# zju3dv/Diffuman4D

Measured on AMD Instinct MI355X. Metric: denoised view-frame latents/sec (44cam x 150fr grid), higher is better.
Workload: dtype bf16; 1 GPU; demo_4d 44cam x 150fr, sliding_fast (window 12, stride 2, 3 rounds, 18 steps/latent), CFG 2.0, 72x40x4 latents; step = 2 spatial (F=16) + 1 temporal (F=24) window calls = 2 denoised latents; VAE excluded; mode=task, unet=SD-2.1 geometry (320,640,1280,1280), 815.6M params, random init seed 0, parallelism=task-parallel x1 (independent tasks per round, no data-path collective), task_streams=3, task_batch=2, precision=fast, finite_outputs=True

## Files before the change

diffuman4d_amd/csrc/gemm.hip:

```cpp
#include "common.h"
#include "gemm_common.h"
#include "gemm_select.h"
#include <stdio.h>


namespace {

template <int BM, int BN, int WM, int WN, bool CONV, int PAR = 0>
__global__ __launch_bounds__(256) void gemm_kernel_glds(GemmParams p) {
  constexpr int BK = 64;
  constexpr int TM = BM / WM, TN = BN / WN, MI = TM / 32, NI = TN / 32;
  constexpr int AW = BM / 32, BW = BN / 32;
  static_assert(WM * WN == 4, "4 waves");
  constexpr int SMEM_MAIN = 2 * (BM + BN) * BK * 2;
  constexpr int SMEM_EPI = 4 * 32 * (EpiGeom<TN>::EPW + 4) * 4;
  constexpr int SMEM_BYTES = SMEM_MAIN > SMEM_EPI ? SMEM_MAIN : SMEM_EPI;
  __shared__ __attribute__((aligned(16))) u16 smem[SMEM_BYTES / 2];
  u16* As = smem;
  u16* Bs = smem + 2 * BM * BK;

  const int tid = threadIdx.x, lane = tid & 63;
  const int wave = __builtin_amdgcn_readfirstlane(tid >> 6);
  const int wm = wave / WN, wn = wave % WN;
  const int l31 = lane & 31, lh = lane >> 5;
// ... 90 lines not shown

  const int sw = (l31 >> 1) & 7;
  issue_slab(0, 0);
  __syncthreads();
  for (int kt = 0; kt < nk; ++kt) {
    const int buf = kt & 1;
    if (kt + 1 < nk) issue_slab(kt + 1, buf ^ 1);
    bf16x8_t af[2][MI], bfr[2][NI];
    auto read_frags = [&](int ks, int slot) {
      const int pos = ((ks * 2 + lh) ^ sw) * 8;
#pragma unroll
      for (int i = 0; i < MI; ++i)
        af[slot][i] = *reinterpret_cast<const bf16x8_t*>(As + (buf * BM + wm * TM + i * 32 + l31) * BK + pos);
#pragma unroll
      for (int j = 0; j < NI; ++j)
        bfr[slot][j] = *reinterpret_cast<const bf16x8_t*>(Bs + (buf * BN + wn * TN + j * 32 + l31) * BK + pos);
    };
    read_frags(0, 0);
#pragma unroll
    for (int ks = 0; ks < 4; ++ks) {
      if (ks + 1 < 4) read_frags(ks + 1, (ks + 1) & 1);
#pragma unroll
      for (int i = 0; i < MI; ++i)
#pragma unroll
        for (int j = 0; j < NI; ++j)
          acc[i][j] = mfma_t<PAR>(af[ks & 1][i], bfr[ks & 1][j], acc[i][j]);
    }
    __syncthreads();
  }
  gemm_epilogue<MI, NI, TM, TN, EpiBudget<WM * WN, MI, NI, SMEM_BYTES>::STRAIGHT, PAR>(p, acc, reinterpret_cast<float*>(smem), m0, n0, wm, wn, wave, lane);
}

template <int Q, int R, int q = 0>
__device__ __forceinline__ void sched_mfma_with_reads() {
  if constexpr (q < Q) {
    constexpr int lo = (q * R) / Q, hi = ((q + 1) * R) / Q;
    if constexpr (hi > lo) __builtin_amdgcn_sched_group_barrier(0x100, hi - lo, 0);
    __builtin_amdgcn_sched_group_barrier(0x008, 1, 0);
    sched_mfma_with_reads<Q, R, q + 1>();
  }
}

template <int MI, int NI, bool RELOAD, int q = 0>
__device__ __forceinline__ void sched_mfma_reload() {
  if constexpr (q < MI * NI) {
    __builtin_amdgcn_sched_group_barrier(0x008, 1, 0);
    constexpr int i = q / NI, j = q % NI;
    constexpr int n = RELOAD ? ((j == NI - 1 ? 1 : 0) + (i == MI - 1 ? 1 : 0)) : 0;
    if constexpr (n > 0) __builtin_amdgcn_sched_group_barrier(0x100, n, 0);
    sched_mfma_reload<MI, NI, RELOAD, q + 1>();
  }
}

template <int BM, int BN, int WM, int WN, int KT = 3, int PAR = 0>
__global__ __launch_bounds__(WM* WN * 64, (BN % 64 != 0 ? 2 : 1)) void conv_strip2_kernel(GemmParams p_in) {
  static_assert(KT == 2 || KT == 3, "3x3 taps, or the 2x2 taps of one upsampling phase");
  constexpr int BK = 64, ROWB = BK * 2;
  constexpr int NW = WM * WN;
  constexpr int TM = BM / WM, TN = BN / WN, MI = TM / 32, NI = TN / 32;
  constexpr int NA = (BM + 8) / 8;
  constexpr int SR = BM + 16;
  constexpr int ZROW = BM + 8;
  constexpr int NB = BN / 8;
  constexpr int AW = (NA + NW - 1) / NW, BW = (NB + NW - 1) / NW;
  constexpr int A_BYTES = SR * ROWB, B_BYTES = BN * ROWB;
  constexpr int SMEM_MAIN = 2 * (A_BYTES + B_BYTES);
  constexpr int SMEM_EPI = NW * 32 * (EpiGeom<TN>::EPW + 4) * 4;
  constexpr int SMEM_BYTES = SMEM_MAIN > SMEM_EPI ? SMEM_MAIN : SMEM_EPI;
  static_assert(SMEM_BYTES <= 160 * 1024, "tile does not fit the LDS");
  static_assert(2 * A_BYTES + 2 * B_BYTES - 1 + 0 < (1 << 20), "LDS offsets");
  __shared__ __attribute__((aligned(16))) char smem[SMEM_BYTES];
  constexpr int BS0 = 2 * A_BYTES;

  const int tid = threadIdx.x, lane = tid & 63;
  const int wave = __builtin_amdgcn_readfirstlane(tid >> 6);
  const int wm = wave / WN, wn = wave % WN;
  const int l31 = lane & 31, lh = lane >> 5;
  int lid = xcd_remap(blockIdx.x, gridDim.x);
  GemmParams p = p_in;
  int xs = -1, ys = -1;
  if constexpr (KT == 2) {
    const int per = gridDim.x / 4, phase = lid / per;
    lid -= phase * per;
    const int py = phase >> 1, px = phase & 1;
    xs = px - 1;
    ys = py - 1;
    p.Wt = p_in.Wt + (int64_t)phase * p_in.N * p_in.ldw;
    p.C = p_in.C + ((int64_t)py * 2 * p_in.W + px) * p_in.ldc * ((PAR && (p_in.flags & DM4D_EPI_F32OUT)) ? 2 : 1);
  }
  int split = 0, tm, tn;
  if (KT == 3 && p.splits > 1) {
    const int rows = gridDim.x / p.tiles_n;
    const int tms = lid % rows;
    tn = lid / rows;
    split = tms / (rows / p.splits);
    tm = tms % (rows / p.splits);
  } else {
    tn = lid % p.tiles_n;
    tm = lid / p.tiles_n;
  }
  const int m0 = tm * BM, n0 = tn * BN;
  const int d_row = lane >> 3, d_pos = lane & 7;
  if (tid < 16) *reinterpret_cast<U4*>(smem + (tid >> 3) * A_BYTES + ZROW * ROWB + (tid & 7) * 16) = U4{0u, 0u, 0u, 0u};

  uint32_t a_voff[AW];
  auto set_a_voff = [&](int ky) {
#pragma unroll
// ... 133 lines not shown
            acc[i][j] = mfma_t<PAR>(af[i], bfr[j], acc[i][j]);
            if (ks + 1 < 4) {
              if (j == NI - 1) af[i] = read_a(ks + 1, i);
              if (i == MI - 1) bfr[j] = read_b(ks + 1, j);
            }
          }
      __builtin_amdgcn_sched_group_barrier(0x100, MI + NI, 0);
      sched_mfma_reload<MI, NI, true>();
      sched_mfma_reload<MI, NI, true>();
      sched_mfma_reload<MI, NI, true>();
      sched_mfma_reload<MI, NI, false>();
    }
  };
  const int cin = p.Cin;
  int c_ky = ky0, c_cs = 0;
  const u16* wp = p.Wt + ky0 * KT * cin;
  set_a_voff(ky0);
  issue_a(p.A, 0);
  issue_b(wp, 0);
  asm volatile("s_waitcnt vmcnt(0)" ::: "memory");
  __syncthreads();
  for (int g = 0; g < nstrips; ++g) {
    if (c_cs == 0) set_a_addrs(c_ky);
    const int abuf = g & 1;
    const int b0 = KT == 3 ? abuf : 0;
    issue_b(wp + cin, b0 ^ 1);
    compute(abuf, std::integral_constant<int, 0>{});
    dma_wait_barrier();
    if constexpr (KT == 3) {
      issue_b(wp + 2 * cin, b0);
      compute(abuf, std::integral_constant<int, 1>{});
      dma_wait_barrier();
    }
    if (++c_cs == nci) {
      c_cs = 0;
      ++c_ky;
    }
    if (g + 1 < nstrips) {
      if (c_cs == 0) set_a_voff(c_ky);
      wp = p.Wt + (c_ky * KT * cin + c_cs * BK);
      issue_a(p.A + c_cs * BK, abuf ^ 1);
      issue_b(wp, KT == 3 ? (abuf ^ 1) : 0);
    }
    compute(abuf, std::integral_constant<int, KT - 1>{});
    dma_wait_barrier();
  }
  if (KT == 3 && p.splits > 1) {
    p.C = reinterpret_cast<u16*>(p.ws + (int64_t)split * p.M * p.N);
    p.ldc = p.N;
    p.flags = DM4D_EPI_F32OUT;
    p.bias = p.rowbias = p.res = nullptr;
    p.out_scale = 1.0f;
  }
  gemm_epilogue<MI, NI, TM, TN, EpiBudget<WM * WN, MI, NI, SMEM_BYTES>::STRAIGHT, PAR>(p, acc, reinterpret_cast<float*>(smem), m0, n0, wm, wn, wave, lane);
}

template <int BM, int BN, int WM, int WN, int NST, bool CONV, int BK = 32, int PAR = 0>
__global__ __launch_bounds__(WM* WN * 64) void gemm_kernel_pipe(GemmParams p) {
  constexpr int NW = WM * WN;
  static_assert(BK == 32 || BK == 64, "K-slab of 32 (64-byte row pieces) or 64 (whole 128-byte lines)");
  constexpr int RPI = 1024 / (BK * 2);
  constexpr int TM = BM / WM, TN = BN / WN, MI = TM / 32, NI = TN / 32;
  constexpr int AW = BM / RPI / NW, BW = BN / RPI / NW;
  static_assert(AW >= 1 && BW >= 1 && NST >= 2 && NST <= 4, "tile/wave/stage combination");
  constexpr int LD = AW + BW;
  constexpr int STAGE = (BM + BN) * BK;
  constexpr int SMEM_MAIN = NST * STAGE * 2;
  constexpr int SMEM_EPI = NW * 32 * (EpiGeom<TN>::EPW + 4) * 4;
  constexpr int SMEM_BYTES = SMEM_MAIN > SMEM_EPI ? SMEM_MAIN : SMEM_EPI;
  __shared__ __attribute__((aligned(16))) u16 smem[SMEM_BYTES / 2];

  const int tid = threadIdx.x, lane = tid & 63;
  const int wave = __builtin_amdgcn_readfirstlane(tid >> 6);
  const int wm = wave / WN, wn = wave % WN;
  const int l31 = lane & 31, lh = lane >> 5;
  const int bid = xcd_remap(blockIdx.x, gridDim.x);
  const int tn = bid % p.tiles_n, tm = bid / p.tiles_n;
  const int m0 = tm * BM;
  const bool geglu = (p.flags & DM4D_EPI_GEGLU) != 0;
  const int n0 = tn * (geglu ? BN / 2 : BN);

  constexpr int CPRW = BK / 8;
  const int d_row = lane / CPRW, d_pos = lane % CPRW;
  auto src_chunk = [&](int row) { return BK == 32 ? (d_pos ^ ((row >> 2) & 3)) : (d_pos ^ ((row >> 1) & 7)); };
  const u16* a_src[AW];
  const u16* a2_src[AW];
  int iy0[AW], ix0[AW], img_off[AW], tap_off[AW];
#pragma unroll
  for (int i = 0; i < AW; ++i) {
    img_off[i] = tap_off[i] = 0;
    const int d_chunk = src_chunk((wave + NW * i) * RPI + d_row);
    int m = m0 + (wave + NW * i) * RPI + d_row;
    if (m > p.M - 1) m = p.M - 1;
    if constexpr (CONV) {
      int ox = m % p.Wo;
      int t = m / p.Wo;
      int oy = t % p.Ho;
      int b = t / p.Ho;
      iy0[i] = oy * p.stride - p.pad;
      ix0[i] = ox * p.stride - p.pad;
      img_off[i] = b * p.H * p.W * p.Cin + d_chunk * 8;
      a_src[i] = p.A;
      a2_src[i] = nullptr;
    } else {
      a_src[i] = p.A + (int64_t)m * p.lda + d_chunk * 8;
      a2_src[i] = p.A2 ? p.A2 + (int64_t)m * p.lda2 + d_chunk * 8 : nullptr;
      iy0[i] = ix0[i] = 0;
    }
  }
  const u16* w_src[BW];
// ... 39 lines not shown
      }
      __builtin_amdgcn_global_load_lds((gptr_t)src, (lptr_t)(As + (wave + NW * i) * RPI * BK), 16, 0, 0);
    }
    if constexpr (CONV) {
      ci0 += BK;
      if (ci0 >= p.Cin) {
        ci0 = 0;
        if (++kx == 3) {
          kx = 0;
          ++ky;
        }
      }
    }
#pragma unroll
    for (int i = 0; i < BW; ++i)
      __builtin_amdgcn_global_load_lds((gptr_t)(w_src[i] + kt * BK), (lptr_t)(Bs + (wave + NW * i) * RPI * BK), 16, 0, 0);
  };

  const int sw = BK == 32 ? ((l31 >> 2) & 3) : ((l31 >> 1) & 7);
#pragma unroll
  for (int s = 0; s < NST - 1; ++s)
    if (s < nk) issue_slab(s, s);
  int st = 0, st_issue = NST - 1;
  for (int kt = 0; kt < nk; ++kt) {
    const int younger = nk - 1 - kt;
    if (NST >= 4 && younger >= 2) {
      asm volatile("s_waitcnt vmcnt(%0)" ::"n"(2 * LD) : "memory");
    } else if (NST >= 3 && younger >= 1) {
      asm volatile("s_waitcnt vmcnt(%0)" ::"n"(LD) : "memory");
    } else {
      asm volatile("s_waitcnt vmcnt(0)" ::: "memory");
    }
    __builtin_amdgcn_s_barrier();
    asm volatile("" ::: "memory");
    if (kt + NST - 1 < nk) issue_slab(kt + NST - 1, st_issue);
    const u16* As = smem + st * STAGE;
    const u16* Bs = As + BM * BK;
#pragma unroll
    for (int ks = 0; ks < BK / 16; ++ks) {
      const int pos = ((ks * 2 + lh) ^ sw) * 8;
      bf16x8_t af[MI], bfr[NI];
#pragma unroll
      for (int i = 0; i < MI; ++i) af[i] = *reinterpret_cast<const bf16x8_t*>(As + (wm * TM + i * 32 + l31) * BK + pos);
#pragma unroll
      for (int j = 0; j < NI; ++j) bfr[j] = *reinterpret_cast<const bf16x8_t*>(Bs + (wn * TN + j * 32 + l31) * BK + pos);
#pragma unroll
      for (int i = 0; i < MI; ++i)
#pragma unroll
        for (int j = 0; j < NI; ++j) acc[i][j] = mfma_t<PAR>(af[i], bfr[j], acc[i][j]);
    }
    st = (st + 1 == NST) ? 0 : st + 1;
    st_issue = (st_issue + 1 == NST) ? 0 : st_issue + 1;
  }
  gemm_epilogue<MI, NI, TM, TN, EpiBudget<WM * WN, MI, NI, SMEM_BYTES>::STRAIGHT, PAR>(p, acc, reinterpret_cast<float*>(smem), m0, n0, wm, wn, wave, lane);
}

template <int BM, int BN, int WM, int WN, int NST, int BK = 64, int PAR = 0>
__global__ __launch_bounds__(WM* WN * 64) void gemm_lin2_kernel(GemmParams p) {
  static_assert(BK == 32 || BK == 64, "K-slab of 32 (64-byte rows, 16 per DMA instruction) or 64 (128-byte rows, 8 per instruction)");
  constexpr int ROWB = BK * 2, RPI = 1024 / ROWB, CPR = BK / 8, KS = BK / 16;
  constexpr int NW = WM * WN;
  constexpr int TM = BM / WM, TN = BN / WN, MI = TM / 32, NI = TN / 32;
  constexpr int AW = BM / RPI / NW, BW = BN / RPI / NW;
  static_assert(AW >= 1 && BW >= 1 && NST >= 2 && NST <= 3, "tile/wave/stage combination");
  constexpr int LD = AW + BW;
  constexpr int STAGE_BYTES = (BM + BN) * ROWB;
  constexpr int SMEM_MAIN = NST * STAGE_BYTES;
  constexpr int SMEM_EPI = NW * 32 * (EpiGeom<TN>::EPW + 4) * 4;
  constexpr int SMEM_BYTES = SMEM_MAIN > SMEM_EPI ? SMEM_MAIN : SMEM_EPI;
  static_assert(SMEM_BYTES <= 160 * 1024, "tile does not fit the LDS");
  __shared__ __attribute__((aligned(16))) char smem[SMEM_BYTES];

  const int tid = threadIdx.x, lane = tid & 63;
  const int wave = __builtin_amdgcn_readfirstlane(tid >> 6);
  const int wm = wave / WN, wn = wave % WN;
  const int l31 = lane & 31, lh = lane >> 5;
  const int bid = xcd_remap(blockIdx.x, gridDim.x);
  const int tn = bid % p.tiles_n, tm = bid / p.tiles_n;
  const int m0 = tm * BM;
  const bool geglu = (p.flags & DM4D_EPI_GEGLU) != 0;
  const int n0 = tn * (geglu ? BN / 2 : BN);
  const int d_row = lane / CPR, d_pos = lane % CPR;
  auto key = [](int row) { return BK == 64 ? ((row >> 1) & 7) : ((row >> 2) & 3); };

  uint32_t a_voff[AW], a2_voff[AW], w_voff[BW];
#pragma unroll
  for (int i = 0; i < AW; ++i) {
    const int row = (wave + NW * i) * RPI + d_row;
    const uint32_t chunk = (uint32_t)(d_pos ^ key(row)) * 16u;
    int m = m0 + row;
    if (m > p.M - 1) m = p.M - 1;
    a_voff[i] = (uint32_t)m * (uint32_t)(p.lda * 2) + chunk;
    a2_voff[i] = (uint32_t)m * (uint32_t)(p.lda2 * 2) + chunk;
  }
#pragma unroll
  for (int i = 0; i < BW; ++i) {
    const int row = (wave + NW * i) * RPI + d_row;
    w_voff[i] = (uint32_t)weight_row<TN>(p, n0, row, geglu) * (uint32_t)(p.ldw * 2) + (uint32_t)(d_pos ^ key(row)) * 16u;
  }
  const uint32_t lds0 = lds_addr(smem);
  const uint32_t a_dst0 = lds0 + wave * 1024, b_dst0 = lds0 + BM * ROWB + wave * 1024;
  const int k1 = p.A2 ? p.K1 : p.K;
  auto issue_slab = [&](int kt, int st) {
    const int k = kt * BK;
    const uint32_t so = st * STAGE_BYTES;
    if (k < k1) {
      const u16* ab = p.A + k;
#pragma unroll
      for (int i = 0; i < AW; ++i) dma16_sv(ab, a_voff[i], a_dst0 + so + NW * i * 1024);
    } else {
// ... 55 lines not shown
        sched_mfma_with_reads<MI * NI, MI + NI>();
        sched_mfma_with_reads<MI * NI, MI + NI>();
      }
      sched_mfma_with_reads<MI * NI, 0>();
    } else {
      bf16x8_t af[MI], bfr[NI];
#pragma unroll
      for (int i = 0; i < MI; ++i) af[i] = read_a(0, i);
#pragma unroll
      for (int j = 0; j < NI; ++j) bfr[j] = read_b(0, j);
#pragma unroll
      for (int ks = 0; ks < KS; ++ks)
#pragma unroll
        for (int i = 0; i < MI; ++i)
#pragma unroll
          for (int j = 0; j < NI; ++j) {
            acc[i][j] = mfma_t<PAR>(af[i], bfr[j], acc[i][j]);
            if (ks + 1 < KS) {
              if (j == NI - 1) af[i] = read_a(ks + 1, i);
              if (i == MI - 1) bfr[j] = read_b(ks + 1, j);
            }
          }
      __builtin_amdgcn_sched_group_barrier(0x100, MI + NI, 0);
      sched_mfma_reload<MI, NI, true>();
      if constexpr (KS == 4) {
        sched_mfma_reload<MI, NI, true>();
        sched_mfma_reload<MI, NI, true>();
      }
      sched_mfma_reload<MI, NI, false>();
    }
  };

  const int nk = p.K / BK;
#pragma unroll
  for (int s = 0; s < NST - 1; ++s)
    if (s < nk) issue_slab(s, s);
  int st = 0, st_issue = NST - 1;
  for (int kt = 0; kt < nk; ++kt) {
    if (NST >= 3 && nk - 1 - kt >= 1) {
      asm volatile("s_waitcnt vmcnt(%0) lgkmcnt(0)" ::"n"(LD) : "memory");
    } else {
      asm volatile("s_waitcnt vmcnt(0) lgkmcnt(0)" ::: "memory");
    }
    __builtin_amdgcn_s_barrier();
    asm volatile("" ::: "memory");
    if (kt + NST - 1 < nk) issue_slab(kt + NST - 1, st_issue);
    compute(st);
    st = (st + 1 == NST) ? 0 : st + 1;
    st_issue = (st_issue + 1 == NST) ? 0 : st_issue + 1;
  }
  asm volatile("s_waitcnt lgkmcnt(0)" ::: "memory");
  __builtin_amdgcn_s_barrier();
  asm volatile("" ::: "memory");
  gemm_epilogue<MI, NI, TM, TN, EpiBudget<WM * WN, MI, NI, SMEM_BYTES>::STRAIGHT, PAR>(p, acc, reinterpret_cast<float*>(smem), m0, n0, wm, wn, wave, lane);
}

template <int BM, int BN, int WM, int WN, bool CONV, int PAR = 0>
__global__ __launch_bounds__(256) void gemm_kernel(GemmParams p) {
  constexpr int LDK = 40;
  constexpr int TM = BM / WM, TN = BN / WN, MI = TM / 32, NI = TN / 32;
  constexpr int AI = BM / 64, BI = BN / 64;
  static_assert(WM * WN == 4, "4 waves");
  constexpr int SMEM_MAIN = 2 * (BM + BN) * LDK * 2;
  constexpr int SMEM_EPI = 4 * 32 * (EpiGeom<TN>::EPW + 4) * 4;
  constexpr int SMEM_BYTES = SMEM_MAIN > SMEM_EPI ? SMEM_MAIN : SMEM_EPI;
  __shared__ __attribute__((aligned(16))) u16 smem[SMEM_BYTES / 2];
  u16* As = smem;
  u16* Bs = smem + 2 * BM * LDK;

  const int tid = threadIdx.x, lane = tid & 63, wave = tid >> 6;
  const int wm = wave / WN, wn = wave % WN;
  const int l31 = lane & 31, lh = lane >> 5;
  const int bid = xcd_remap(blockIdx.x, gridDim.x);
  const int tn = bid % p.tiles_n, tm = bid / p.tiles_n;
  const int m0 = tm * BM;
  const bool geglu = (p.flags & DM4D_EPI_GEGLU) != 0;
  const int n0 = tn * (geglu ? BN / 2 : BN);
  const int a_c = tid & 3, a_r = tid >> 2;

  const u16* a_base[AI];
  const u16* a2_base[AI];
  int iy0[AI], ix0[AI];
#pragma unroll
  for (int i = 0; i < AI; ++i) {
    int m = m0 + a_r + 64 * i;
    if (m > p.M - 1) m = p.M - 1;
    if constexpr (CONV) {
      int ox = m % p.Wo;
      int t = m / p.Wo;
      int oy = t % p.Ho;
      int b = t / p.Ho;
      iy0[i] = oy * p.stride - p.pad;
      ix0[i] = ox * p.stride - p.pad;
      a_base[i] = p.A + (int64_t)b * p.H * p.W * p.Cin;
      a2_base[i] = nullptr;
    } else {
      a_base[i] = p.A + (int64_t)m * p.lda;
      a2_base[i] = p.A2 ? p.A2 + (int64_t)m * p.lda2 : nullptr;
      iy0[i] = ix0[i] = 0;
    }
  }
  const u16* w_base[BI];
#pragma unroll
  for (int i = 0; i < BI; ++i) w_base[i] = p.Wt + (int64_t)weight_row<TN>(p, n0, a_r + 64 * i, geglu) * p.ldw;

  f32x16_t acc[MI][NI];
  acc_init<MI, NI, TN, PAR>(p, acc, n0, wn, lane, geglu);

  const int nk = p.K / 32;
  const int Hin = p.upsample ? 2 * p.H : p.H, Win = p.upsample ? 2 * p.W : p.W;
// ... 8 lines not shown
        bool ok = (unsigned)iy < (unsigned)Hin && (unsigned)ix < (unsigned)Win;
        int sy = p.upsample ? (iy >> 1) : iy, sx = p.upsample ? (ix >> 1) : ix;
        U4 z = {0u, 0u, 0u, 0u};
        ra[i] = ok ? ldg16(a_base[i] + ((int64_t)sy * p.W + sx) * p.Cin + ci0 + a_c * 8) : z;
      }
      ci0 += 32;
      if (ci0 >= p.Cin) {
        ci0 = 0;
        if (++kx == 3) {
          kx = 0;
          ++ky;
        }
      }
    } else {
      const int kcol = kt * 32;
      const bool second = (p.A2 != nullptr) && (kcol >= p.K1);
#pragma unroll
      for (int i = 0; i < AI; ++i)
        ra[i] = second ? ldg16(a2_base[i] + (kcol - p.K1) + a_c * 8) : ldg16(a_base[i] + kcol + a_c * 8);
    }
#pragma unroll
    for (int i = 0; i < BI; ++i) rb[i] = ldg16(w_base[i] + kt * 32 + a_c * 8);
  };
  auto store_slab = [&](int buf) {
#pragma unroll
    for (int i = 0; i < AI; ++i) *reinterpret_cast<U4*>(As + (buf * BM + a_r + 64 * i) * LDK + a_c * 8) = ra[i];
#pragma unroll
    for (int i = 0; i < BI; ++i) *reinterpret_cast<U4*>(Bs + (buf * BN + a_r + 64 * i) * LDK + a_c * 8) = rb[i];
  };

  load_slab(0);
  store_slab(0);
  __syncthreads();
  for (int kt = 0; kt < nk; ++kt) {
    const int buf = kt & 1;
    if (kt + 1 < nk) load_slab(kt + 1);
#pragma unroll
    for (int ks = 0; ks < 2; ++ks) {
      bf16x8_t af[MI], bfr[NI];
#pragma unroll
      for (int i = 0; i < MI; ++i)
        af[i] = *reinterpret_cast<const bf16x8_t*>(As + (buf * BM + wm * TM + i * 32 + l31) * LDK + ks * 16 + lh * 8);
#pragma unroll
      for (int j = 0; j < NI; ++j)
        bfr[j] = *reinterpret_cast<const bf16x8_t*>(Bs + (buf * BN + wn * TN + j * 32 + l31) * LDK + ks * 16 + lh * 8);
#pragma unroll
      for (int i = 0; i < MI; ++i)
#pragma unroll
        for (int j = 0; j < NI; ++j) acc[i][j] = mfma_t<PAR>(af[i], bfr[j], acc[i][j]);
    }
    if (kt + 1 < nk) store_slab(buf ^ 1);
    __syncthreads();
  }
  gemm_epilogue<MI, NI, TM, TN, EpiBudget<WM * WN, MI, NI, SMEM_BYTES>::STRAIGHT, PAR>(p, acc, reinterpret_cast<float*>(smem), m0, n0, wm, wn, wave, lane);
}

template <int BM, int BN>
unsigned tile_grid(GemmParams& p) {
  const int bn_out = is_geglu(p) ? BN / 2 : BN;
  p.tiles_n = (p.N + bn_out - 1) / bn_out;
  return (unsigned)(((p.M + BM - 1) / BM) * p.tiles_n);
}

template <int BM, int BN, int WM, int WN, bool CONV, bool GLDS, int PAR = 0>
int launch_cfg(hipStream_t st, GemmParams& p) {
  const dim3 grid(tile_grid<BM, BN>(p));
  if constexpr (GLDS) {
    hipLaunchKernelGGL((gemm_kernel_glds<BM, BN, WM, WN, CONV, PAR>), grid, dim3(256), 0, st, p);
  } else {
    hipLaunchKernelGGL((gemm_kernel<BM, BN, WM, WN, CONV, PAR>), grid, dim3(256), 0, st, p);
  }
  return dm4d_check_launch("gemm_kernel");
}

template <int BM, int BN, int WM, int WN, int NST, bool CONV, int BK = 32, int PAR = 0>
int launch_pipe(hipStream_t st, GemmParams& p) {
  const dim3 grid(tile_grid<BM, BN>(p));
  hipLaunchKernelGGL((gemm_kernel_pipe<BM, BN, WM, WN, NST, CONV, BK, PAR>), grid, dim3(WM * WN * 64), 0, st, p);
  return dm4d_check_launch("gemm_kernel_pipe");
}

template <int BM, int BN, int WM, int WN, int NST, int BK = 64, int PAR = 0>
int launch_lin2(hipStream_t st, GemmParams& p) {
  const dim3 grid(tile_grid<BM, BN>(p));
  hipLaunchKernelGGL((gemm_lin2_kernel<BM, BN, WM, WN, NST, BK, PAR>), grid, dim3(WM * WN * 64), 0, st, p);
  return dm4d_check_launch("gemm_lin2_kernel");
}

template <int PAR = 0>
__global__ __launch_bounds__(256) void splitk_reduce_kernel(GemmParams p) {
  const int nv = p.N / 8;
  const int64_t id = (int64_t)blockIdx.x * 256 + threadIdx.x;
  if (id >= (int64_t)p.M * nv) return;
  const int m = (int)(id / nv), n = (int)(id % nv) * 8;
  const int64_t plane = (int64_t)p.M * p.N;
  const float* w = p.ws + (int64_t)m * p.N + n;
  float v[8];
  {
    const f32x4_t a0 = *reinterpret_cast<const f32x4_t*>(w), a1 = *reinterpret_cast<const f32x4_t*>(w + 4);
    v[0] = a0[0]; v[1] = a0[1]; v[2] = a0[2]; v[3] = a0[3];
    v[4] = a1[0]; v[5] = a1[1]; v[6] = a1[2]; v[7] = a1[3];
  }
  for (int s = 1; s < p.splits; ++s) {
    const f32x4_t a0 = *reinterpret_cast<const f32x4_t*>(w + s * plane), a1 = *reinterpret_cast<const f32x4_t*>(w + s * plane + 4);
    v[0] += a0[0]; v[1] += a0[1]; v[2] += a0[2]; v[3] += a0[3];
    v[4] += a1[0]; v[5] += a1[1]; v[6] += a1[2]; v[7] += a1[3];
  }
  const bool f32side = PAR == 2 && (p.flags & DM4D_EPI_F32SIDE) != 0;
  auto side = [&](const u16* base, int64_t off, float* t) {
    if (f32side) {
      const float* f = reinterpret_cast<const float*>(base) + off;
      const f32x4_t t0 = *reinterpret_cast<const f32x4_t*>(f), t1 = *reinterpret_cast<const f32x4_t*>(f + 4);
      t[0] = t0[0]; t[1] = t0[1]; t[2] = t0[2]; t[3] = t0[3];
      t[4] = t1[0]; t[5] = t1[1]; t[6] = t1[2]; t[7] = t1[3];
    } else if constexpr (PAR == 2) {
      unpack8h(ldg16(base + off), t);
    } else {
      unpack8(ldg16(base + off), t);
    }
  };
  float t[8];
  if (p.bias) {
    if constexpr (PAR == 2) unpack8h(ldg16(p.bias + n), t);
    else unpack8(ldg16(p.bias + n), t);
#pragma unroll
    for (int e = 0; e < 8; ++e) v[e] += t[e];
  }
  if (p.rowbias) {
    side(p.rowbias, (int64_t)(m / p.rows_per_rb) * p.ld_rb + n, t);
#pragma unroll
    for (int e = 0; e < 8; ++e) v[e] += t[e];
  }
  if (p.res) {
    side(p.res, (int64_t)m * p.ld_res + n, t);
#pragma unroll
    for (int e = 0; e < 8; ++e) v[e] += t[e];
  }
#pragma unroll
  for (int e = 0; e < 8; ++e) v[e] *= p.out_scale;
  if (PAR == 2 && (p.flags & DM4D_EPI_F32OUT)) {
    float* cf = reinterpret_cast<float*>(p.C) + (int64_t)m * p.ldc + n;
    const f32x4_t o0 = {v[0], v[1], v[2], v[3]}, o1 = {v[4], v[5], v[6], v[7]};
    *reinterpret_cast<f32x4_t*>(cf) = o0;
    *reinterpret_cast<f32x4_t*>(cf + 4) = o1;
  } else if constexpr (PAR == 2) {
    stg16(p.C + (int64_t)m * p.ldc + n, pack8h(v));
  } else {
    stg16(p.C + (int64_t)m * p.ldc + n, pack8(v));
  }
}

template <int BM, int BN, int WM, int WN, int PAR = 0>
int launch_strip2(hipStream_t st, GemmParams& p) {
  if (!strip2_ok(p)) return DM4D_ERR_ARG;
  if (BN % 64 != 0 && p.splits > 1) return DM4D_ERR_ARG;
  if (p.splits < 1) p.splits = 1;
  const dim3 grid(tile_grid<BM, BN>(p) * p.splits);
  hipLaunchKernelGGL((conv_strip2_kernel<BM, BN, WM, WN, 3, PAR>), grid, dim3(WM * WN * 64), 0, st, p);
  int rc = dm4d_check_launch("conv_strip2_kernel");
  if (rc || p.splits == 1) return rc;
  const int64_t nthreads = (int64_t)p.M * (p.N / 8);
  hipLaunchKernelGGL((splitk_reduce_kernel<PAR>), dim3((unsigned)((nthreads + 255) / 256)), dim3(256), 0, st, p);
  return dm4d_check_launch("splitk_reduce_kernel");
}

template <int BM, int BN, int WM, int WN, int PAR = 0>
int launch_up2x(hipStream_t st, GemmParams& p) {
  p.splits = 1;
  const dim3 grid(4 * tile_grid<BM, BN>(p));
  hipLaunchKernelGGL((conv_strip2_kernel<BM, BN, WM, WN, 2, PAR>), grid, dim3(WM * WN * 64), 0, st, p);
  return dm4d_check_launch("conv_strip2_kernel<up2x>");
}

template <bool H16 = false>
__global__ __launch_bounds__(256) void up2x_prepare_kernel(const u16* W, u16* Wp, int N, int Cin) {
  const int64_t total = (int64_t)4 * N * 4 * Cin;
  const int64_t id = (int64_t)blockIdx.x * 256 + threadIdx.x;
  if (id >= total) return;
  const int ci = (int)(id % Cin);
  int64_t t = id / Cin;
  const int dx = (int)(t & 1), dy = (int)((t >> 1) & 1);
  t >>= 2;
  const int n = (int)(t % N), phase = (int)(t / N);
  const int py = phase >> 1, px = phase & 1;
  const int ky_lo = py == 0 ? (dy == 0 ? 0 : 1) : (dy == 0 ? 0 : 2), ky_hi = py == 0 ? (dy == 0 ? 0 : 2) : (dy == 0 ? 1 : 2);
  const int kx_lo = px == 0 ? (dx == 0 ? 0 : 1) : (dx == 0 ? 0 : 2), kx_hi = px == 0 ? (dx == 0 ? 0 : 2) : (dx == 0 ? 1 : 2);
  float acc = 0.f;
  for (int ky = ky_lo; ky <= ky_hi; ++ky)
    for (int kx = kx_lo; kx <= kx_hi; ++kx) {
      const u16 w = W[(int64_t)n * 9 * Cin + (ky * 3 + kx) * Cin + ci];
      acc += H16 ? h2f(w) : bf2f(w);
    }
  Wp[id] = H16 ? f2h(acc) : f2bf(acc);
}

int g_tune_cfg = 0;

template <int ID, bool CONV, int PAR>
int launch_id(hipStream_t st, GemmParams& p) {
  constexpr bool STRIP = ID >= 31 && ID <= 37, LIN2 = ID >= 61;
  const bool geglu = is_geglu(p);
  if constexpr ((STRIP && !CONV) || (LIN2 && CONV)) return DM4D_ERR_ARG;
  else if ((ID <= 4 && !k64<CONV>(p)) || (STRIP && !strip_conv(p)) || (LIN2 && !lin2_ok(p))) return DM4D_ERR_ARG;
  else if constexpr (ID == 1) return launch_cfg<128, 128, 2, 2, CONV, true, PAR>(st, p);
  else if constexpr (ID == 2) return launch_cfg<256, 64, 4, 1, CONV, true, PAR>(st, p);
  else if constexpr (ID == 3) return launch_cfg<128, 64, 4, 1, CONV, true, PAR>(st, p);
  else if constexpr (ID == 4) return geglu ? DM4D_ERR_ARG : launch_cfg<64, 64, 2, 2, CONV, true, PAR>(st, p);
  else if constexpr (ID == 13) return launch_pipe<256, 256, 2, 4, 4, CONV, 32, PAR>(st, p);
  else if constexpr (ID == 14) return launch_pipe<256, 128, 4, 2, 3, CONV, 32, PAR>(st, p);
  else if constexpr (ID == 20) return launch_pipe<256, 256, 4, 4, 4, CONV, 32, PAR>(st, p);
  else if constexpr (ID == 46) return (k64<CONV>(p) && !geglu) ? launch_pipe<256, 320, 4, 2, 2, CONV, 64, PAR>(st, p) : DM4D_ERR_ARG;
  else if constexpr (ID == 31) return launch_strip2<128, 128, 2, 2, PAR>(st, p);
  else if constexpr (ID == 32) return launch_strip2<256, 128, 4, 2, PAR>(st, p);
  else if constexpr (ID == 33) return launch_strip2<128, 64, 4, 1, PAR>(st, p);
  else if constexpr (ID == 34) return launch_strip2<256, 256, 2, 4, PAR>(st, p);
  else if constexpr (ID == 35) return launch_strip2<256, 320, 4, 2, PAR>(st, p);
  else if constexpr (ID == 36) return launch_strip2<128, 160, 4, 1, PAR>(st, p);
  else if constexpr (ID == 37) return launch_strip2<256, 160, 8, 1, PAR>(st, p);
  else if constexpr (ID == 67) return launch_lin2<256, 256, 2, 4, 2, 64, PAR>(st, p);
  else if constexpr (ID == 65) return launch_lin2<256, 128, 4, 2, 3, 32, PAR>(st, p);
  else if constexpr (ID == 61) return launch_lin2<256, 128, 4, 2, 3, 64, PAR>(st, p);
  else if constexpr (ID == 69) return geglu ? DM4D_ERR_ARG : launch_lin2<128, 160, 4, 1, 2, 64, PAR>(st, p);
  else if constexpr (ID == 63) return launch_lin2<128, 128, 2, 2, 2, 64, PAR>(st, p);
  else if constexpr (ID == 64) return launch_lin2<128, 128, 4, 2, 3, 64, PAR>(st, p);
  else if constexpr (ID == 21) return launch_cfg<256, 128, 2, 2, CONV, false, PAR>(st, p);
  else if constexpr (ID == 22) return launch_cfg<128, 128, 2, 2, CONV, false, PAR>(st, p);
  else if constexpr (ID == 23) return launch_cfg<256, 64, 4, 1, CONV, false, PAR>(st, p);
  else return launch_cfg<128, 64, 4, 1, CONV, false, PAR>(st, p);
}

template <bool CONV, int PAR>
int launch_from(IdList<>, int, hipStream_t, GemmParams&) { return DM4D_ERR_ARG; }
template <bool CONV, int PAR, int ID, int... REST>
int launch_from(IdList<ID, REST...>, int id, hipStream_t st, GemmParams& p) {
  return id == ID ? launch_id<ID, CONV, PAR>(st, p) : launch_from<CONV, PAR>(IdList<REST...>{}, id, st, p);
}
template <bool CONV, int PAR = 0>
int launch_by_id(int id, hipStream_t st, GemmParams& p) {
  return launch_from<CONV, PAR>(std::conditional_t<PAR == 1, ParIds<CONV>, AllIds>{}, id, st, p);
}

template <bool CONV, bool H16>
int launch(hipStream_t st, GemmParams& p) {
  const bool par = !H16 && (p.flags & (DM4D_EPI_F32SIDE | DM4D_EPI_SPLITOUT)) != 0, forced = !H16 && !par && g_tune_cfg != 0;
  const GemmChoice c = forced ? GemmChoice{g_tune_cfg, 1} : select_cfg<CONV>(p, H16 ? PREC_H16 : par ? PREC_PAR : PREC_FAST);
  if (!c.id) return dm4d_set_error(DM4D_ERR_ARG, "conv3x3: parity-precision launches need Cin % 64 == 0 (a two-term operand of Cin / 2 channels)");
  p.splits = c.splits;
  int rc;
  if constexpr (H16) rc = launch_by_id<CONV, 2>(c.id, st, p);
  else rc = par ? launch_by_id<CONV, 1>(c.id, st, p) : launch_by_id<CONV>(c.id, st, p);
  if (forced && rc == DM4D_ERR_ARG) return dm4d_set_error(DM4D_ERR_ARG, "gemm: forced configuration does not support this shape");
  return rc;
}

int arg_error(const char* name, const char* what) {
  char msg[256];
  snprintf(msg, sizeof(msg), "%s: %s", name, what);
  return dm4d_set_error(DM4D_ERR_ARG, msg);
}

template <bool H16>
int gemm_entry(const char* name, void* stream, const void* A, int64_t lda, const void* A2, int64_t lda2, int K1, const void* W, int64_t ldw, void* C,
               int64_t ldc, int M, int N, int K, const void* bias, const void* rowbias, int64_t ld_rowbias, int rows_per_rowbias,
               const void* residual, int64_t ld_res, unsigned flags, float out_scale, int scale_cols, float col_scale) {
  if (!A || !W || !C || M <= 0 || N <= 0 || K <= 0) return arg_error(name, "null pointer or empty shape");
  if (K % 32 != 0) return arg_error(name, "K must be a multiple of 32");
  if ((lda & 7) || (ldw & 7)) return arg_error(name, "lda/ldw must be multiples of 8");
  if (A2 && ((K1 % 32) != 0 || K1 <= 0 || K1 >= K || (lda2 & 7))) return arg_error(name, "bad split-A arguments");
  if (rowbias && rows_per_rowbias <= 0) return arg_error(name, "rows_per_rowbias <= 0");
  if ((flags & DM4D_EPI_GEGLU) && (N % 32 != 0)) return arg_error(name, "GEGLU needs N % 32 == 0");
  if (H16 && (flags & ~(DM4D_EPI_GEGLU | DM4D_EPI_SILU | DM4D_EPI_F32OUT | DM4D_EPI_F32SIDE)))
    return arg_error(name, "only GEGLU, SILU, F32OUT and F32SIDE apply");
  if (H16 && (scale_cols < 0 || scale_cols > N || (scale_cols & 7))) return arg_error(name, "scale_cols must be a multiple of 8 in [0, N]");
  GemmParams p{};
  p.A = (const u16*)A; p.lda = lda; p.A2 = (const u16*)A2; p.lda2 = lda2; p.K1 = K1;
  p.Wt = (const u16*)W; p.ldw = ldw; p.C = (u16*)C; p.ldc = ldc; p.M = M; p.N = N; p.K = K;
  p.bias = (const u16*)bias; p.rowbias = (const u16*)rowbias; p.ld_rb = ld_rowbias; p.rows_per_rb = rows_per_rowbias;
  p.res = (const u16*)residual; p.ld_res = ld_res; p.flags = H16 ? flags | DM4D_EPI_H16 : flags; p.out_scale = out_scale;
  p.scale_cols = scale_cols; p.col_scale = col_scale;
  return launch<false, H16>((hipStream_t)stream, p);
}

template <bool H16>
int conv3x3_entry(const char* name, void* stream, const void* X, int B, int H, int W, int Cin, const void* Wt, void* Y, int Ho, int Wo, int Cout,
                  int stride, int pad, int upsample, const void* bias, const void* rowbias, int64_t ld_rowbias, const void* residual, int64_t ld_res,
                  float out_scale, unsigned flags, void* ws, size_t ws_bytes) {
  if (!X || !Wt || !Y || B <= 0 || H <= 0 || W <= 0 || Ho <= 0 || Wo <= 0 || Cout <= 0) return arg_error(name, "null pointer or empty shape");
  if (Cin % 32 != 0) return arg_error(name, "Cin must be a multiple of 32 (pad the input)");
  if (stride != 1 && stride != 2) return arg_error(name, "stride must be 1 or 2");
  if (upsample && stride != 1) return arg_error(name, "upsample needs stride 1");
  if (flags & ~(DM4D_EPI_F32OUT | DM4D_EPI_F32SIDE)) return arg_error(name, "only DM4D_EPI_F32OUT and DM4D_EPI_F32SIDE apply to a convolution");
  if ((int64_t)B * H * W * Cin >= (int64_t)1 << 31 || (int64_t)B * Ho * Wo * Cout >= (int64_t)1 << 31)
    return arg_error(name, "tensors of 2^31 or more elements are not supported (split the batch)");
  GemmParams p{};
  p.A = (const u16*)X; p.H = H; p.W = W; p.Cin = Cin; p.Ho = Ho; p.Wo = Wo; p.stride = stride; p.pad = pad; p.upsample = upsample;
  p.Wt = (const u16*)Wt; p.ldw = (int64_t)9 * Cin; p.C = (u16*)Y; p.ldc = Cout; p.M = B * Ho * Wo; p.N = Cout; p.K = 9 * Cin;
  p.bias = (const u16*)bias; p.rowbias = (const u16*)rowbias; p.ld_rb = ld_rowbias; p.rows_per_rb = Ho * Wo;
  p.res = (const u16*)residual; p.ld_res = ld_res; p.flags = H16 ? flags | DM4D_EPI_H16 : flags; p.out_scale = out_scale;
  const size_t need = strip_ws_bytes(p, B);
  p.ws = (ws && need && ws_bytes >= need) ? (float*)ws : nullptr;
  return launch<true, H16>((hipStream_t)stream, p);
}

template <bool H16>
int conv_up2x_entry(const char* name, void* stream, const void* X, int B, int H, int W, int Cin, const void* Wp, void* Y, int Cout, const void* bias,
                    unsigned flags) {
  if (!X || !Wp || !Y || B <= 0 || H <= 0 || W <= 0 || Cout <= 0) return arg_error(name, "null pointer or empty shape");
  if (Cin % 64 != 0 || (Cout & 7) != 0)
    return arg_error(name, H16 ? "Cin must be a multiple of 64 and Cout of 8 (use conv3x3_f16 with upsample = 1)"
                               : "Cin must be a multiple of 64 and Cout of 8 (use conv3x3 with upsample = 1)");
  if (H16 && (flags & ~DM4D_EPI_F32OUT)) return arg_error(name, "only DM4D_EPI_F32OUT applies");
  if ((int64_t)B * H * W * Cin >= (int64_t)1 << 31 || (int64_t)B * 4 * H * W * Cout >= (int64_t)1 << 31)
    return arg_error(name, "tensors of 2^31 or more elements are not supported (split the batch)");
  GemmParams p{};
  p.A = (const u16*)X; p.H = H; p.W = W; p.Cin = Cin; p.Ho = H; p.Wo = W; p.stride = 1; p.pad = 1; p.upsample = 0;
  p.Wt = (const u16*)Wp; p.ldw = (int64_t)4 * Cin; p.C = (u16*)Y; p.ldc = Cout; p.M = B * H * W; p.N = Cout; p.K = 4 * Cin;
  p.bias = (const u16*)bias; p.rows_per_rb = H * W; p.flags = H16 ? flags | DM4D_EPI_H16 : flags; p.out_scale = 1.0f; p.up_w = W;
  if (!strip2_ok(p)) return arg_error(name, "input or weights of 4 GiB or more");
  constexpr int PAR = H16 ? 2 : 0;
  hipStream_t st = (hipStream_t)stream;
  switch (choose_up2x(p)) {
    case 32: return launch_up2x<256, 128, 4, 2, PAR>(st, p);
    case 31: return launch_up2x<128, 128, 2, 2, PAR>(st, p);
    default: return launch_up2x<128, 64, 4, 1, PAR>(st, p);
  }
}

template <bool H16>
int conv_up2x_prepare_entry(const char* name, void* stream, const void* W, void* Wp, int Cout, int Cin) {
  if (!W || !Wp || Cout <= 0 || Cin <= 0) return arg_error(name, "null pointer or empty shape");
  const int64_t total = (int64_t)16 * Cout * Cin;
  hipLaunchKernelGGL(up2x_prepare_kernel<H16>, dim3((unsigned)((total + 255) / 256)), dim3(256), 0, (hipStream_t)stream,
                     (const u16*)W, (u16*)Wp, Cout, Cin);
  return dm4d_check_launch("up2x_prepare_kernel");
}

}

#ifdef DM4D_GEMM_H16_TU
extern "C" int dm4d_gemm_f16(void* stream, const void* A, int64_t lda, const void* A2, int64_t lda2, int K1, const void* W, int64_t ldw, void* C,
                             int64_t ldc, int M, int N, int K, const void* bias, const void* rowbias, int64_t ld_rowbias, int rows_per_rowbias,
                             const void* residual, int64_t ld_res, unsigned flags, float out_scale, int scale_cols, float col_scale) {
  return gemm_entry<true>("gemm_f16", stream, A, lda, A2, lda2, K1, W, ldw, C, ldc, M, N, K, bias, rowbias, ld_rowbias, rows_per_rowbias, residual,
                          ld_res, flags, out_scale, scale_cols, col_scale);
}

extern "C" int dm4d_conv3x3_nhwc_f16(void* stream, const void* X, int B, int H, int W, int Cin, const void* Wt, void* Y, int Ho, int Wo, int Cout,
                                     int stride, int pad, int upsample, const void* bias, const void* rowbias, int64_t ld_rowbias,
                                     const void* residual, int64_t ld_res, float out_scale, unsigned flags, void* ws, size_t ws_bytes) {
  return conv3x3_entry<true>("conv3x3_f16", stream, X, B, H, W, Cin, Wt, Y, Ho, Wo, Cout, stride, pad, upsample, bias, rowbias, ld_rowbias, residual,
                             ld_res, out_scale, flags, ws, ws_bytes);
}

extern "C" int dm4d_conv_up2x_prepare_f16(void* stream, const void* W, void* Wp, int Cout, int Cin) {
  return conv_up2x_prepare_entry<true>("conv_up2x_prepare_f16", stream, W, Wp, Cout, Cin);
}

extern "C" int dm4d_conv_up2x_nhwc_f16(void* stream, const void* X, int B, int H, int W, int Cin, const void* Wp, void* Y, int Cout, const void* bias,
                                       unsigned flags) {
  return conv_up2x_entry<true>("conv_up2x_f16", stream, X, B, H, W, Cin, Wp, Y, Cout, bias, flags);
}
#else

extern "C" int dm4d_tune_set_gemm_config(int id) {
  g_tune_cfg = id;
  return DM4D_OK;
}

extern "C" int dm4d_gemm_bf16(void* stream, const void* A, int64_t lda, const void* A2, int64_t lda2, int K1, const void* W, int64_t ldw, void* C,
                              int64_t ldc, int M, int N, int K, const void* bias, const void* rowbias, int64_t ld_rowbias, int rows_per_rowbias,
                              const void* residual, int64_t ld_res, unsigned flags, float out_scale) {
  return gemm_entry<false>("gemm", stream, A, lda, A2, lda2, K1, W, ldw, C, ldc, M, N, K, bias, rowbias, ld_rowbias, rows_per_rowbias, residual, ld_res,
                           flags, out_scale, 0, 0.0f);
}

extern "C" size_t dm4d_conv3x3_ws_bytes(int B, int H, int W, int Cin, int Ho, int Wo, int Cout, int stride, int pad, int upsample) {
  GemmParams p{};
  p.H = H; p.W = W; p.Cin = Cin; p.Ho = Ho; p.Wo = Wo; p.stride = stride; p.pad = pad; p.upsample = upsample; p.N = Cout; p.ldc = Cout;
  return strip_ws_bytes(p, B);
}

extern "C" int dm4d_conv3x3_nhwc_bf16(void* stream, const void* X, int B, int H, int W, int Cin, const void* Wt, void* Y, int Ho, int Wo, int Cout,
                                      int stride, int pad, int upsample, const void* bias, const void* rowbias, int64_t ld_rowbias,
                                      const void* residual, int64_t ld_res, float out_scale) {
  return conv3x3_entry<false>("conv3x3", stream, X, B, H, W, Cin, Wt, Y, Ho, Wo, Cout, stride, pad, upsample, bias, rowbias, ld_rowbias, residual,
                              ld_res, out_scale, 0, nullptr, 0);
}

extern "C" int dm4d_conv3x3_nhwc_bf16_flags(void* stream, const void* X, int B, int H, int W, int Cin, const void* Wt, void* Y, int Ho, int Wo,
                                            int Cout, int stride, int pad, int upsample, const void* bias, const void* rowbias, int64_t ld_rowbias,
                                            const void* residual, int64_t ld_res, float out_scale, unsigned flags) {
  return conv3x3_entry<false>("conv3x3", stream, X, B, H, W, Cin, Wt, Y, Ho, Wo, Cout, stride, pad, upsample, bias, rowbias, ld_rowbias, residual,
                              ld_res, out_scale, flags, nullptr, 0);
}

extern "C" int dm4d_conv3x3_nhwc_bf16_ws(void* stream, const void* X, int B, int H, int W, int Cin, const void* Wt, void* Y, int Ho, int Wo, int Cout,
                                         int stride, int pad, int upsample, const void* bias, const void* rowbias, int64_t ld_rowbias,
                                         const void* residual, int64_t ld_res, float out_scale, void* ws, size_t ws_bytes) {
  return conv3x3_entry<false>("conv3x3", stream, X, B, H, W, Cin, Wt, Y, Ho, Wo, Cout, stride, pad, upsample, bias, rowbias, ld_rowbias, residual,
                              ld_res, out_scale, 0, ws, ws_bytes);
}

extern "C" int dm4d_conv_up2x_prepare_bf16(void* stream, const void* W, void* Wp, int Cout, int Cin) {
  return conv_up2x_prepare_entry<false>("conv_up2x_prepare", stream, W, Wp, Cout, Cin);
}

extern "C" int dm4d_conv_up2x_nhwc_bf16(void* stream, const void* X, int B, int H, int W, int Cin, const void* Wp, void* Y, int Cout,
                                        const void* bias) {
  return conv_up2x_entry<false>("conv_up2x", stream, X, B, H, W, Cin, Wp, Y, Cout, bias, 0);
}
#endif
```

diffuman4d_amd/csrc/gemm_common.h:

```cpp
#pragma once
#include "common.h"
#include "dm4d.h"
#include "errors.h"
#include "gemm_params.h"
#include <stdlib.h>
#include <type_traits>

namespace {

__device__ __attribute__((aligned(16))) const uint32_t g_zero16[4] = {0u, 0u, 0u, 0u};

template <int TN>
__device__ __forceinline__ int weight_row(const GemmParams& p, int n0, int r, bool geglu) {
  int n;
  if (geglu) {
    int wr = r / TN, rr = r % TN;
    n = n0 + wr * (TN / 2) + (rr % (TN / 2));
    if (n > p.N - 1) n = p.N - 1;
    if (rr >= TN / 2) n += p.N;
  } else {
    n = n0 + r;
    if (n > p.N - 1) n = p.N - 1;
  }
  return n;
// ... 12 lines not shown
#pragma unroll
    for (int q = 0; q < 4; ++q) {
      float v[4];
#pragma unroll
      for (int e = 0; e < 4; ++e) {
        const int r = 4 * q + e;
        v[e] = a[J0 + j][r];
        if constexpr (geglu) {
          v[e] = v[e] * gelu_erf_f(a[J0 + j + NI / 2][r]);
        }
        if constexpr (MODE == 1) v[e] = silu_f(v[e]);
      }
      if constexpr (PLAIN) {
        uint2 pk;
        pk.x = pack_bf2(v[0], v[1]);
        pk.y = pack_bf2(v[2], v[3]);
        *reinterpret_cast<uint2*>(reinterpret_cast<u16*>(srow) + j * 32 + 8 * q) = pk;
      } else {
        const f32x4_t v4 = {v[0], v[1], v[2], v[3]};
        *reinterpret_cast<f32x4_t*>(reinterpret_cast<float*>(srow) + j * 32 + 8 * q) = v4;
      }
    }
  }
}

__device__ __forceinline__ bf16x8_t k0_fragment(u16 bits, int lh) {
  union {
    uint32_t u[4];
    bf16x8_t v;
  } f;
  f.u[0] = lh ? 0u : (uint32_t)bits;
  f.u[1] = f.u[2] = f.u[3] = 0u;
  return f.v;
}

template <int MI, int NI, int TN, int PAR = 0>
__device__ __forceinline__ void acc_init(const GemmParams& p, f32x16_t (&acc)[MI][NI], int n0, int wn, int lane, bool geglu) {
  const int l31 = lane & 31, lh = lane >> 5;
  const bf16x8_t one0 = k0_fragment(PAR == 2 ? 0x3c00 : 0x3f80, lh);
  f32x16_t zero;
#pragma unroll
  for (int r = 0; r < 16; ++r) zero[r] = 0.f;
  const bool use = p.bias != nullptr && p.splits <= 1;
#pragma unroll
  for (int j = 0; j < NI; ++j) {
    u16 bits = 0;
    if (use) bits = p.bias[weight_row<TN>(p, n0, wn * TN + j * 32 + l31, geglu)];
    const bf16x8_t bf = k0_fragment(bits, lh);
#pragma unroll
    for (int i = 0; i < MI; ++i) acc[i][j] = mfma_t<PAR>(one0, bf, zero);
  }
}

template <int MI, int NI, int TM, int TN, int MODE, int EPW, int J0, int JN, bool SYNC, bool STRAIGHT, int PAR = 0>
__device__ __forceinline__ void gemm_epilogue_impl(const GemmParams& p, f32x16_t (&acc)[MI][NI], float* smem_f, int m0, int n0,
                                                   int wm, int wn, int wave, int lane) {
  const int l31 = lane & 31, lh = lane >> 5;
  constexpr bool geglu = MODE == 2;
  constexpr int NJ = geglu ? NI / 2 : NI;
  static_assert(J0 + JN <= NJ && JN * 32 <= EPW, "column group outside the wave's tile or wider than its staging area");
  constexpr int TNO = JN * 32;
  constexpr int SLD = TNO + 4;
  constexpr int SBH = TNO + 4;
  constexpr int CPR = TNO / 8;
  constexpr int TASKS = 32 * CPR;
  float* stage = smem_f + wave * 32 * (EPW + 4);
  const int ncol0 = n0 + wn * (NJ * 32) + J0 * 32;

  const bool vec_ok = ((p.ldc & 7) == 0) && ((p.N & 7) == 0) && (!p.res || (p.ld_res & 7) == 0) &&
                      (!p.rowbias || (p.ld_rb & 7) == 0);
  const bool f32out = (p.flags & DM4D_EPI_F32OUT) != 0;
  constexpr bool CPR_POW2 = (CPR & (CPR - 1)) == 0;
  constexpr int cshift = CPR >= 16 ? 4 : (CPR >= 8 ? 3 : (CPR >= 4 ? 2 : (CPR >= 2 ? 1 : 0)));
  constexpr int cmask = CPR - 1;
  constexpr bool H16 = PAR == 2;
  const bool f32side = PAR && (p.flags & DM4D_EPI_F32SIDE) != 0, splitout = PAR == 1 && (p.flags & DM4D_EPI_SPLITOUT) != 0;
  const bool fast_ok = CPR_POW2 && vec_ok && p.ldc < (1 << 24) && (!p.res || p.ld_res < (1 << 24)) &&
                       (!p.rowbias || p.rows_per_rb > 0) && !f32out && !(PAR && (f32side || splitout)) && p.up_w == 0 && !H16;
  const bool plain = fast_ok && !p.res && !p.rowbias && p.out_scale == 1.0f;
  if constexpr (SYNC) __syncthreads();
#pragma unroll
  for (int i = 0; i < MI; ++i) {
    const int m_base = m0 + wm * TM + i * 32;
    if (plain) {
      u16* sb = reinterpret_cast<u16*>(stage);
      u16* srow = sb + l31 * SBH + 4 * lh;
      stage_block<NI, MODE, J0, JN, true>(acc[i], srow);
      __builtin_amdgcn_fence(__ATOMIC_RELEASE, "wavefront");
      __builtin_amdgcn_fence(__ATOMIC_ACQUIRE, "wavefront");
      u16* c_base = p.C + (int64_t)m_base * p.ldc + ncol0;
      if (TASKS % 64 == 0 && m_base + 32 <= p.M && ncol0 + TNO <= p.N) {
        U4 o[TASKS / 64 > 0 ? TASKS / 64 : 1];
#pragma unroll
        for (int it = 0; it < TASKS / 64; ++it) {
          const int id = lane + it * 64;
          const int row = id >> cshift, cc = id & cmask;
          const uint2* s = reinterpret_cast<const uint2*>(sb + row * SBH + cc * 8);
          const uint2 lo = s[0], hi = s[1];
          o[it].x = lo.x; o[it].y = lo.y; o[it].z = hi.x; o[it].w = hi.y;
        }
#pragma unroll
        for (int it = 0; it < TASKS / 64; ++it) {
          const int id = lane + it * 64;
          const int row = id >> cshift, cc = id & cmask;
          stg16(c_base + (uint32_t)(row * (int)p.ldc + cc * 8), o[it]);
        }
      } else {
#pragma unroll
        for (int it = 0; it < (TASKS + 63) / 64; ++it) {
          const int id = lane + it * 64;
          if (TASKS % 64 != 0 && id >= TASKS) continue;
          const int row = id >> cshift, cc = id & cmask;
          if (m_base + row >= p.M || ncol0 + cc * 8 >= p.N) continue;
          const uint2* s = reinterpret_cast<const uint2*>(sb + row * SBH + cc * 8);
          const uint2 lo = s[0], hi = s[1];
          U4 o;
          o.x = lo.x; o.y = lo.y; o.z = hi.x; o.w = hi.y;
          stg16(c_base + (uint32_t)(row * (int)p.ldc + cc * 8), o);
        }
      }
      __builtin_amdgcn_fence(__ATOMIC_RELEASE, "wavefront");
      __builtin_amdgcn_fence(__ATOMIC_ACQUIRE, "wavefront");
      continue;
    }
    float* srow = stage + l31 * SLD + 4 * lh;
    stage_block<NI, MODE, J0, JN, false>(acc[i], srow);
    __builtin_amdgcn_fence(__ATOMIC_RELEASE, "wavefront");
    __builtin_amdgcn_fence(__ATOMIC_ACQUIRE, "wavefront");
    if (fast_ok) {
      const u16* res_base = p.res ? p.res + (int64_t)m_base * p.ld_res + ncol0 : nullptr;
      u16* c_base = p.C + (int64_t)m_base * p.ldc + ncol0;
      int q0 = 0, r0 = 0;
      if (p.rowbias) {
        q0 = m_base / p.rows_per_rb;
        r0 = m_base - q0 * p.rows_per_rb;
      }
// ... 242 lines not shown
              const u16 hi = f2bf(x);
              p.C[mo * p.ldc + n + e] = hi;
              p.C[mo * p.ldc + p.N + n + e] = f2bf(x - bf2f(hi));
            } else {
              p.C[mo * p.ldc + n + e] = f2bf(x);
            }
          }
        }
      } else {
        if (vec_ok) {
          if (p.rowbias) {
            float t[8];
            unpack8(ldg16(p.rowbias + (int64_t)(m / p.rows_per_rb) * p.ld_rb + n), t);
  #pragma unroll
            for (int e = 0; e < 8; ++e) v[e] += t[e];
          }
          if (p.res) {
            float t[8];
            unpack8(ldg16(p.res + (int64_t)m * p.ld_res + n), t);
  #pragma unroll
            for (int e = 0; e < 8; ++e) v[e] += t[e];
          }
  #pragma unroll
          for (int e = 0; e < 8; ++e) v[e] *= p.out_scale;
          if (f32out) {
            float* cf = reinterpret_cast<float*>(p.C) + mo * p.ldc + n;
            f32x4_t o0 = {v[0], v[1], v[2], v[3]}, o1 = {v[4], v[5], v[6], v[7]};
            *reinterpret_cast<f32x4_t*>(cf) = o0;
            *reinterpret_cast<f32x4_t*>(cf + 4) = o1;
          } else {
            stg16(p.C + mo * p.ldc + n, pack8(v));
          }
        } else {
          for (int e = 0; e < 8 && n + e < p.N; ++e) {
            float x = v[e];
            if (p.rowbias) x += bf2f(p.rowbias[(int64_t)(m / p.rows_per_rb) * p.ld_rb + n + e]);
            if (p.res) x += bf2f(p.res[(int64_t)m * p.ld_res + n + e]);
            if (f32out) reinterpret_cast<float*>(p.C)[mo * p.ldc + n + e] = x * p.out_scale;
            else p.C[mo * p.ldc + n + e] = f2bf(x * p.out_scale);
          }
        }
      }
    }
    __builtin_amdgcn_fence(__ATOMIC_RELEASE, "wavefront");
    __builtin_amdgcn_fence(__ATOMIC_ACQUIRE, "wavefront");
  }
}

template <int TN>
struct EpiGeom {
  static constexpr int EPW = TN <= 128 ? TN : 128;
};

template <int MI, int NI, int TM, int TN, int MODE, bool STRAIGHT, int PAR = 0>
__device__ __forceinline__ void gemm_epilogue_mode(const GemmParams& p, f32x16_t (&acc)[MI][NI], float* smem_f, int m0, int n0,
                                                   int wm, int wn, int wave, int lane) {
  constexpr int NJ = MODE == 2 ? NI / 2 : NI;
  constexpr int EPW = EpiGeom<TN>::EPW;
  constexpr int G = EPW / 32;
  if constexpr (NJ <= G) {
    gemm_epilogue_impl<MI, NI, TM, TN, MODE, EPW, 0, NJ, true, STRAIGHT, PAR>(p, acc, smem_f, m0, n0, wm, wn, wave, lane);
  } else {
    static_assert(NJ <= 2 * G, "at most two column groups");
    gemm_epilogue_impl<MI, NI, TM, TN, MODE, EPW, 0, G, true, STRAIGHT, PAR>(p, acc, smem_f, m0, n0, wm, wn, wave, lane);
    gemm_epilogue_impl<MI, NI, TM, TN, MODE, EPW, G, NJ - G, false, STRAIGHT, PAR>(p, acc, smem_f, m0, n0, wm, wn, wave, lane);
  }
}

template <int NW, int MI, int NI, int SMEM>
struct EpiBudget {
  static constexpr bool STRAIGHT = NW <= 8 && MI * NI <= 8 && !(NW == 8 && SMEM <= 80 * 1024);
};

template <int MI, int NI, int TM, int TN, bool STRAIGHT = false, int PAR = 0>
__device__ __forceinline__ void gemm_epilogue(const GemmParams& p, f32x16_t (&acc)[MI][NI], float* smem_f, int m0, int n0,
                                              int wm, int wn, int wave, int lane) {
  if constexpr (NI >= 2 && NI % 2 == 0) {
    if (p.flags & DM4D_EPI_GEGLU) {
      gemm_epilogue_mode<MI, NI, TM, TN, 2, STRAIGHT, PAR>(p, acc, smem_f, m0, n0, wm, wn, wave, lane);
      return;
    }
  }
  if (p.flags & DM4D_EPI_SILU) gemm_epilogue_mode<MI, NI, TM, TN, 1, STRAIGHT, PAR>(p, acc, smem_f, m0, n0, wm, wn, wave, lane);
  else gemm_epilogue_mode<MI, NI, TM, TN, 0, STRAIGHT, PAR>(p, acc, smem_f, m0, n0, wm, wn, wave, lane);
}


__device__ __forceinline__ void dma16_sv(const void* uniform_base, uint32_t lane_byte_off, uint32_t lds_dst) {
  asm volatile("s_mov_b32 m0, %2\n\ts_nop 0\n\tglobal_load_lds_dwordx4 %0, %1"
               :
               : "v"(lane_byte_off), "s"(uniform_base), "s"(lds_dst)
               : "memory");
}


}
```

diffuman4d_amd/csrc/gemm_params.h:

```cpp
#pragma once
#include <stdint.h>

typedef unsigned short u16;

namespace {

struct GemmParams {
  const u16* A;
  int64_t lda;
  const u16* A2;
  int64_t lda2;
  int K1;
  int H, W, Cin, Ho, Wo, stride, pad, upsample;
  const u16* Wt;
  int64_t ldw;
  u16* C;
  int64_t ldc;
  int M, N, K;
  const u16* bias;
  const u16* rowbias;
  int64_t ld_rb;
  int rows_per_rb;
  const u16* res;
  int64_t ld_res;
  unsigned flags;
  float out_scale;
  int tiles_n;
  int splits;
  float* ws;
  int up_w;
  int scale_cols;
  float col_scale;
};

}
```

diffuman4d_amd/csrc/gemm_select.h:

```cpp
#pragma once
#include "dm4d.h"
#include "gemm_params.h"
#include <stddef.h>
#include <type_traits>
#include <utility>

namespace {

enum { PREC_FAST = 0, PREC_PAR = 1, PREC_H16 = 2 };
struct GemmChoice { int id, splits; };

inline bool is_geglu(const GemmParams& p) { return (p.flags & DM4D_EPI_GEGLU) != 0; }

inline bool strip_conv(const GemmParams& p) {
  return p.stride == 1 && p.pad == 1 && !p.upsample && p.Ho == p.H && p.Wo == p.W && p.Cin % 64 == 0;
}

template <bool CONV>
inline bool k64(const GemmParams& p) { return CONV ? (p.Cin % 64 == 0) : (p.K % 64 == 0 && (!p.A2 || p.K1 % 64 == 0)); }
inline bool n128(const GemmParams& p) { return is_geglu(p) || (p.N % 128 == 0) || (p.N > 1024); }

inline bool lin2_ok(const GemmParams& p) {
  return p.K % 64 == 0 && (!p.A2 || p.K1 % 64 == 0) && (uint64_t)p.M * (uint64_t)p.lda * 2u < (1ull << 32) &&
         (!p.A2 || (uint64_t)p.M * (uint64_t)p.lda2 * 2u < (1ull << 32)) &&
// ... 74 lines not shown
      if (p.N % 256 == 0 && tm256 * (p.N / 256) >= 256) return 20;
    }
    if (!geglu && p.N % 256 == 0 && tm256 * (p.N / 256) >= 384) return 13;
  }
  if (n128(p)) {
    if (tm128 * tn >= 256) return 1;
    if (geglu) return 3;
    return tm128 * tn >= 200 ? 3 : 4;
  }
  return tm256 * ((p.N + 63) / 64) >= 384 ? 2 : 3;
}

template <int... I>
using IdList = std::integer_sequence<int, I...>;
using AllIds = IdList<1, 2, 3, 4, 13, 14, 20, 46, 31, 32, 33, 35, 36, 37, 34, 67, 65, 61, 69, 63, 64, 21, 22, 23, 24>;
template <bool CONV>
using ParIds = std::conditional_t<CONV, IdList<33, 32, 31, 1, 3, 4>, IdList<22, 24, 67, 65, 61, 69, 63, 64, 1, 3, 4>>;

template <int... I>
constexpr bool has_id(IdList<I...>, int id) { return ((id == I) || ...); }
constexpr bool par_has_id(bool conv, int id) { return conv ? has_id(ParIds<true>{}, id) : has_id(ParIds<false>{}, id); }

template <bool CONV>
int choose_par(const GemmParams& p) {
  const bool geglu = is_geglu(p);
  const long tm128 = (p.M + 127) / 128, tm256 = (p.M + 255) / 256, tn = (p.N + (geglu ? 63 : 127)) / (geglu ? 64 : 128);
  if (CONV) {
    if (!k64<CONV>(p)) return 0;
    if (strip_conv(p) && strip2_ok(p)) {
      if (!n128(p)) return 33;
      return tm256 * tn >= 200 ? 32 : 31;
    }
  } else {
    if (!k64<CONV>(p)) return n128(p) ? 22 : 24;
    if (lin2_ok(p)) {
      const int id = choose_cfg<false>(p);
      if (id >= 61 && par_has_id(false, id)) return id;
    }
  }
  if (n128(p)) {
    if (tm128 * tn >= 256 || geglu) return 1;
    return tm128 * tn >= 200 ? 3 : 4;
  }
  return 3;
}

template <bool CONV>
GemmChoice select_cfg(const GemmParams& p, int prec) {
  if (prec == PREC_PAR) return {choose_par<CONV>(p), 1};
  if (CONV && p.ws && strip_conv(p) && strip_split_ok(p) && strip2_ok(p)) return {31, 3};
  return {choose_cfg<CONV>(p), 1};
}

inline int choose_up2x(const GemmParams& p) {
  const long tm256 = (p.M + 255) / 256;
  if (p.N % 128 == 0) return tm256 * (p.N / 128) >= 200 ? 32 : 31;
  return 33;
}

}
```

diffuman4d_amd/csrc/norm.hip:

```cpp
#include "common.h"
#include "dm4d.h"
#include "errors.h"

namespace {

constexpr int GN_THREADS = 256;
constexpr int GN_MAXC = 4096;

__host__ __device__ inline int gn_nchunk(int B, int HW) {
  int n = (2048 + B - 1) / B;
  int cap = (HW + 15) / 16;
  if (n > cap) n = cap;
  if (n < 1) n = 1;
  return n;
}

template <int IO>
struct NormIO;
template <>
struct NormIO<0> {
  typedef u16 in_t;
  typedef U4 raw_t;
  static __device__ __forceinline__ raw_t ldraw(const u16* p) { return ldg16(p); }
  static __device__ __forceinline__ void unpack(const raw_t& r, float* v) { unpack8(r, v); }
  static __device__ __forceinline__ float ld1(const u16* p) { return bf2f(*p); }
  static __device__ __forceinline__ void st8(u16* p, const float* v) { stg16(p, pack8(v)); }
  static __device__ __forceinline__ void par8(const u16* p, float* v) { unpack8(ldg16(p), v); }
};
template <>
struct NormIO<2> {
  typedef float in_t;
  struct raw_t {
    f32x4_t a, b;
  };
  static __device__ __forceinline__ raw_t ldraw(const float* p) {
    raw_t r;
    r.a = *reinterpret_cast<const f32x4_t*>(p);
    r.b = *reinterpret_cast<const f32x4_t*>(p + 4);
    return r;
  }
  static __device__ __forceinline__ void unpack(const raw_t& r, float* v) {
    v[0] = r.a[0]; v[1] = r.a[1]; v[2] = r.a[2]; v[3] = r.a[3];
    v[4] = r.b[0]; v[5] = r.b[1]; v[6] = r.b[2]; v[7] = r.b[3];
  }
  static __device__ __forceinline__ float ld1(const float* p) { return *p; }
  static __device__ __forceinline__ void st8(u16* p, const float* v) { stg16(p, pack8h_sat(v)); }
  static __device__ __forceinline__ void par8(const u16* p, float* v) { unpack8h(ldg16(p), v); }
};

template <>
struct NormIO<3> {
  typedef u16 in_t;
  typedef U4 raw_t;
  static __device__ __forceinline__ raw_t ldraw(const u16* p) { return ldg16(p); }
  static __device__ __forceinline__ void unpack(const raw_t& r, float* v) { unpack8h(r, v); }
  static __device__ __forceinline__ float ld1(const u16* p) { return h2f(*p); }
  static __device__ __forceinline__ void st8(u16* p, const float* v) { stg16(p, pack8h_sat(v)); }
  static __device__ __forceinline__ void par8(const u16* p, float* v) { unpack8h(ldg16(p), v); }
};

struct GNParams {
  const void* X1;
  const void* X2;
  int C1, C2, B, HW, groups, nchunk;
  float eps;
  const u16* gamma;
  const u16* beta;
  u16* Y;
  int silu;
  float* ws;
  u16* Yraw;
};

template <int IO = 0>
__device__ __forceinline__ float gn_shift(const GNParams& p, int b, int g, int gs) {
  typedef typename NormIO<IO>::in_t in_t;
  const int c = g * gs;
  return c < p.C1 ? NormIO<IO>::ld1(static_cast<const in_t*>(p.X1) + (int64_t)b * p.HW * p.C1 + c)
                  : NormIO<IO>::ld1(static_cast<const in_t*>(p.X2) + (int64_t)b * p.HW * p.C2 + (c - p.C1));
}
template <int IO = 0>
__device__ __forceinline__ void gn_shift8(const GNParams& p, int b, int cv, int gs, float (&sh)[8]) {
  const int g0 = (cv * 8) / gs, g1 = (cv * 8 + 7) / gs;
  if (g1 - g0 <= 1) {
    const float s0 = gn_shift<IO>(p, b, g0, gs), s1 = g1 != g0 ? gn_shift<IO>(p, b, g1, gs) : s0;
#pragma unroll
    for (int e = 0; e < 8; ++e) sh[e] = (cv * 8 + e) / gs == g0 ? s0 : s1;
  } else {
#pragma unroll
    for (int e = 0; e < 8; ++e) sh[e] = gn_shift<IO>(p, b, (cv * 8 + e) / gs, gs);
  }
}

template <int IO = 0>
__global__ __launch_bounds__(GN_THREADS) void gn_stats_kernel(GNParams p) {
  typedef NormIO<IO> io;
  typedef typename io::in_t in_t;
  typedef typename io::raw_t raw_t;
  extern __shared__ __attribute__((aligned(16))) float sm[];
  const int C = p.C1 + p.C2, CV = C / 8, CV1 = p.C1 / 8;
  const int b = blockIdx.x / p.nchunk, chunk = blockIdx.x % p.nchunk;
  const int per = (p.HW + p.nchunk - 1) / p.nchunk;
  const int p0 = chunk * per, p1 = min(p0 + per, p.HW);
  const int PPB = CV >= GN_THREADS ? 1 : GN_THREADS / CV;
  const int tid = threadIdx.x;

  for (int slot = tid; slot < CV * PPB; slot += GN_THREADS) {
    const int cv = slot % CV, prow = slot / CV;
    float s[8], q[8], sh[8];
    gn_shift8<IO>(p, b, cv, C / p.groups, sh);
#pragma unroll
    for (int e = 0; e < 8; ++e) s[e] = q[e] = 0.f;
    const in_t* src;
    int ld, c;
    if (cv < CV1) {
      src = static_cast<const in_t*>(p.X1) + (int64_t)b * p.HW * p.C1;
      ld = p.C1;
      c = cv * 8;
    } else {
      src = static_cast<const in_t*>(p.X2) + (int64_t)b * p.HW * p.C2;
      ld = p.C2;
      c = (cv - CV1) * 8;
    }
    auto add = [&](const raw_t& r) {
// ... 1 lines not shown
      io::unpack(r, v);
#pragma unroll
      for (int e = 0; e < 8; ++e) {
        const float d = v[e] - sh[e];
        s[e] += d;
        q[e] += d * d;
      }
    };
    int px = p0 + prow;
#pragma nounroll
    for (; px + PPB < p1; px += 2 * PPB) {
      const in_t* a = src + (int64_t)px * ld + c;
      const raw_t r0 = io::ldraw(a), r1 = io::ldraw(a + (int64_t)PPB * ld);
      add(r0);
      add(r1);
    }
    for (; px < p1; px += PPB) add(io::ldraw(src + (int64_t)px * ld + c));
#pragma unroll
    for (int e = 0; e < 8; ++e) {
      sm[(prow * C + cv * 8 + e) * 2 + 0] = s[e];
      sm[(prow * C + cv * 8 + e) * 2 + 1] = q[e];
    }
  }
  __syncthreads();
  const int gs = C / p.groups;
  for (int g = tid; g < p.groups; g += GN_THREADS) {
    float s = 0.f, q = 0.f;
    for (int r = 0; r < PPB; ++r)
      for (int c = g * gs; c < (g + 1) * gs; ++c) {
        s += sm[(r * C + c) * 2 + 0];
        q += sm[(r * C + c) * 2 + 1];
      }
    float* w = p.ws + (((int64_t)b * p.nchunk + chunk) * p.groups + g) * 2;
    w[0] = s;
    w[1] = q;
  }
}

template <int IO = 0>
__global__ __launch_bounds__(GN_THREADS) void gn_apply_kernel(GNParams p) {
  typedef NormIO<IO> io;
  typedef typename io::in_t in_t;
  typedef typename io::raw_t raw_t;
  extern __shared__ __attribute__((aligned(16))) float sm[];
  const int C = p.C1 + p.C2, CV = C / 8, CV1 = p.C1 / 8;
  float* sc = sm;
  float* mean = sm + (2 * C > 2 * GN_THREADS ? 2 * C : 2 * GN_THREADS);
  float* rstd = mean + p.groups;
  const int b = blockIdx.x / p.nchunk, chunk = blockIdx.x % p.nchunk;
  const int per = (p.HW + p.nchunk - 1) / p.nchunk;
  const int p0 = chunk * per, p1 = min(p0 + per, p.HW);
  const int tid = threadIdx.x;
  const int gs = C / p.groups;
  {
    const int slices = GN_THREADS / p.groups > 0 ? GN_THREADS / p.groups : 1;
    const int g = tid % p.groups, sl = tid / p.groups;
    float s = 0.f, q = 0.f;
    if (sl < slices) {
      for (int k = sl; k < p.nchunk; k += slices) {
        const float* w = p.ws + (((int64_t)b * p.nchunk + k) * p.groups + g) * 2;
        s += w[0];
        q += w[1];
      }
      sc[(sl * p.groups + g) * 2 + 0] = s;
      sc[(sl * p.groups + g) * 2 + 1] = q;
    }
    __syncthreads();
  }
  for (int g = tid; g < p.groups; g += GN_THREADS) {
    const int slices = GN_THREADS / p.groups > 0 ? GN_THREADS / p.groups : 1;
    float s = 0.f, q = 0.f;
    for (int sl = 0; sl < slices; ++sl) {
      s += sc[(sl * p.groups + g) * 2 + 0];
      q += sc[(sl * p.groups + g) * 2 + 1];
    }
    const float n = (float)gs * (float)p.HW;
    const float dm = s / n;
    float var = q / n - dm * dm;
    var = var < 0.f ? 0.f : var;
    mean[g] = gn_shift<IO>(p, b, g, gs) + dm;
    rstd[g] = rsqrtf(var + p.eps);
  }
  __syncthreads();
  const int PPB = CV >= GN_THREADS ? 1 : GN_THREADS / CV;
  for (int slot = tid; slot < CV * PPB; slot += GN_THREADS) {
    const int cv = slot % CV, prow = slot / CV;
    float a[8], sft[8];
    {
      float gm[8], bt[8];
      io::par8(p.gamma + cv * 8, gm);
      io::par8(p.beta + cv * 8, bt);
#pragma unroll
      for (int e = 0; e < 8; ++e) {
        const int g = (cv * 8 + e) / gs;
        a[e] = gm[e] * rstd[g];
        sft[e] = bt[e] - mean[g] * a[e];
      }
    }
    const in_t* src;
    int ld;
    if (cv < CV1) {
      src = static_cast<const in_t*>(p.X1) + (int64_t)b * p.HW * p.C1 + cv * 8;
      ld = p.C1;
    } else {
      src = static_cast<const in_t*>(p.X2) + (int64_t)b * p.HW * p.C2 + (cv - CV1) * 8;
      ld = p.C2;
    }
    u16* dst = p.Y + (int64_t)b * p.HW * C + cv * 8;
    u16* dst_raw = (IO == 2 && p.Yraw) ? p.Yraw + (int64_t)b * p.HW * C + cv * 8 : nullptr;
    auto put = [&](const raw_t& r, int px) {
      float v[8];
      io::unpack(r, v);
      if constexpr (IO == 2) {
        if (dst_raw) io::st8(dst_raw + (int64_t)px * C, v);
      }
#pragma unroll
      for (int e = 0; e < 8; ++e) {
        const float y = v[e] * a[e] + sft[e];
        v[e] = p.silu ? silu_f(y) : y;
      }
      io::st8(dst + (int64_t)px * C, v);
    };
    int px = p0 + prow;
#pragma nounroll
    for (; px + 3 * PPB < p1; px += 4 * PPB) {
      const in_t* s0 = src + (int64_t)px * ld;
      const raw_t r0 = io::ldraw(s0), r1 = io::ldraw(s0 + (int64_t)PPB * ld), r2 = io::ldraw(s0 + (int64_t)2 * PPB * ld), r3 = io::ldraw(s0 + (int64_t)3 * PPB * ld);
      put(r0, px);
      put(r1, px + PPB);
      put(r2, px + 2 * PPB);
      put(r3, px + 3 * PPB);
    }
    for (; px < p1; px += PPB) put(io::ldraw(src + (int64_t)px * ld), px);
  }
}

constexpr int GN_RES_MAXGPS = 8;

template <int NV, int IO = 0>
__global__ __launch_bounds__(GN_THREADS) void gn_resident_kernel(GNParams p, int gps, int SV, int PPB, int NS, int xcd_map) {
  typedef NormIO<IO> io;
  typedef typename io::in_t in_t;
  typedef typename io::raw_t raw_t;
  __shared__ float sm[2 * 8 * GN_THREADS];
  __shared__ float sm2[2 * GN_THREADS];
  __shared__ float stat[2 * GN_RES_MAXGPS];
  const int C = p.C1 + p.C2, CV1 = p.C1 / 8, gs = C / p.groups, SC = SV * 8;
  int b, slab;
  if (xcd_map) {
    const int x = blockIdx.x & 7, j = blockIdx.x >> 3;
    b = x + 8 * (j / NS);
    slab = j % NS;
  } else {
    b = blockIdx.x / NS;
    slab = blockIdx.x % NS;
  }
  const int tid = threadIdx.x, sv = tid % SV, prow = tid / SV;
  const bool active = prow < PPB;
  const int cv = slab * gps * gs / 8 + sv;
  const in_t* src;
  int ld;
  if (cv < CV1) {
    src = static_cast<const in_t*>(p.X1) + (int64_t)b * p.HW * p.C1 + cv * 8;
    ld = p.C1;
  } else {
    src = static_cast<const in_t*>(p.X2) + (int64_t)b * p.HW * p.C2 + (cv - CV1) * 8;
    ld = p.C2;
  }
  raw_t r[NV];
#pragma unroll
  for (int k = 0; k < NV; ++k) {
    const int px = prow + k * PPB;
    if (active && px < p.HW) r[k] = io::ldraw(src + (int64_t)px * ld);
  }
  {
    float s[8], q[8], sh[8];
    gn_shift8<IO>(p, b, cv, gs, sh);
#pragma unroll
    for (int e = 0; e < 8; ++e) s[e] = q[e] = 0.f;
#pragma unroll
    for (int k = 0; k < NV; ++k) {
      const int px = prow + k * PPB;
      if (active && px < p.HW) {
        float v[8];
        io::unpack(r[k], v);
#pragma unroll
// ... 204 lines not shown
    w.y = pack_bf2(__builtin_amdgcn_exp2f(fmaf(v[2], c, -mc)) * inv, __builtin_amdgcn_exp2f(fmaf(v[3], c, -mc)) * inv);
    o[i] = w;
  }
  if (tail) prow[4 * n4 + tid] = f2bf(et * inv);
}

}

extern "C" size_t dm4d_groupnorm_ws_bytes(int B, int HW, int groups) {
  return (size_t)B * gn_nchunk(B, HW) * groups * 2 * sizeof(float);
}

template <int IO>
static int groupnorm_impl(void* stream, const void* X1, int C1, const void* X2, int C2, int B, int HW, int groups, float eps,
                          const void* gamma, const void* beta, void* Y, int apply_silu, void* ws, void* Yraw = nullptr) {
  if (!X1 || !gamma || !beta || !Y || !ws || B <= 0 || HW <= 0 || groups <= 0)
    return dm4d_set_error(DM4D_ERR_ARG, "groupnorm: null pointer or empty shape");
  if (!X2) C2 = 0;
  const int C = C1 + C2;
  if ((C1 & 7) || (C2 & 7) || C % groups != 0 || C > GN_MAXC)
    return dm4d_set_error(DM4D_ERR_ARG, "groupnorm: channels must be multiples of 8, divisible by groups, <= 4096");
  GNParams p{X1, X2, C1, C2, B, HW, groups, gn_nchunk(B, HW), eps,
             (const u16*)gamma, (const u16*)beta, (u16*)Y, apply_silu, (float*)ws, (u16*)Yraw};
  hipStream_t st = (hipStream_t)stream;
  {
    int gps, SV, RPB, NV;
    if (g_gn_resident && gn_resident_plan(C, HW, groups, &gps, &SV, &RPB, &NV)) {
      const int NS = groups / gps, xcd = (B % 8 == 0);
      const dim3 grid(B * NS), blk(GN_THREADS);
      if (NV <= 2) hipLaunchKernelGGL((gn_resident_kernel<2, IO>), grid, blk, 0, st, p, gps, SV, RPB, NS, xcd);
      else if (NV <= 4) hipLaunchKernelGGL((gn_resident_kernel<4, IO>), grid, blk, 0, st, p, gps, SV, RPB, NS, xcd);
      else if (NV <= 8) hipLaunchKernelGGL((gn_resident_kernel<8, IO>), grid, blk, 0, st, p, gps, SV, RPB, NS, xcd);
      else hipLaunchKernelGGL((gn_resident_kernel<16, IO>), grid, blk, 0, st, p, gps, SV, RPB, NS, xcd);
      return dm4d_check_launch("gn_resident_kernel");
    }
  }
  const int CV = C / 8;
  const int PPB = CV >= GN_THREADS ? 1 : GN_THREADS / CV;
  const size_t sm1 = (size_t)PPB * C * 2 * sizeof(float);
  const size_t sm2 = ((size_t)(2 * C > 2 * GN_THREADS ? 2 * C : 2 * GN_THREADS) + 2 * groups) * sizeof(float);
  hipLaunchKernelGGL(gn_stats_kernel<IO>, dim3(B * p.nchunk), dim3(GN_THREADS), sm1, st, p);
  int rc = dm4d_check_launch("gn_stats_kernel");
  if (rc) return rc;
  hipLaunchKernelGGL(gn_apply_kernel<IO>, dim3(B * p.nchunk), dim3(GN_THREADS), sm2, st, p);
  return dm4d_check_launch("gn_apply_kernel");
}

extern "C" int dm4d_groupnorm_nhwc_bf16(void* stream, const void* X1, int C1, const void* X2, int C2, int B, int HW,
                                        int groups, float eps, const void* gamma, const void* beta, void* Y,
                                        int apply_silu, void* ws) {
  return groupnorm_impl<0>(stream, X1, C1, X2, C2, B, HW, groups, eps, gamma, beta, Y, apply_silu, ws);
}

extern "C" int dm4d_groupnorm_f32_f16_general(void* stream, const float* X1, int C1, const float* X2, int C2, int B, int HW, int groups,
                                              float eps, const void* gamma, const void* beta, void* Y, int apply_silu, void* ws);
extern "C" int dm4d_groupnorm_nhwc_f32_f16(void* stream, const float* X1, int C1, const float* X2, int C2, int B, int HW, int groups,
                                           float eps, const void* gamma, const void* beta, void* Y, int apply_silu, void* ws) {
  if (!X2) C2 = 0;
  if ((C1 & 7) || (C2 & 7) || (((uintptr_t)X1) & 15) || (X2 && (((uintptr_t)X2) & 15)) || (((uintptr_t)Y) & 15))
    return dm4d_groupnorm_f32_f16_general(stream, X1, C1, X2, C2, B, HW, groups, eps, gamma, beta, Y, apply_silu, ws);
  return groupnorm_impl<2>(stream, X1, C1, X2, C2, B, HW, groups, eps, gamma, beta, Y, apply_silu, ws);
}

extern "C" int dm4d_groupnorm_nhwc_f16_f16(void* stream, const void* X1, int C1, const void* X2, int C2, int B, int HW, int groups,
                                           float eps, const void* gamma, const void* beta, void* Y, int apply_silu, void* ws) {
  if (!X2) C2 = 0;
  if ((C1 & 7) || (C2 & 7) || (((uintptr_t)X1) & 15) || (X2 && (((uintptr_t)X2) & 15)) || (((uintptr_t)Y) & 15))
    return dm4d_set_error(DM4D_ERR_ARG, "groupnorm_f16_f16: channel counts must be multiples of 8, tensors 16-byte aligned");
  return groupnorm_impl<3>(stream, X1, C1, X2, C2, B, HW, groups, eps, gamma, beta, Y, apply_silu, ws);
}

extern "C" int dm4d_groupnorm_nhwc_f32_f16_raw(void* stream, const float* X1, int C1, const float* X2, int C2, int B, int HW, int groups,
                                               float eps, const void* gamma, const void* beta, void* Y, void* Yraw, int apply_silu,
                                               void* ws) {
  if (!X2) C2 = 0;
  if (!Yraw || (C1 & 7) || (C2 & 7) || (((uintptr_t)X1) & 15) || (X2 && (((uintptr_t)X2) & 15)) || ((((uintptr_t)Y) | ((uintptr_t)Yraw)) & 15))
    return dm4d_set_error(DM4D_ERR_ARG, "groupnorm_f32_f16_raw: needs Yraw, channel counts that are multiples of 8 and 16-byte aligned tensors");
  return groupnorm_impl<2>(stream, X1, C1, X2, C2, B, HW, groups, eps, gamma, beta, Y, apply_silu, ws, Yraw);
}

template <int IO>
static int layernorm_impl(void* stream, const void* X, int64_t ldx, const void* gamma, const void* beta, void* Y, int64_t ldy, int M,
                          int C, float eps) {
  typedef typename NormIO<IO>::in_t in_t;
  hipStream_t st = (hipStream_t)stream;
  const int nv = (C / 8 + 63) / 64;
  dim3 grid((M + 3) / 4), block(256);
#define LN_LAUNCH(NV) \
  hipLaunchKernelGGL((ln_kernel<NV, IO>), grid, block, 0, st, (const in_t*)X, ldx, (const u16*)gamma, (const u16*)beta, (u16*)Y, ldy, M, C, eps)
  if (nv <= 1) LN_LAUNCH(1);
  else if (nv <= 2) LN_LAUNCH(2);
  else if (nv <= 3) LN_LAUNCH(3);
  else if (nv <= 4) LN_LAUNCH(4);
  else LN_LAUNCH(8);
#undef LN_LAUNCH
  return dm4d_check_launch("ln_kernel");
}

extern "C" int dm4d_layernorm_bf16(void* stream, const void* X, int64_t ldx, const void* gamma, const void* beta,
                                   void* Y, int64_t ldy, int M, int C, float eps) {
  if (!X || !gamma || !beta || !Y || M <= 0 || C <= 0)
    return dm4d_set_error(DM4D_ERR_ARG, "layernorm: null pointer or empty shape");
  if ((C & 7) || (ldx & 7) || (ldy & 7) || C > 64 * 8 * 8)
    return dm4d_set_error(DM4D_ERR_ARG, "layernorm: C must be a multiple of 8 and <= 4096");
  return layernorm_impl<0>(stream, X, ldx, gamma, beta, Y, ldy, M, C, eps);
}
// ... 35 lines not shown
```

diffuman4d_amd/host/lib.py:

```python
from __future__ import annotations

import ctypes as C
from pathlib import Path

_LIB_PATH = Path(__file__).resolve().parent.parent / "libdm4d.so"
_lib = None

_vp, _i, _i64, _f, _u = C.c_void_p, C.c_int, C.c_int64, C.c_float, C.c_uint

SIGNATURES = {
    "dm4d_version": (_i, []),
    "dm4d_last_error": (C.c_char_p, []),
    "dm4d_gemm_bf16": (_i, [_vp, _vp, _i64, _vp, _i64, _i, _vp, _i64, _vp, _i64, _i, _i, _i, _vp, _vp, _i64, _i, _vp,
                            _i64, _u, _f]),
    "dm4d_conv3x3_nhwc_bf16": (_i, [_vp, _vp, _i, _i, _i, _i, _vp, _vp, _i, _i, _i, _i, _i, _i, _vp, _vp, _i64, _vp,
                                    _i64, _f]),
    "dm4d_conv3x3_nhwc_bf16_ws": (_i, [_vp, _vp, _i, _i, _i, _i, _vp, _vp, _i, _i, _i, _i, _i, _i, _vp, _vp, _i64, _vp,
                                    _i64, _f, _vp, C.c_size_t]),
    "dm4d_conv3x3_nhwc_bf16_flags": (_i, [_vp, _vp, _i, _i, _i, _i, _vp, _vp, _i, _i, _i, _i, _i, _i, _vp, _vp, _i64, _vp,
                                          _i64, _f, _u]),
    "dm4d_conv3x3_ws_bytes": (C.c_size_t, [_i, _i, _i, _i, _i, _i, _i, _i, _i, _i]),
    "dm4d_conv2d_direct_nhwc_bf16": (_i, [_vp, _vp, _i, _i, _i, _i, _vp, _vp, _vp, _i, _i, _i, _i, _i, _i, _i]),
    "dm4d_conv2d_direct_nhwc_f32": (_i, [_vp, _vp, _i, _i, _i, _i, _vp, _vp, _vp, _i, _i, _i, _i, _i, _i, _i]),
    "dm4d_groupnorm_ws_bytes": (C.c_size_t, [_i, _i, _i]),
    "dm4d_groupnorm_nhwc_bf16": (_i, [_vp, _vp, _i, _vp, _i, _i, _i, _i, _f, _vp, _vp, _vp, _i, _vp]),
    "dm4d_layernorm_bf16": (_i, [_vp, _vp, _i64, _vp, _vp, _vp, _i64, _i, _i, _f]),
    "dm4d_attention_bf16": (_i, [_vp, _vp, _vp, _vp, _vp, _i64, _i64, _i64, _i64, _i, _i, _i, _f]),
    "dm4d_attention_kv_bf16": (_i, [_vp, _vp, _vp, _vp, _vp, _i64, _i64, _i64, _i64, _i, _i, _i, _i, _f]),
    "dm4d_attention_qscaled_kv_bf16": (_i, [_vp, _vp, _vp, _vp, _vp, _i64, _i64, _i64, _i64, _i, _i, _i, _i]),
    "dm4d_softmax_rows_bf16": (_i, [_vp, _vp, _i64, _vp, _i64, _i, _i, _f]),
    "dm4d_softmax_rows_f32in_bf16": (_i, [_vp, _vp, _i64, _vp, _i64, _i, _i, _f]),
    "dm4d_timestep_embedding_bf16": (_i, [_vp, _vp, _vp, _i, _i, _i, _f]),
    "dm4d_silu_bf16": (_i, [_vp, _vp, _vp, _i64]),
    "dm4d_pack_model_input_bf16": (_i, [_vp, _vp, _vp, _vp, _vp, _vp, _vp, _vp, _vp, _i, _i, _i, _i]),
    "dm4d_cfg_ddim_step_bf16": (_i, [_vp, _vp, _vp, _i64, _vp, _vp, _vp, _i, _i, _i, _f, _i]),
    "dm4d_cfg_linear_step_bf16": (_i, [_vp, _vp, _vp, _vp, _i64, _vp, _vp, _vp, _i, _i, _i, _f]),
    "dm4d_cfg_multistep_step_bf16": (_i, [_vp, _vp, _vp, _vp, _vp, _vp, _i64, _vp, _vp, _vp, _i, _i, _i, _f]),
    "dm4d_vae_sample_bf16": (_i, [_vp, _vp, _i64, _vp, _vp, _i64, _i, _f]),
    "dm4d_scale_pad_bf16": (_i, [_vp, _vp, _i64, _vp, _i, _i64, _i, _f]),
    "dm4d_resize_nchw_f32_to_nhwc_bf16": (_i, [_vp, _vp, _vp, _i, _i, _i, _i, _i, _i, _i]),
    "dm4d_plucker_latent_bf16": (_i, [_vp, _vp, _vp, _i, _i, _i, _i, _i]),
    "dm4d_postprocess_images_bf16": (_i, [_vp, _vp, _vp, _i, _i, _i, _i]),
    "dm4d_resize_aa_nchw_f32": (_i, [_vp, _vp, _vp, _i64, _i, _i, _i, _i]),
    "dm4d_conv_up2x_prepare_bf16": (_i, [_vp, _vp, _vp, _i, _i]),
    "dm4d_conv_up2x_nhwc_bf16": (_i, [_vp, _vp, _i, _i, _i, _i, _vp, _vp, _i, _vp]),
    "dm4d_ff_geglu_prepare_bf16": (_i, [_vp, _vp, _vp, _vp, _vp, _vp, _vp, _i, _i]),
    "dm4d_ff_geglu_supported": (_i, [_i, _i]),
    "dm4d_ff_geglu_fused_bf16": (_i, [_vp, _vp, _i64, _vp, _vp, _f, _vp, _vp, _vp, _vp, _vp, _i64, _vp, _i64, _i, _i, _i]),
    "dm4d_attn_out_ff_geglu_fused_bf16": (_i, [_vp, _vp, _i64, _vp, _vp, _vp, _i64, _vp, _vp, _f, _vp, _vp, _vp, _vp, _vp, _i64, _i, _i,
                                                _i]),
    "dm4d_l0_linear_fused_supported": (_i, [_i]),
    "dm4d_proj_in_ln_qkv_fused_bf16": (_i, [_vp, _vp, _i64, _vp, _vp, _vp, _vp, _f, _vp, _vp, _i64, _vp, _i64, _vp, _i64, _i, _i]),
    "dm4d_split_f32": (_i, [_vp, _vp, _i64, _i64, _i, _vp, _i64, _i, _vp, _i64, _i64, _i, _i, _f, _i]),
    "dm4d_groupnorm_f32_ws_bytes": (C.c_size_t, [_i, _i, _i]),
    "dm4d_groupnorm_nhwc_f32_split": (_i, [_vp, _vp, _i, _vp, _i, _i, _i, _i, _f, _vp, _vp, _vp, _i, _vp]),
    "dm4d_layernorm_f32_split": (_i, [_vp, _vp, _i64, _vp, _vp, _vp, _i64, _i, _i, _f]),
    "dm4d_softmax_rows_f32_split": (_i, [_vp, _vp, _i64, _vp, _i64, _i, _i, _i, _f]),
    "dm4d_attention_split_bf16": (_i, [_vp, _vp, _vp, _vp, _vp, _i64, _i64, _i64, _i64, _i64, _i64, _i64, _i64, _i, _i, _i, _i, _f]),
    "dm4d_timestep_embedding_f32": (_i, [_vp, _vp, _vp, _i, _i, _i, _f]),
    "dm4d_pack_model_input_f32_split": (_i, [_vp, _vp, _vp, _vp, _vp, _vp, _vp, _vp, _vp, _i, _i, _i, _i]),
    "dm4d_cfg_ddim_step_f32": (_i, [_vp, _vp, _vp, _i64, _vp, _vp, _vp, _i, _i, _i, _f, _i]),
    "dm4d_cfg_linear_step_f32": (_i, [_vp, _vp, _vp, _vp, _i64, _vp, _vp, _vp, _i, _i, _i, _f]),
    "dm4d_cfg_multistep_step_f32": (_i, [_vp, _vp, _vp, _vp, _vp, _vp, _i64, _vp, _vp, _vp, _i, _i, _i, _f]),
    "dm4d_vae_sample_f32": (_i, [_vp, _vp, _i64, _vp, _vp, _i64, _i, _f]),
    "dm4d_resize_nchw_f32_to_nhwc_f32": (_i, [_vp, _vp, _vp, _i, _i, _i, _i, _i, _i, _i]),
    "dm4d_plucker_latent_f32": (_i, [_vp, _vp, _vp, _i, _i, _i, _i, _i]),
    "dm4d_postprocess_images_f32": (_i, [_vp, _vp, _vp, _i, _i, _i, _i]),
    "dm4d_nhwc_to_nchw_f32": (_i, [_vp, _vp, _vp, _i, _i, _i, _i]),
    "dm4d_gemm_f16": (_i, [_vp, _vp, _i64, _vp, _i64, _i, _vp, _i64, _vp, _i64, _i, _i, _i, _vp, _vp, _i64, _i, _vp, _i64, _u, _f, _i, _f]),
    "dm4d_conv3x3_nhwc_f16": (_i, [_vp, _vp, _i, _i, _i, _i, _vp, _vp, _i, _i, _i, _i, _i, _i, _vp, _vp, _i64, _vp, _i64, _f, _u, _vp,
                                   C.c_size_t]),
    "dm4d_conv_up2x_prepare_f16": (_i, [_vp, _vp, _vp, _i, _i]),
    "dm4d_conv_up2x_nhwc_f16": (_i, [_vp, _vp, _i, _i, _i, _i, _vp, _vp, _i, _vp, _u]),
    "dm4d_to_f16_f32": (_i, [_vp, _vp, _i64, _i64, _i, _vp, _i64, _i, _vp, _i64, _i64, _i, _i, _f]),
    "dm4d_groupnorm_nhwc_f32_f16": (_i, [_vp, _vp, _i, _vp, _i, _i, _i, _i, _f, _vp, _vp, _vp, _i, _vp]),
    "dm4d_groupnorm_nhwc_f16_f16": (_i, [_vp, _vp, _i, _vp, _i, _i, _i, _i, _f, _vp, _vp, _vp, _i, _vp]),
    "dm4d_groupnorm_nhwc_f32_f16_raw": (_i, [_vp, _vp, _i, _vp, _i, _i, _i, _i, _f, _vp, _vp, _vp, _vp, _i, _vp]),
    "dm4d_layernorm_f32_f16": (_i, [_vp, _vp, _i64, _vp, _vp, _vp, _i64, _i, _i, _f]),
# ... 71 lines not shown
```

diffuman4d_amd/host/ops.py:

```python
from __future__ import annotations

import os

from typing import Optional, Tuple

import torch

from . import lib as _l

BF16 = torch.bfloat16
F16 = torch.float16
F32 = torch.float32


def _stream() -> int:
    return torch.cuda.current_stream().cuda_stream


TRACE = None


def _trace(name: str, out, **inputs) -> None:
    if TRACE is not None:
        TRACE.append((name, inputs, out))


def _req(t: torch.Tensor, name: str, dtype=BF16):
    if not isinstance(t, torch.Tensor) or not t.is_cuda:
        raise _l.Dm4dError(f"{name}: expected a tensor on a HIP device (no CPU fallback in diffuman4d_amd)")
    if t.dtype != dtype:
        raise _l.Dm4dError(f"{name}: expected dtype {dtype}, got {t.dtype}")
    if t.stride(-1) != 1:
        raise _l.Dm4dError(f"{name}: last dim must be contiguous")
    return t


def _p(t: Optional[torch.Tensor]):
    return None if t is None else t.data_ptr()


def gemm(a: torch.Tensor, w: torch.Tensor, *, a2: Optional[torch.Tensor] = None, bias=None, rowbias=None,
         rows_per_rowbias: int = 1, residual=None, geglu: bool = False, silu: bool = False, out_scale: float = 1.0,
         out: Optional[torch.Tensor] = None, out_f32: bool = False, split_out: bool = False, scale_cols: int = 0,
         col_scale: float = 1.0) -> torch.Tensor:
    if isinstance(w, torch.Tensor) and w.dtype == F16:
        return _gemm_f16(a, w, a2, bias, rowbias, rows_per_rowbias, residual, geglu, silu, out_scale, out, out_f32, scale_cols, col_scale)
    assert scale_cols == 0
    lib = _l.load()
    _req(a, "a"), _req(w, "w")
    M, K1 = a.shape
    K = w.shape[1]
    N = w.shape[0] // 2 if geglu else w.shape[0]
    if a2 is not None:
        _req(a2, "a2")
        assert a2.shape[0] == M and K1 + a2.shape[1] == K
    else:
        assert K1 == K, (K1, K)
    if bias is not None:
        _req(bias, "bias")
    side = [t for t in (rowbias, residual) if t is not None]
    f32_side = bool(side) and side[0].dtype == F32
    for t, n in ((rowbias, "rowbias"), (residual, "residual")):
        if t is not None:
            _req(t, n, F32 if f32_side else BF16)
    assert not (out_f32 and split_out)
    odt, ocols = (F32 if out_f32 else BF16), (2 * N if split_out else N)
    if out is None:
        out = torch.empty((M, ocols), dtype=odt, device=a.device)
    _req(out, "out", odt)
    assert out.shape[1] >= ocols or out.stride(0) >= ocols
    flags = ((_l.EPI_GEGLU if geglu else 0) | (_l.EPI_SILU if silu else 0) | (_l.EPI_F32OUT if out_f32 else 0)
             | (_l.EPI_F32SIDE if f32_side else 0) | (_l.EPI_SPLITOUT if split_out else 0))
    with _Prof("linear", 2.0 * M * w.shape[0] * K, "flop", M):
        rc = lib.dm4d_gemm_bf16(_stream(), _p(a), a.stride(0), _p(a2), a2.stride(0) if a2 is not None else 0,
                                K1 if a2 is not None else 0, _p(w), w.stride(0), _p(out), out.stride(0), M, N, K,
                                _p(bias), _p(rowbias), rowbias.stride(0) if rowbias is not None else 0,
                                rows_per_rowbias, _p(residual), residual.stride(0) if residual is not None else 0,
                                flags, out_scale)
    _l.check(rc, "dm4d_gemm_bf16")
    _trace("gemm", out, a=a, w=w, a2=a2, bias=bias, rowbias=rowbias, rows_per_rowbias=rows_per_rowbias, residual=residual, geglu=geglu,
           silu=silu, out_scale=out_scale, out_f32=out_f32, split_out=split_out)
    return out


def _gemm_f16(a, w, a2, bias, rowbias, rows_per_rowbias, residual, geglu, silu, out_scale, out, out_f32, scale_cols, col_scale):
    lib = _l.load()
    _req(a, "a", F16), _req(w, "w", F16)
    M, K1 = a.shape
    K = w.shape[1]
    N = w.shape[0] // 2 if geglu else w.shape[0]
    if a2 is not None:
        _req(a2, "a2", F16)
        assert a2.shape[0] == M and K1 + a2.shape[1] == K
    else:
        assert K1 == K, (K1, K)
    if bias is not None:
        _req(bias, "bias", F16)
    side = [t for t in (rowbias, residual) if t is not None]
    f32_side = bool(side) and side[0].dtype == F32
    for t, n in ((rowbias, "rowbias"), (residual, "residual")):
        if t is not None:
            _req(t, n, F32 if f32_side else F16)
    odt = F32 if out_f32 else F16
    if out is None:
        out = torch.empty((M, N), dtype=odt, device=a.device)
    _req(out, "out", odt)
    assert out.shape[1] >= N or out.stride(0) >= N
    flags = ((_l.EPI_GEGLU if geglu else 0) | (_l.EPI_SILU if silu else 0) | (_l.EPI_F32OUT if out_f32 else 0)
             | (_l.EPI_F32SIDE if f32_side else 0))
    with _Prof("linear", 2.0 * M * w.shape[0] * K, "flop", M):
        rc = lib.dm4d_gemm_f16(_stream(), _p(a), a.stride(0), _p(a2), a2.stride(0) if a2 is not None else 0,
                               K1 if a2 is not None else 0, _p(w), w.stride(0), _p(out), out.stride(0), M, N, K,
                               _p(bias), _p(rowbias), rowbias.stride(0) if rowbias is not None else 0,
                               rows_per_rowbias, _p(residual), residual.stride(0) if residual is not None else 0,
                               flags, out_scale, int(scale_cols), float(col_scale))
    _l.check(rc, "dm4d_gemm_f16")
    return out


def conv_out_hw(h: int, w: int, stride: int, pad: int, upsample: bool, pad_hi: Optional[int] = None) -> Tuple[int, int]:
    if upsample:
        return 2 * h, 2 * w
    ph = pad if pad_hi is None else pad_hi
    return (h + pad + ph - 3) // stride + 1, (w + pad + ph - 3) // stride + 1


def conv3x3(x: torch.Tensor, wt: torch.Tensor, *, bias=None, rowbias=None, residual=None, stride: int = 1,
            pad: int = 1, pad_hi: Optional[int] = None, upsample: bool = False, out_scale: float = 1.0,
            out_f32: bool = False) -> torch.Tensor:
    lib = _l.load()
    if isinstance(wt, torch.Tensor) and wt.dtype == F16:
        return _conv3x3_f16(x, wt, bias, rowbias, residual, stride, pad, pad_hi, upsample, out_scale, out_f32)
    _req(x, "x"), _req(wt, "wt")
    assert x.is_contiguous() and wt.is_contiguous()
    B, H, W, Cin = x.shape
    Cout = wt.shape[0]
    assert wt.shape[1] == 9 * Cin, (wt.shape, Cin)
    Ho, Wo = conv_out_hw(H, W, stride, pad, upsample, pad_hi)
    y = torch.empty((B, Ho, Wo, Cout), dtype=F32 if out_f32 else BF16, device=x.device)
    side = F32 if out_f32 else BF16
    if residual is not None:
        _req(residual, "residual", side)
        assert residual.numel() == y.numel() and residual.is_contiguous()
    if rowbias is not None:
        _req(rowbias, "rowbias", side)
        assert rowbias.shape[0] == B
    if out_f32:
        with _Prof("conv3x3", 2.0 * B * Ho * Wo * 9 * Cin * Cout, "flop", B * Ho * Wo):
            rc = lib.dm4d_conv3x3_nhwc_bf16_flags(_stream(), _p(x), B, H, W, Cin, _p(wt), _p(y), Ho, Wo, Cout, stride, pad,
                                                  1 if upsample else 0, _p(bias), _p(rowbias),
                                                  rowbias.stride(0) if rowbias is not None else 0, _p(residual),
                                                  Cout if residual is not None else 0, out_scale, _l.EPI_F32OUT | _l.EPI_F32SIDE)
        _l.check(rc, "dm4d_conv3x3_nhwc_bf16_flags")
        _trace("conv3x3", y, x=x, wt=wt, bias=bias, rowbias=rowbias, residual=residual, stride=stride, pad=pad, pad_hi=pad_hi,
               upsample=upsample, out_scale=out_scale, out_f32=True)
        return y
    ws_bytes = lib.dm4d_conv3x3_ws_bytes(B, H, W, Cin, Ho, Wo, Cout, stride, pad, 1 if upsample else 0)
    ws = torch.empty(ws_bytes // 4, dtype=torch.float32, device=x.device) if ws_bytes else None
    with _Prof("conv3x3", 2.0 * B * Ho * Wo * 9 * Cin * Cout, "flop", B * Ho * Wo):
        rc = lib.dm4d_conv3x3_nhwc_bf16_ws(_stream(), _p(x), B, H, W, Cin, _p(wt), _p(y), Ho, Wo, Cout, stride, pad,
                                           1 if upsample else 0, _p(bias), _p(rowbias),
                                           rowbias.stride(0) if rowbias is not None else 0, _p(residual),
                                           Cout if residual is not None else 0, out_scale, _p(ws), ws_bytes)
    _l.check(rc, "dm4d_conv3x3_nhwc_bf16_ws")
    _trace("conv3x3", y, x=x, wt=wt, bias=bias, rowbias=rowbias, residual=residual, stride=stride, pad=pad, pad_hi=pad_hi,
           upsample=upsample, out_scale=out_scale, out_f32=False)
    return y


def _conv3x3_f16(x, wt, bias, rowbias, residual, stride, pad, pad_hi, upsample, out_scale, out_f32) -> torch.Tensor:
    lib = _l.load()
    _req(x, "x", F16), _req(wt, "wt", F16)
    assert x.is_contiguous() and wt.is_contiguous()
    B, H, W, Cin = x.shape
    Cout = wt.shape[0]
    assert wt.shape[1] == 9 * Cin, (wt.shape, Cin)
    Ho, Wo = conv_out_hw(H, W, stride, pad, upsample, pad_hi)
    y = torch.empty((B, Ho, Wo, Cout), dtype=F32 if out_f32 else F16, device=x.device)
    sides = [t for t in (rowbias, residual) if t is not None]
    side = F32 if (out_f32 or (sides and sides[0].dtype == F32)) else F16
    if bias is not None:
        _req(bias, "bias", F16)
    if residual is not None:
        _req(residual, "residual", side)
        assert residual.numel() == y.numel() and residual.is_contiguous()
    if rowbias is not None:
        _req(rowbias, "rowbias", side)
        assert rowbias.shape[0] == B
    ws_bytes = lib.dm4d_conv3x3_ws_bytes(B, H, W, Cin, Ho, Wo, Cout, stride, pad, 1 if upsample else 0)
    ws = torch.empty(ws_bytes // 4, dtype=torch.float32, device=x.device) if ws_bytes else None
    with _Prof("conv3x3", 2.0 * B * Ho * Wo * 9 * Cin * Cout, "flop", B * Ho * Wo):
        rc = lib.dm4d_conv3x3_nhwc_f16(_stream(), _p(x), B, H, W, Cin, _p(wt), _p(y), Ho, Wo, Cout, stride, pad,
                                       1 if upsample else 0, _p(bias), _p(rowbias),
                                       rowbias.stride(0) if rowbias is not None else 0, _p(residual),
                                       Cout if residual is not None else 0, out_scale,
                                       (_l.EPI_F32OUT if out_f32 else 0) | (_l.EPI_F32SIDE if side == F32 else 0), _p(ws), ws_bytes)
    _l.check(rc, "dm4d_conv3x3_nhwc_f16")
    return y


def dup_k(w: torch.Tensor, taps: int = 1, times: int = 2) -> torch.Tensor:
    n, k = w.shape
    c = k // taps
    return w.reshape(n, taps, 1, c).expand(n, taps, times, c).reshape(n, taps * times * c).contiguous()


def split(x: torch.Tensor, x2: Optional[torch.Tensor] = None, *, cpad: Optional[int] = None, silu: bool = False,
          scale: float = 1.0, pattern: int = 0, transposed: bool = False, h16: bool = False) -> torch.Tensor:
    lib = _l.load()
    if not isinstance(x, torch.Tensor) or not x.is_cuda or x.dtype != F32:
        raise _l.Dm4dError("split: expected an fp32 tensor on a HIP device")
    planes = 1 if h16 else (2 if pattern == 0 else 3)
    if transposed:
        assert x.ndim == 2 and x2 is None and x.stride(1) == 1
        C1, M = x.shape
        rs1, cs1, lead = 1, x.stride(0), (M,)
    else:
        assert x.stride(-1) == 1
        C1 = x.shape[-1]
        x2d = x.reshape(-1, C1) if x.is_contiguous() else x
# ... 191 lines not shown
                raise _l.Dm4dError("Upsampler: phase kernels were not prepared on the input's device")
            return conv_up2x(split(x, h16=True), self.wp, bias=self.bias, out_f32=True)
        if self.parity:
            return conv3x3(split(x, h16=self.h16), self.wt, bias=self.bias, upsample=True, out_f32=True)
        if not self.phase or x.numel() * 2 >= (1 << 32):
            return conv3x3(x, self.wt, bias=self.bias, upsample=True)
        if self.wp is None or self.wp.device != x.device:
            raise _l.Dm4dError(f"Upsampler: phase kernels live on {None if self.wp is None else self.wp.device}, input on {x.device} "
                            "(reload the pipeline on the new device: host/loader.py does)")
        return conv_up2x(x, self.wp, bias=self.bias)


def conv_up2x(x: torch.Tensor, wp: torch.Tensor, *, bias=None, out_f32: bool = False) -> torch.Tensor:
    lib = _l.load()
    h16 = wp.dtype == F16
    dt = F16 if h16 else BF16
    _req(x, "x", dt), _req(wp, "wp", dt)
    assert x.is_contiguous() and wp.is_contiguous() and (h16 or not out_f32)
    B, H, W, Cin = x.shape
    Cout = wp.shape[1]
    assert wp.shape == (4, Cout, 4 * Cin), (wp.shape, Cin)
    y = torch.empty((B, 2 * H, 2 * W, Cout), dtype=F32 if out_f32 else dt, device=x.device)
    with _Prof("conv3x3", 2.0 * B * 4 * H * W * 4 * Cin * Cout, "flop", B * 4 * H * W):
        if h16:
            rc = lib.dm4d_conv_up2x_nhwc_f16(_stream(), _p(x), B, H, W, Cin, _p(wp), _p(y), Cout, _p(bias), _l.EPI_F32OUT if out_f32 else 0)
        else:
            rc = lib.dm4d_conv_up2x_nhwc_bf16(_stream(), _p(x), B, H, W, Cin, _p(wp), _p(y), Cout, _p(bias))
    _l.check(rc, "dm4d_conv_up2x_nhwc")
    if not h16:
        _trace("conv_up2x", y, x=x, wp=wp, bias=bias)
    return y


def conv2d_direct(x: torch.Tensor, wt: torch.Tensor, *, ksize: int, bias=None, stride: int = 1, pad: int = 1,
                  silu: bool = False) -> torch.Tensor:
    lib = _l.load()
    dt = F32 if x.dtype == F32 else BF16
    _req(x, "x", dt), _req(wt, "wt", dt)
    if bias is not None:
        _req(bias, "bias", dt)
    assert x.is_contiguous() and wt.is_contiguous()
    B, H, W, Cin = x.shape
    Cout = wt.shape[0]
    assert wt.shape[1] == ksize * ksize * Cin, (wt.shape, ksize, Cin)
    Ho, Wo = (H + 2 * pad - ksize) // stride + 1, (W + 2 * pad - ksize) // stride + 1
    y = torch.empty((B, Ho, Wo, Cout), dtype=dt, device=x.device)
    fn = lib.dm4d_conv2d_direct_nhwc_f32 if dt == F32 else lib.dm4d_conv2d_direct_nhwc_bf16
    rc = fn(_stream(), _p(x), B, H, W, Cin, _p(wt), _p(bias), _p(y), Ho, Wo, Cout, ksize, stride, pad, 1 if silu else 0)
    _l.check(rc, "dm4d_conv2d_direct_nhwc")
    return y


def groupnorm(x1: torch.Tensor, gamma: torch.Tensor, beta: torch.Tensor, groups: int, eps: float, *,
              x2: Optional[torch.Tensor] = None, silu: bool = False, raw_out: bool = False):
    lib = _l.load()
    if isinstance(x1, torch.Tensor) and x1.dtype == F32:
        return _groupnorm_f32(x1, gamma, beta, groups, eps, x2, silu, raw_out)
    assert not raw_out
    if isinstance(x1, torch.Tensor) and x1.dtype == F16:
        return _groupnorm_f16(x1, gamma, beta, groups, eps, x2, silu)
    _req(x1, "x1"), _req(gamma, "gamma"), _req(beta, "beta")
    assert x1.is_contiguous()
    B, C1 = x1.shape[0], x1.shape[-1]
    HW = x1.numel() // (B * C1)
    C2 = 0
    if x2 is not None:
        _req(x2, "x2")
        assert x2.is_contiguous() and x2.shape[0] == B
        C2 = x2.shape[-1]
    y = torch.empty(x1.shape[:-1] + (C1 + C2,), dtype=BF16, device=x1.device)
    ws = torch.empty(lib.dm4d_groupnorm_ws_bytes(B, HW, groups) // 4, dtype=torch.float32, device=x1.device)
    with _Prof("groupnorm", 2.0 * y.numel() * 2, "byte", B * HW):
        rc = lib.dm4d_groupnorm_nhwc_bf16(_stream(), _p(x1), C1, _p(x2), C2, B, HW, groups, eps, _p(gamma), _p(beta),
                                          _p(y), 1 if silu else 0, _p(ws))
    _l.check(rc, "dm4d_groupnorm_nhwc_bf16")
    _trace("groupnorm", y, x1=x1, x2=x2, gamma=gamma, beta=beta, groups=groups, eps=eps, silu=silu)
    return y


def _groupnorm_f32(x1, gamma, beta, groups, eps, x2, silu, raw_out=False):
    lib = _l.load()
    h16 = gamma.dtype == F16
    pdt = F16 if h16 else BF16
    _req(x1, "x1", F32), _req(gamma, "gamma", pdt), _req(beta, "beta", pdt)
    assert x1.is_contiguous()
    B, C1 = x1.shape[0], x1.shape[-1]
    HW = x1.numel() // (B * C1)
    C2 = 0
    if x2 is not None:
        _req(x2, "x2", F32)
        assert x2.is_contiguous() and x2.shape[0] == B
        C2 = x2.shape[-1]
    y = torch.empty(x1.shape[:-1] + ((1 if h16 else 2) * (C1 + C2),), dtype=pdt, device=x1.device)
    ws = torch.empty(lib.dm4d_groupnorm_f32_ws_bytes(B, HW, groups) // 8, dtype=torch.float64, device=x1.device)
    bpe = 6.0 if h16 else 8.0
    if raw_out:
        if not h16:
            raise _l.Dm4dError("groupnorm: raw_out is a feature of the fp16 precision")
        fused = C1 % 8 == 0 and C2 % 8 == 0 and all(t is None or t.data_ptr() % 16 == 0 for t in (x1, x2))
        if not fused:
            M = B * HW
            return (_groupnorm_f32(x1, gamma, beta, groups, eps, x2, silu),
                    split(x1.reshape(M, C1), x2.reshape(M, C2) if x2 is not None else None, h16=True).view(y.shape))
        raw = torch.empty_like(y)
        with _Prof("groupnorm", (bpe + 2.0) * (x1.numel() + (x2.numel() if x2 is not None else 0)), "byte", B * HW):
            rc = lib.dm4d_groupnorm_nhwc_f32_f16_raw(_stream(), _p(x1), C1, _p(x2), C2, B, HW, groups, eps, _p(gamma), _p(beta), _p(y), _p(raw),
                                                     1 if silu else 0, _p(ws))
        _l.check(rc, "dm4d_groupnorm_nhwc_f32_f16_raw")
        return y, raw
    with _Prof("groupnorm", bpe * x1.numel() + (bpe * x2.numel() if x2 is not None else 0.0), "byte", B * HW):
        fn = lib.dm4d_groupnorm_nhwc_f32_f16 if h16 else lib.dm4d_groupnorm_nhwc_f32_split
        rc = fn(_stream(), _p(x1), C1, _p(x2), C2, B, HW, groups, eps, _p(gamma), _p(beta), _p(y), 1 if silu else 0, _p(ws))
    _l.check(rc, "dm4d_groupnorm_nhwc_f32_split")
    return y


def _groupnorm_f16(x1, gamma, beta, groups, eps, x2, silu):
    lib = _l.load()
    _req(x1, "x1", F16), _req(gamma, "gamma", F16), _req(beta, "beta", F16)
    assert x1.is_contiguous()
    B, C1 = x1.shape[0], x1.shape[-1]
    HW = x1.numel() // (B * C1)
    C2 = 0
# ... 640 lines not shown
```

diffuman4d_amd/host/unet.py:

```python
from __future__ import annotations

import os

import json
from dataclasses import dataclass, fields
from pathlib import Path
from typing import Dict, List, Optional, Sequence, Tuple

import torch

from . import ops

BF16 = torch.bfloat16
F16 = torch.float16
PRECISIONS = ("fast", "parity", "fp16")
H16_CONV1_F16 = os.environ.get("DM4D_H16_CONV1_F16", "1") != "0"


HEAD_DIMS = (40, 64, 80, 160)


def check_precision(precision: str) -> None:
    if precision not in PRECISIONS:
        raise ValueError(f"Unsupported precision: {precision}. Supported values are 'fast', 'parity' and 'fp16'.")
# ... 78 lines not shown
    def linear(self, key: str) -> torch.Tensor:
        w = self.get(key)
        if w.ndim == 4:
            w = w.reshape(w.shape[0], w.shape[1])
        return self.mat(w)

    def conv3(self, key: str, cin_pad: Optional[int] = None, cout_pad: Optional[int] = None) -> torch.Tensor:
        w = self.get(key).float()
        co, ci = w.shape[0], w.shape[1]
        cin_pad, cout_pad = cin_pad or ci, cout_pad or co
        wp = torch.zeros(cout_pad, 3, 3, cin_pad)
        wp[:co, :, :, :ci] = w.permute(0, 2, 3, 1)
        return self.mat(wp.reshape(cout_pad, 9 * cin_pad), taps=9)


class _PoseEncoder:

    LAYERS = ((3, 3, 3, 1), (3, 16, 4, 2), (16, 16, 3, 1), (16, 32, 4, 2), (32, 32, 3, 1), (32, 64, 4, 2),
              (64, 64, 3, 1), (64, 128, 3, 1))

    def __init__(self, W: _Weights, pfx: str):
        self.layers = []
        for n, (ci, co, k, s) in enumerate(self.LAYERS):
            w = W.get(pfx + f"conv_layers.{2 * n}.weight").float()
            b = W.get(pfx + f"conv_layers.{2 * n}.bias").float()
            if tuple(w.shape) != (co, ci, k, k):
                raise ValueError(f"pose_encoder.conv_layers.{2 * n}: unexpected weight shape {tuple(w.shape)}")
            cip, cop = _round_up(ci, 4), _round_up(co, 4)
            wp, bp = torch.zeros(cop, k, k, cip), torch.zeros(cop)
            wp[:co, :, :, :ci] = w.permute(0, 2, 3, 1)
            bp[:co] = b
            dt = torch.float32 if W.wide else BF16
            self.layers.append((wp.to(W.wdtype).reshape(cop, k * k * cip).to(W.device, dt).contiguous(), bp.to(W.wdtype).to(W.device, dt), k, s))
        self.wide, self.h16 = W.wide, W.h16
        self.proj_w, self.proj_b = W.linear(pfx + "final_proj.weight"), W.vec(pfx + "final_proj.bias")
        self.scale = float(W.get(pfx + "scale").to(W.wdtype).float().reshape(-1)[0])

    def __call__(self, x: torch.Tensor, batch: int = 16) -> torch.Tensor:
        if x.shape[-1] != 4:
            raise ValueError("pose encoder input must be NHWC with 4 (3 + pad) channels")
        outs = []
        for xb in x.split(batch):
            y = xb.float().contiguous() if self.wide else xb.contiguous()
            for (w, b, k, s) in self.layers:
                y = ops.conv2d_direct(y, w, ksize=k, bias=b, stride=s, pad=1, silu=True)
            B, h, wd, C = y.shape
            y = y.view(B * h * wd, C)
            if self.wide:
                y = ops.split(y, h16=self.h16)
            outs.append(ops.gemm(y, self.proj_w, bias=self.proj_b, out_scale=self.scale, out_f32=self.wide).view(B, h, wd, -1))
        return outs[0] if len(outs) == 1 else torch.cat(outs)


class _Resnet:
    def __init__(self, W: _Weights, pfx: str, groups: int, eps: float, scale: float, temb_list: List):
        self.groups, self.eps, self.scale, self.wide, self.h16 = groups, eps, scale, W.wide, W.h16
        self.n1w, self.n1b = W.vec(pfx + "norm1.weight"), W.vec(pfx + "norm1.bias")
        self.c1w, self.c1b = W.conv3(pfx + "conv1.weight"), W.vec(pfx + "conv1.bias")
        self.n2w, self.n2b = W.vec(pfx + "norm2.weight"), W.vec(pfx + "norm2.bias")
        self.c2w, self.c2b = W.conv3(pfx + "conv2.weight"), W.vec(pfx + "conv2.bias")
        self.cout = self.c1w.shape[0]
        self.has_sc = (pfx + "conv_shortcut.weight") in W.sd
        if self.has_sc:
            self.scw, self.scb = W.linear(pfx + "conv_shortcut.weight"), W.vec(pfx + "conv_shortcut.bias")
        self.t_off = sum(t[0].shape[0] for t in temb_list)
        temb_list.append((W.get(pfx + "time_emb_proj.weight"), W.get(pfx + "time_emb_proj.bias")))

    def __call__(self, x: torch.Tensor, tproj: torch.Tensor, skip: Optional[torch.Tensor] = None) -> torch.Tensor:
        P = self.wide
        B, H, Wd = x.shape[:3]
        raw = None
        if self.h16 and self.has_sc:
            h, raw = ops.groupnorm(x, self.n1w, self.n1b, self.groups, self.eps, x2=skip, silu=True, raw_out=True)
        else:
            h = ops.groupnorm(x, self.n1w, self.n1b, self.groups, self.eps, x2=skip, silu=True)
        h = ops.conv3x3(h, self.c1w, bias=self.c1b, rowbias=tproj[:, self.t_off:self.t_off + self.cout],
                        out_f32=P and not (self.h16 and H16_CONV1_F16))
        h = ops.groupnorm(h, self.n2w, self.n2b, self.groups, self.eps, silu=True)
        if self.has_sc:
            M = B * H * Wd
            if raw is not None:
                sc = ops.gemm(raw.view(M, -1), self.scw, bias=self.scb, out_f32=True)
            elif P:
                sc = ops.gemm(ops.split(x.view(M, -1), skip.view(M, -1) if skip is not None else None, h16=self.h16), self.scw, bias=self.scb,
                              out_f32=True)
            else:
                sc = ops.gemm(x.view(M, -1), self.scw, a2=skip.view(M, -1) if skip is not None else None, bias=self.scb)
            sc = sc.view(B, H, Wd, self.cout)
        else:
            assert skip is None
            sc = x
        return ops.conv3x3(h, self.c2w, bias=self.c2b, residual=sc, out_scale=1.0 / self.scale, out_f32=P)


class _TransformerBlock:
    def __init__(self, W: _Weights, pfx: str, heads: int):
        self.heads, self.wide, self.h16 = heads, W.wide, W.h16
        self.n1w, self.n1b = W.vec(pfx + "norm1.weight"), W.vec(pfx + "norm1.bias")
        q, k, v = (W.get(pfx + f"attn1.to_{n}.weight") for n in "qkv")
        self.scale = (q.shape[0] // heads) ** -0.5
        if not W.wide:
            q = q.float() * (self.scale * ops.LOG2E)
        self.qkv = W.mat(torch.cat([q.float(), k.float(), v.float()], dim=0))
        self.ow, self.ob = W.linear(pfx + "attn1.to_out.0.weight"), W.vec(pfx + "attn1.to_out.0.bias")
        self.n3w, self.n3b = W.vec(pfx + "norm3.weight"), W.vec(pfx + "norm3.bias")
        w1, b1 = W.linear(pfx + "ff.net.0.proj.weight"), W.vec(pfx + "ff.net.0.proj.bias")
        w2, b2 = W.linear(pfx + "ff.net.2.weight"), W.vec(pfx + "ff.net.2.bias")
        self.ff = (w1, b1, w2, b2) if (W.wide and not W.h16) else ops.FeedForward(w1, b1, w2, b2)
        if (pfx + "attn2.to_q.weight") in W.sd:
            raise NotImplementedError(f"unet checkpoint holds '{pfx}attn2.*' (a cross-attention block, i.e. unet/config.json: "
                                      "cross_attention_dim is not null): not supported -- the reference never passes encoder_hidden_states "
                                      "(pipeline_diffuman4d.py:398-405)")

    def __call__(self, h: torch.Tensor, batch: int, seq: int, shard=None, operand_out: bool = False, qkv=None) -> torch.Tensor:
        if self.wide:
            return self._call_wide(h, batch, seq, shard, operand_out)
        C = h.shape[1]
        if shard is None:
            if qkv is None:
                qkv = ops.gemm(ops.layernorm(h, self.n1w, self.n1b, 1e-5), self.qkv)
            a = ops.attention(qkv[:, :C], qkv[:, C:2 * C], qkv[:, 2 * C:], batch, self.heads, seq, q_scaled=True)
        else:
            assert qkv is None
            n = ops.layernorm(h, self.n1w, self.n1b, 1e-5)
            kv = ops.gemm(n, self.qkv[C:])
            pending = shard.gather_kv_start(kv.view(batch, seq, 2 * C))
            q = ops.gemm(n, self.qkv[:C])
            kvg = shard.gather_kv_finish(pending).view(batch * shard.world * seq, 2 * C)
            a = ops.attention(q, kvg[:, :C], kvg[:, C:], batch, self.heads, seq, kv_seq=shard.world * seq, q_scaled=True)
        return self.ff.after_attention(a, self.ow, self.ob, h, (self.n3w, self.n3b, 1e-5))

    def _call_wide(self, h: torch.Tensor, batch: int, seq: int, shard=None, operand_out: bool = False) -> torch.Tensor:
        C = h.shape[1]
        n = ops.layernorm(h, self.n1w, self.n1b, 1e-5)
        if self.h16:
            qs = self.scale * ops.LOG2E
            if shard is None:
                qkv = ops.gemm(n, self.qkv, scale_cols=C, col_scale=qs)
                a = ops.attention(qkv[:, :C], qkv[:, C:2 * C], qkv[:, 2 * C:], batch, self.heads, seq, q_scaled=True)
            else:
                kv = ops.gemm(n, self.qkv[C:])
                pending = shard.gather_kv_start(kv.view(batch, seq, 2 * C))
                q = ops.gemm(n, self.qkv[:C], scale_cols=C, col_scale=qs)
                kvg = shard.gather_kv_finish(pending).view(batch * shard.world * seq, 2 * C)
                a = ops.attention(q, kvg[:, :C], kvg[:, C:], batch, self.heads, seq, kv_seq=shard.world * seq, q_scaled=True)
        elif shard is None:
            qkv = ops.gemm(n, self.qkv, split_out=True)
            a = ops.attention_split(qkv, batch, self.heads, seq, self.scale)
        else:
            kv = ops.gemm(n, self.qkv[C:], split_out=True)
            pending = shard.gather_kv_start(kv.view(batch, seq, 4 * C))
            q = ops.gemm(n, self.qkv[:C], split_out=True)
            kvg = shard.gather_kv_finish(pending).view(batch * shard.world * seq, 4 * C)
            a = ops.attention_split(None, batch, self.heads, seq, self.scale, q=q, kv=kvg, kv_seq=shard.world * seq)
        if self.h16:
            return self.ff.after_attention_f16(a, self.ow, self.ob, h, (self.n3w, self.n3b, 1e-5), out_f32=not operand_out)
        w1, b1, w2, b2 = self.ff
        h = ops.gemm(a, self.ow, bias=self.ob, residual=h, out_f32=True)
        f = ops.gemm(ops.layernorm(h, self.n3w, self.n3b, 1e-5), w1, bias=b1, geglu=True, split_out=True)
        return ops.gemm(f, w2, bias=b2, residual=h, out_f32=not operand_out, split_out=operand_out)


class _Transformer:

    def __init__(self, W: _Weights, pfx: str, heads: int, groups: int):
        self.groups, self.wide, self.h16 = groups, W.wide, W.h16
        self.nw, self.nb = W.vec(pfx + "norm.weight"), W.vec(pfx + "norm.bias")
        self.piw, self.pib = W.linear(pfx + "proj_in.weight"), W.vec(pfx + "proj_in.bias")
        self.pow, self.pob = W.linear(pfx + "proj_out.weight"), W.vec(pfx + "proj_out.bias")
        self.blocks = []
        i = 0
        while (pfx + f"transformer_blocks.{i}.norm1.weight") in W.sd:
            self.blocks.append(_TransformerBlock(W, pfx + f"transformer_blocks.{i}.", heads))
            i += 1
        d = self.pob.shape[0] // heads
        if d * heads != self.pob.shape[0] or d not in HEAD_DIMS:
            raise NotImplementedError(
                f"unet/config.json: block_out_channels / attention_head_dim give a head dimension of {d} at "
                f"'{pfx[:-1]}' ({self.pob.shape[0]} channels over {heads} heads -- `attention_head_dim` is the NUMBER of heads, "
                "unet_multiview_condition.py:222-228); the HIP attention kernels are built for head dimensions "
                + ", ".join(str(x) for x in HEAD_DIMS) + " (64: SD-2.1 geometry; 40 / 80 / 160: SD-1.x, attention_head_dim = 8)")

    def __call__(self, x: torch.Tensor, num_frames: int, shard=None) -> torch.Tensor:
        B, H, Wd, C = x.shape
        M, HW = B * H * Wd, H * Wd
        P = self.wide
        n = ops.groupnorm(x, self.nw, self.nb, self.groups, 1e-6, silu=False)
        qkv = None
        if not P and shard is None and self.blocks:
            b0 = self.blocks[0]
            h, qkv = ops.proj_in_ln_qkv(n.view(M, -1), self.piw, self.pib, (b0.n1w, b0.n1b, 1e-5), b0.qkv)
        else:
            h = ops.gemm(n.view(M, -1), self.piw, bias=self.pib, out_f32=P)
        for i, blk in enumerate(self.blocks):
            h = blk(h, B // num_frames, num_frames * HW, shard, operand_out=P and i == len(self.blocks) - 1, qkv=qkv if i == 0 else None)
        if P and not self.blocks:
            h = ops.split(h, h16=self.h16)
        return ops.gemm(h, self.pow, bias=self.pob, residual=x.view(M, C), out_f32=P).view(B, H, Wd, C)


class UNetMultiviewConditionModel:

    IN_PAD = 32

    def __init__(self, config: UNetConfig, state_dict: Dict[str, torch.Tensor], device="cuda", precision: str = "fast",
                 weight_dtype=BF16):
        cfg = self.config = config
        self.device = torch.device(device)
        check_precision(precision)
        self.precision, self.parity, self.h16 = precision, precision == "parity", precision == "fp16"
        self.wide = self.parity or self.h16
        if cfg.cross_attention_dim is not None:
            raise NotImplementedError(
                f"unet/config.json: cross_attention_dim = {cfg.cross_attention_dim}; this path builds self-attention blocks only -- the "
                "reference's UNet forward takes no encoder_hidden_states and its pipeline never passes any "
                "(unet_multiview_condition.py:290-291, :501-509; pipeline_diffuman4d.py:398-405), so cross_attention_dim must be null")
        if cfg.in_channels > 64:
            raise NotImplementedError(f"unet/config.json: in_channels = {cfg.in_channels}; conv_in is built for up to 64 input channels "
                                      "(the reference's pipeline assembles 15, or 11 with enable_pose_encoder: pipeline_diffuman4d.py:389-395)")
        self.IN_PAD = 32 if cfg.in_channels <= 32 else 64
        W = _Weights(state_dict, self.device, self.parity, self.h16, weight_dtype)
        boc = cfg.block_out_channels
        g, eps = cfg.norm_num_groups, cfg.norm_eps
        temb_list: List = []
        self.conv_in_w = W.conv3("conv_in.weight", cin_pad=self.IN_PAD)
        self.conv_in_b = W.vec("conv_in.bias")
        self.te = [W.linear("time_embedding.linear_1.weight"), W.vec("time_embedding.linear_1.bias"),
                   W.linear("time_embedding.linear_2.weight"), W.vec("time_embedding.linear_2.bias")]
        self.pose_encoder = _PoseEncoder(W, "pose_encoder.") if cfg.enable_pose_encoder else None
        self.tpe = None
        if cfg.enable_tem_embeds:
            self.tpe = [W.linear("temporal_pos_embed.linear_1.weight"), W.vec("temporal_pos_embed.linear_1.bias"),
                        W.linear("temporal_pos_embed.linear_2.weight"), W.vec("temporal_pos_embed.linear_2.bias")]
        self.down = []
        for i, t in enumerate(cfg.down_block_types):
            p = f"down_blocks.{i}."
            has_attn = t != "DownBlock2D"
            res = [_Resnet(W, p + f"resnets.{j}.", g, eps, 1.0, temb_list)
                   for j in range(cfg.layers_per_block)]
            att = [_Transformer(W, p + f"attentions.{j}.", cfg.heads(i), g) for j in range(cfg.layers_per_block)] if has_attn else None
            ds = None
            if i != len(boc) - 1:
                ds = (W.conv3(p + "downsamplers.0.conv.weight"), W.vec(p + "downsamplers.0.conv.bias"))
            self.down.append((res, att, ds))
        mp = "mid_block."
        self.mid = ([_Resnet(W, mp + f"resnets.{j}.", g, eps, cfg.mid_block_scale_factor, temb_list) for j in range(2)],
                    _Transformer(W, mp + "attentions.0.", cfg.heads(len(boc) - 1), g))
        self.up = []
        for i, t in enumerate(cfg.up_block_types):
            p = f"up_blocks.{i}."
# ... 20 lines not shown
    def from_pretrained(cls, path, device="cuda", variant: Optional[str] = None, precision: str = "fast",
                        weight_dtype=BF16) -> "UNetMultiviewConditionModel":
        from .weights import load_component_state_dict
        path = Path(path)
        cfg = UNetConfig.from_dict(json.loads((path / "config.json").read_text()))
        return cls(cfg, load_component_state_dict(path, variant), device, precision, weight_dtype)

    def _temb(self, timestep: torch.Tensor, domains: Sequence[str], num_frames: int, shard=None) -> torch.Tensor:
        cfg, P = self.config, self.wide
        c0 = cfg.block_out_channels[0]
        op = (lambda t, **kw: ops.split(t, h16=self.h16, **kw)) if P else (lambda t, silu=False: ops.silu(t) if silu else t)
        t_emb = ops.timestep_embedding(timestep.to(self.device, torch.float32), c0, cfg.flip_sin_to_cos, float(cfg.freq_shift), out_f32=P)
        emb = ops.gemm(ops.gemm(op(t_emb), self.te[0], bias=self.te[1], silu=True, split_out=P), self.te[2], bias=self.te[3], out_f32=P)
        if self.tpe is not None:
            if len(domains) * num_frames != emb.shape[0]:
                raise ValueError(f"num_frames: {num_frames} * len(domains): {len(domains)} != len(emb): {emb.shape[0]}")
            idx = []
            world = shard.world if shard is not None else 1
            for d in domains:
                if d == "spatial":
                    full = torch.zeros(num_frames * world)
                elif d == "temporal":
                    full = torch.arange(num_frames * world // 2).repeat(2).float()
                else:
                    raise ValueError(f"Invalid domain for temporal embedding: {d}")
                idx.append(full if shard is None else full[shard.local_frames(num_frames * world)])
            f_emb = ops.timestep_embedding(torch.cat(idx).to(self.device), c0, True, 0.0, out_f32=P)
            emb = ops.gemm(ops.gemm(op(f_emb), self.tpe[0], bias=self.tpe[1], silu=True, split_out=P), self.tpe[2], bias=self.tpe[3],
                           residual=emb, out_f32=P)
        return ops.gemm(op(emb, silu=True), self.tproj_w, bias=self.tproj_b, out_f32=P)

    @torch.no_grad()
    def forward(self, sample: torch.Tensor, timestep: torch.Tensor, skeletons=None, domains: Sequence[str] = ("spatial",),
                num_frames: int = 1, shard=None, pose_features: Optional[torch.Tensor] = None,
                keep_rows: Optional[torch.Tensor] = None) -> torch.Tensor:
        cfg, P = self.config, self.wide
        if sample.shape[-1] != (2 * self.IN_PAD if self.parity else self.IN_PAD):
            raise ValueError(f"sample must be NHWC with {self.IN_PAD} (padded) channels" + (" as a two-term operand [hi | lo]" if self.parity else ""))
        if sample.dtype != (F16 if self.h16 else BF16):
            raise ValueError(f"sample must be {'fp16' if self.h16 else 'bf16'} for precision '{self.precision}'")
        if sample.shape[0] % num_frames != 0:
            raise ValueError("batch must be a multiple of num_frames")
        tproj = self._temb(timestep, domains, num_frames, shard)
        if self.pose_encoder is not None:
            if pose_features is None:
                if skeletons is None:
                    raise ValueError("enable_pose_encoder: skeletons or pose_features are required")
                pose_features = self.pose_encoder(skeletons)
            if pose_features.shape[:3] != sample.shape[:3]:
                raise ValueError("pose features do not match the sample's batch / latent size")
            pose_features = pose_features.contiguous()
        else:
            pose_features = None
        x = ops.conv3x3(sample, self.conv_in_w, bias=self.conv_in_b, residual=pose_features, out_f32=P)
        skips = [x]
        nd = len(self.down)
        for i, (res, att, ds) in enumerate(self.down):
            is3d = att is not None and nd - i - 1 < cfg.num_3d_attn_blocks
            for j, r in enumerate(res):
                x = r(x, tproj)
                if att is not None:
                    x = att[j](x, num_frames if is3d else 1, shard if is3d else None)
                skips.append(x)
            if ds is not None:
                x = ops.conv3x3(ops.split(x, h16=self.h16) if P else x, ds[0], bias=ds[1], stride=2, pad=1, out_f32=P)
                skips.append(x)
        x = self.mid[0][0](x, tproj)
        x = self.mid[1](x, num_frames, shard)
        x = self.mid[0][1](x, tproj)
        def prune(x, tproj, skips):
            return (x.index_select(0, keep_rows), tproj.index_select(0, keep_rows),
                    [sk.index_select(0, keep_rows) for sk in skips])

        last3d = max((i for i, (_, att, _) in enumerate(self.up) if att is not None and i < cfg.num_3d_attn_blocks), default=-1)
        if keep_rows is not None and last3d < 0:
            x, tproj, skips = prune(x, tproj, skips)
        for i, (res, att, us) in enumerate(self.up):
            is3d = att is not None and i < cfg.num_3d_attn_blocks
            for j, r in enumerate(res):
                x = r(x, tproj, skip=skips.pop())
                if att is not None:
                    x = att[j](x, num_frames if is3d else 1, shard if is3d else None)
            if keep_rows is not None and i == last3d:
                x, tproj, skips = prune(x, tproj, skips)
            if us is not None:
                x = us(x)
        x = ops.groupnorm(x, self.no_w, self.no_b, cfg.norm_num_groups, cfg.norm_eps, silu=True)
        return ops.conv3x3(x, self.conv_out_w, bias=self.conv_out_b, out_f32=P)

    __call__ = forward
```

include/dm4d.h:

```cpp
#ifndef DM4D_H
#define DM4D_H

#include <stddef.h>
#include <stdint.h>

#ifdef __cplusplus
extern "C" {
#endif

#define DM4D_OK 0
#define DM4D_ERR_ARG -1
#define DM4D_ERR_LAUNCH -2

#define DM4D_EPI_GEGLU 1u
#define DM4D_EPI_SILU 2u
#define DM4D_EPI_F32OUT 4u
#define DM4D_EPI_F32SIDE 8u
#define DM4D_EPI_SPLITOUT 16u
#define DM4D_EPI_H16 32u

int dm4d_version(void);
const char* dm4d_last_error(void);

int dm4d_gemm_bf16(void* stream, const void* A, int64_t lda, const void* A2, int64_t lda2, int K1, const void* W,
                   int64_t ldw, void* C, int64_t ldc, int M, int N, int K, const void* bias, const void* rowbias,
                   int64_t ld_rowbias, int rows_per_rowbias, const void* residual, int64_t ld_res, unsigned flags,
                   float out_scale);

int dm4d_conv3x3_nhwc_bf16(void* stream, const void* X, int B, int H, int W, int Cin, const void* Wt, void* Y, int Ho,
                           int Wo, int Cout, int stride, int pad, int upsample, const void* bias, const void* rowbias,
                           int64_t ld_rowbias, const void* residual, int64_t ld_res, float out_scale);

size_t dm4d_conv3x3_ws_bytes(int B, int H, int W, int Cin, int Ho, int Wo, int Cout, int stride, int pad, int upsample);
int dm4d_conv3x3_nhwc_bf16_ws(void* stream, const void* X, int B, int H, int W, int Cin, const void* Wt, void* Y, int Ho,
                              int Wo, int Cout, int stride, int pad, int upsample, const void* bias, const void* rowbias,
                              int64_t ld_rowbias, const void* residual, int64_t ld_res, float out_scale, void* ws,
                              size_t ws_bytes);

int dm4d_conv3x3_nhwc_bf16_flags(void* stream, const void* X, int B, int H, int W, int Cin, const void* Wt, void* Y, int Ho,
                                 int Wo, int Cout, int stride, int pad, int upsample, const void* bias, const void* rowbias,
                                 int64_t ld_rowbias, const void* residual, int64_t ld_res, float out_scale, unsigned flags);

int dm4d_conv_up2x_prepare_bf16(void* stream, const void* W, void* Wp, int Cout, int Cin);
int dm4d_conv_up2x_nhwc_bf16(void* stream, const void* X, int B, int H, int W, int Cin, const void* Wp, void* Y, int Cout,
                             const void* bias);

int dm4d_conv2d_direct_nhwc_bf16(void* stream, const void* X, int B, int H, int W, int Cin, const void* Wt,
                                 const void* bias, void* Y, int Ho, int Wo, int Cout, int ksize, int stride, int pad,
                                 int apply_silu);
int dm4d_conv2d_direct_nhwc_f32(void* stream, const void* X, int B, int H, int W, int Cin, const void* Wt,
                                const void* bias, void* Y, int Ho, int Wo, int Cout, int ksize, int stride, int pad,
                                int apply_silu);

size_t dm4d_groupnorm_ws_bytes(int B, int HW, int groups);
int dm4d_groupnorm_nhwc_bf16(void* stream, const void* X1, int C1, const void* X2, int C2, int B, int HW, int groups,
                             float eps, const void* gamma, const void* beta, void* Y, int apply_silu, void* ws);

int dm4d_layernorm_bf16(void* stream, const void* X, int64_t ldx, const void* gamma, const void* beta, void* Y,
                        int64_t ldy, int M, int C, float eps);

int dm4d_attention_bf16(void* stream, const void* Q, const void* K, const void* V, void* O, int64_t ldq, int64_t ldk,
                        int64_t ldv, int64_t ldo, int batch, int heads, int L, float scale);

int dm4d_attention_kv_bf16(void* stream, const void* Q, const void* K, const void* V, void* O, int64_t ldq, int64_t ldk,
                           int64_t ldv, int64_t ldo, int batch, int heads, int Lq, int Lk, float scale);

#define DM4D_LOG2E 1.4426950408889634
int dm4d_attention_qscaled_kv_bf16(void* stream, const void* Q, const void* K, const void* V, void* O, int64_t ldq,
                                   int64_t ldk, int64_t ldv, int64_t ldo, int batch, int heads, int Lq, int Lk);

int dm4d_softmax_rows_bf16(void* stream, const void* S, int64_t lds, void* P, int64_t ldp, int M, int N, float scale);
int dm4d_softmax_rows_f32in_bf16(void* stream, const float* S, int64_t lds, void* P, int64_t ldp, int M, int N, float scale);

int dm4d_timestep_embedding_bf16(void* stream, const float* t, void* out, int B, int dim, int flip_sin_to_cos,
                                 float freq_shift);

int dm4d_silu_bf16(void* stream, const void* X, void* Y, int64_t n);

int dm4d_pack_model_input_bf16(void* stream, void* latents, const void* pv_lat, const void* plucker, const void* skel,
                               const void* mask, const int32_t* is_cond, const int32_t* frame_idx, void* out, int F,
                               int HW, int cpad, int use_cfg);

int dm4d_cfg_ddim_step_bf16(void* stream, void* latents, const void* noise_pred, int64_t ldn, const float* coef,
                            const int32_t* is_cond, const int32_t* frame_idx, int F, int HW, int use_cfg,
                            float guidance_scale, int v_prediction);

int dm4d_cfg_linear_step_bf16(void* stream, void* latents, void* x0_prev, const void* noise_pred, int64_t ldn,
                              const float* coef, const int32_t* is_cond, const int32_t* frame_idx, int F, int HW, int use_cfg,
                              float guidance_scale);

int dm4d_cfg_multistep_step_bf16(void* stream, void* latents, void* s1, void* s2, void* s3, const void* noise_pred, int64_t ldn,
                                 const float* coef, const int32_t* is_cond, const int32_t* frame_idx, int F, int HW, int use_cfg,
                                 float guidance_scale);

int dm4d_vae_sample_bf16(void* stream, const void* moments, int64_t ldm, const void* noise, void* out, int64_t M, int C,
                         float scale);

int dm4d_scale_pad_bf16(void* stream, const void* X, int64_t ldx, void* Y, int cpad, int64_t M, int C, float scale);

int dm4d_resize_nchw_f32_to_nhwc_bf16(void* stream, const float* X, void* Y, int B, int C, int H, int W, int h, int w,
                                      int bilinear);

int dm4d_plucker_latent_bf16(void* stream, const float* cams, void* Y, int N, int H, int W, int h, int w);

int dm4d_resize_aa_nchw_f32(void* stream, const float* X, float* Y, int64_t planes, int H, int W, int h, int w);

#define DM4D_CAPTURE_FIELDS 16
int dm4d_capture_crop_resize_f32(void* stream, const void* staging, int64_t staging_bytes, const int64_t* desc_host,
                                 const int64_t* desc_dev, int n_frames, const int32_t* tab_host, const int32_t* tab_dev, int64_t tab_len,
// ... 168 lines not shown
```

Baseline: 28.85 latents/s.

## Emit GroupNorm partial statistics from GEMM/conv epilogues to skip the stats pass

Adds a statistics variant of the conv-strip, pipe, lin2 and basic GEMM epilogues. It writes per-32-row per-column mean and M2 partials of the bf16 output, and a GroupNorm entry consumes those partials instead of re-reading the activation to reduce it. The UNet wrapper tracks which tensors carry stats and passes them through resnet blocks, attention outputs, skips and pruning. This removes one full read of each normalized activation, at the cost of extra epilogue work, a stats buffer and more complicated bookkeeping. Numerics differ slightly because the merge is pairwise over bf16-rounded outputs.

```diff
diff --git a/diffuman4d_amd/csrc/gemm.hip b/diffuman4d_amd/csrc/gemm.hip
--- a/diffuman4d_amd/csrc/gemm.hip
+++ b/diffuman4d_amd/csrc/gemm.hip
@@ -166,7 +166,7 @@
   }
 }
 
-template <int BM, int BN, int WM, int WN, int KT = 3, int PAR = 0>
+template <int BM, int BN, int WM, int WN, int KT = 3, int PAR = 0, bool ST = false>
 __global__ __launch_bounds__(WM* WN * 64, (BN % 64 != 0 ? 2 : 1)) void conv_strip2_kernel(GemmParams p_in) {
   static_assert(KT == 2 || KT == 3, "3x3 taps, or the 2x2 taps of one upsampling phase");
   constexpr int BK = 64, ROWB = BK * 2;
@@ -406,10 +406,10 @@
     p.bias = p.rowbias = p.res = nullptr;
     p.out_scale = 1.0f;
   }
-  gemm_epilogue<MI, NI, TM, TN, EpiBudget<WM * WN, MI, NI, SMEM_BYTES>::STRAIGHT, PAR>(p, acc, reinterpret_cast<float*>(smem), m0, n0, wm, wn, wave, lane);
-}
-
-template <int BM, int BN, int WM, int WN, int NST, bool CONV, int BK = 32, int PAR = 0>
+  gemm_epilogue<MI, NI, TM, TN, EpiBudget<WM * WN, MI, NI, SMEM_BYTES>::STRAIGHT, PAR, ST>(p, acc, reinterpret_cast<float*>(smem), m0, n0, wm, wn, wave, lane);
+}
+
+template <int BM, int BN, int WM, int WN, int NST, bool CONV, int BK = 32, int PAR = 0, bool ST = false>
 __global__ __launch_bounds__(WM* WN * 64) void gemm_kernel_pipe(GemmParams p) {
   constexpr int NW = WM * WN;
   static_assert(BK == 32 || BK == 64, "K-slab of 32 (64-byte row pieces) or 64 (whole 128-byte lines)");
@@ -555,10 +555,10 @@
     st = (st + 1 == NST) ? 0 : st + 1;
     st_issue = (st_issue + 1 == NST) ? 0 : st_issue + 1;
   }
-  gemm_epilogue<MI, NI, TM, TN, EpiBudget<WM * WN, MI, NI, SMEM_BYTES>::STRAIGHT, PAR>(p, acc, reinterpret_cast<float*>(smem), m0, n0, wm, wn, wave, lane);
-}
-
-template <int BM, int BN, int WM, int WN, int NST, int BK = 64, int PAR = 0>
+  gemm_epilogue<MI, NI, TM, TN, EpiBudget<WM * WN, MI, NI, SMEM_BYTES>::STRAIGHT, PAR, ST>(p, acc, reinterpret_cast<float*>(smem), m0, n0, wm, wn, wave, lane);
+}
+
+template <int BM, int BN, int WM, int WN, int NST, int BK = 64, int PAR = 0, bool ST = false>
 __global__ __launch_bounds__(WM* WN * 64) void gemm_lin2_kernel(GemmParams p) {
   static_assert(BK == 32 || BK == 64, "K-slab of 32 (64-byte rows, 16 per DMA instruction) or 64 (128-byte rows, 8 per instruction)");
   constexpr int ROWB = BK * 2, RPI = 1024 / ROWB, CPR = BK / 8, KS = BK / 16;
@@ -720,10 +720,10 @@
   asm volatile("s_waitcnt lgkmcnt(0)" ::: "memory");
   __builtin_amdgcn_s_barrier();
   asm volatile("" ::: "memory");
-  gemm_epilogue<MI, NI, TM, TN, EpiBudget<WM * WN, MI, NI, SMEM_BYTES>::STRAIGHT, PAR>(p, acc, reinterpret_cast<float*>(smem), m0, n0, wm, wn, wave, lane);
-}
-
-template <int BM, int BN, int WM, int WN, bool CONV, int PAR = 0>
+  gemm_epilogue<MI, NI, TM, TN, EpiBudget<WM * WN, MI, NI, SMEM_BYTES>::STRAIGHT, PAR, ST>(p, acc, reinterpret_cast<float*>(smem), m0, n0, wm, wn, wave, lane);
+}
+
+template <int BM, int BN, int WM, int WN, bool CONV, int PAR = 0, bool ST = false>
 __global__ __launch_bounds__(256) void gemm_kernel(GemmParams p) {
   constexpr int LDK = 40;
   constexpr int TM = BM / WM, TN = BN / WN, MI = TM / 32, NI = TN / 32;
@@ -838,7 +838,7 @@
     if (kt + 1 < nk) store_slab(buf ^ 1);
     __syncthreads();
   }
-  gemm_epilogue<MI, NI, TM, TN, EpiBudget<WM * WN, MI, NI, SMEM_BYTES>::STRAIGHT, PAR>(p, acc, reinterpret_cast<float*>(smem), m0, n0, wm, wn, wave, lane);
+  gemm_epilogue<MI, NI, TM, TN, EpiBudget<WM * WN, MI, NI, SMEM_BYTES>::STRAIGHT, PAR, ST>(p, acc, reinterpret_cast<float*>(smem), m0, n0, wm, wn, wave, lane);
 }
 
 template <int BM, int BN>
@@ -848,28 +848,29 @@
   return (unsigned)(((p.M + BM - 1) / BM) * p.tiles_n);
 }
 
-template <int BM, int BN, int WM, int WN, bool CONV, bool GLDS, int PAR = 0>
+template <int BM, int BN, int WM, int WN, bool CONV, bool GLDS, int PAR = 0, bool ST = false>
 int launch_cfg(hipStream_t st, GemmParams& p) {
   const dim3 grid(tile_grid<BM, BN>(p));
   if constexpr (GLDS) {
+    static_assert(!ST, "no statistics variant of the K-slab 64 four-wave kernels");
     hipLaunchKernelGGL((gemm_kernel_glds<BM, BN, WM, WN, CONV, PAR>), grid, dim3(256), 0, st, p);
   } else {
-    hipLaunchKernelGGL((gemm_kernel<BM, BN, WM, WN, CONV, PAR>), grid, dim3(256), 0, st, p);
+    hipLaunchKernelGGL((gemm_kernel<BM, BN, WM, WN, CONV, PAR, ST>), grid, dim3(256), 0, st, p);
   }
   return dm4d_check_launch("gemm_kernel");
 }
 
-template <int BM, int BN, int WM, int WN, int NST, bool CONV, int BK = 32, int PAR = 0>
+template <int BM, int BN, int WM, int WN, int NST, bool CONV, int BK = 32, int PAR = 0, bool ST = false>
 int launch_pipe(hipStream_t st, GemmParams& p) {
   const dim3 grid(tile_grid<BM, BN>(p));
-  hipLaunchKernelGGL((gemm_kernel_pipe<BM, BN, WM, WN, NST, CONV, BK, PAR>), grid, dim3(WM * WN * 64), 0, st, p);
+  hipLaunchKernelGGL((gemm_kernel_pipe<BM, BN, WM, WN, NST, CONV, BK, PAR, ST>), grid, dim3(WM * WN * 64), 0, st, p);
   return dm4d_check_launch("gemm_kernel_pipe");
 }
 
-template <int BM, int BN, int WM, int WN, int NST, int BK = 64, int PAR = 0>
+template <int BM, int BN, int WM, int WN, int NST, int BK = 64, int PAR = 0, bool ST = false>
 int launch_lin2(hipStream_t st, GemmParams& p) {
   const dim3 grid(tile_grid<BM, BN>(p));
-  hipLaunchKernelGGL((gemm_lin2_kernel<BM, BN, WM, WN, NST, BK, PAR>), grid, dim3(WM * WN * 64), 0, st, p);
+  hipLaunchKernelGGL((gemm_lin2_kernel<BM, BN, WM, WN, NST, BK, PAR, ST>), grid, dim3(WM * WN * 64), 0, st, p);
   return dm4d_check_launch("gemm_lin2_kernel");
 }
 
@@ -936,13 +937,14 @@
   }
 }
 
-template <int BM, int BN, int WM, int WN, int PAR = 0>
+template <int BM, int BN, int WM, int WN, int PAR = 0, bool ST = false>
 int launch_strip2(hipStream_t st, GemmParams& p) {
   if (!strip2_ok(p)) return DM4D_ERR_ARG;
   if (BN % 64 != 0 && p.splits > 1) return DM4D_ERR_ARG;
   if (p.splits < 1) p.splits = 1;
   const dim3 grid(tile_grid<BM, BN>(p) * p.splits);
-  hipLaunchKernelGGL((conv_strip2_kernel<BM, BN, WM, WN, 3, PAR>), grid, dim3(WM * WN * 64), 0, st, p);
+  if (ST && p.splits > 1) return DM4D_ERR_ARG;
+  hipLaunchKernelGGL((conv_strip2_kernel<BM, BN, WM, WN, 3, PAR, ST>), grid, dim3(WM * WN * 64), 0, st, p);
   int rc = dm4d_check_launch("conv_strip2_kernel");
   if (rc || p.splits == 1) return rc;
   const int64_t nthreads = (int64_t)p.M * (p.N / 8);
@@ -985,7 +987,23 @@
 template <int ID, bool CONV, int PAR>
 int launch_id(hipStream_t st, GemmParams& p) {
   constexpr bool STRIP = ID >= 31 && ID <= 37, LIN2 = ID >= 61;
+  constexpr bool ST = PAR == 0 && stats_id(CONV, ID);
   const bool geglu = is_geglu(p);
+  if (p.stats && !ST) return DM4D_ERR_ARG;
+  if constexpr (ST) {
+    if (p.stats) {
+      if (geglu || (STRIP && !strip_conv(p)) || (LIN2 && !lin2_ok(p))) return DM4D_ERR_ARG;
+      if constexpr (ID == 33) return launch_strip2<128, 64, 4, 1, PAR, true>(st, p);
+      else if constexpr (ID == 35) return launch_strip2<256, 320, 4, 2, PAR, true>(st, p);
+      else if constexpr (ID == 36) return launch_strip2<128, 160, 4, 1, PAR, true>(st, p);
+      else if constexpr (ID == 37) return launch_strip2<256, 160, 8, 1, PAR, true>(st, p);
+      else if constexpr (ID == 23) return launch_cfg<256, 64, 4, 1, CONV, false, PAR, true>(st, p);
+      else if constexpr (ID == 24) return launch_cfg<128, 64, 4, 1, CONV, false, PAR, true>(st, p);
+      else if constexpr (ID == 69) return launch_lin2<128, 160, 4, 1, 2, 64, PAR, true>(st, p);
+      else if constexpr (ID == 46) return k64<CONV>(p) ? launch_pipe<256, 320, 4, 2, 2, CONV, 64, PAR, true>(st, p) : DM4D_ERR_ARG;
+      else return DM4D_ERR_ARG;
+    }
+  }
   if constexpr ((STRIP && !CONV) || (LIN2 && CONV)) return DM4D_ERR_ARG;
   else if ((ID <= 4 && !k64<CONV>(p)) || (STRIP && !strip_conv(p)) || (LIN2 && !lin2_ok(p))) return DM4D_ERR_ARG;
   else if constexpr (ID == 1) return launch_cfg<128, 128, 2, 2, CONV, true, PAR>(st, p);
@@ -1039,6 +1057,17 @@
   return rc;
 }
 
+template <bool CONV>
+void attach_stats(GemmParams& p, void* stats, size_t stats_bytes, int rows_per_sample, int* wrote) {
+  p.stats = nullptr;
+  if (wrote) *wrote = 0;
+  if (!stats || !wrote || (((uintptr_t)stats) & 15)) return;
+  if (!epi_stats_ok<CONV>(p, PREC_FAST, rows_per_sample, g_tune_cfg)) return;
+  if (stats_bytes < (size_t)(p.M / 32) * p.N * 2 * sizeof(float)) return;
+  p.stats = (float*)stats;
+  *wrote = 1;
+}
+
 int arg_error(const char* name, const char* what) {
   char msg[256];
   snprintf(msg, sizeof(msg), "%s: %s", name, what);
@@ -1048,7 +1077,8 @@
 template <bool H16>
 int gemm_entry(const char* name, void* stream, const void* A, int64_t lda, const void* A2, int64_t lda2, int K1, const void* W, int64_t ldw, void* C,
                int64_t ldc, int M, int N, int K, const void* bias, const void* rowbias, int64_t ld_rowbias, int rows_per_rowbias,
-               const void* residual, int64_t ld_res, unsigned flags, float out_scale, int scale_cols, float col_scale) {
+               const void* residual, int64_t ld_res, unsigned flags, float out_scale, int scale_cols, float col_scale, void* stats = nullptr,
+               size_t stats_bytes = 0, int rows_per_sample = 0, int* stats_wrote = nullptr) {
   if (!A || !W || !C || M <= 0 || N <= 0 || K <= 0) return arg_error(name, "null pointer or empty shape");
   if (K % 32 != 0) return arg_error(name, "K must be a multiple of 32");
   if ((lda & 7) || (ldw & 7)) return arg_error(name, "lda/ldw must be multiples of 8");
@@ -1064,13 +1094,15 @@
   p.bias = (const u16*)bias; p.rowbias = (const u16*)rowbias; p.ld_rb = ld_rowbias; p.rows_per_rb = rows_per_rowbias;
   p.res = (const u16*)residual; p.ld_res = ld_res; p.flags = H16 ? flags | DM4D_EPI_H16 : flags; p.out_scale = out_scale;
   p.scale_cols = scale_cols; p.col_scale = col_scale;
+  if constexpr (!H16) attach_stats<false>(p, stats, stats_bytes, rows_per_sample, stats_wrote);
   return launch<false, H16>((hipStream_t)stream, p);
 }
 
 template <bool H16>
 int conv3x3_entry(const char* name, void* stream, const void* X, int B, int H, int W, int Cin, const void* Wt, void* Y, int Ho, int Wo, int Cout,
                   int stride, int pad, int upsample, const void* bias, const void* rowbias, int64_t ld_rowbias, const void* residual, int64_t ld_res,
-                  float out_scale, unsigned flags, void* ws, size_t ws_bytes) {
+                  float out_scale, unsigned flags, void* ws, size_t ws_bytes, void* stats = nullptr, size_t stats_bytes = 0,
+                  int* stats_wrote = nullptr) {
   if (!X || !Wt || !Y || B <= 0 || H <= 0 || W <= 0 || Ho <= 0 || Wo <= 0 || Cout <= 0) return arg_error(name, "null pointer or empty shape");
   if (Cin % 32 != 0) return arg_error(name, "Cin must be a multiple of 32 (pad the input)");
   if (stride != 1 && stride != 2) return arg_error(name, "stride must be 1 or 2");
@@ -1085,6 +1117,7 @@
   p.res = (const u16*)residual; p.ld_res = ld_res; p.flags = H16 ? flags | DM4D_EPI_H16 : flags; p.out_scale = out_scale;
   const size_t need = strip_ws_bytes(p, B);
   p.ws = (ws && need && ws_bytes >= need) ? (float*)ws : nullptr;
+  if constexpr (!H16) attach_stats<true>(p, stats, stats_bytes, Ho * Wo, stats_wrote);
   return launch<true, H16>((hipStream_t)stream, p);
 }
 
@@ -1187,6 +1220,22 @@
                               ld_res, out_scale, 0, ws, ws_bytes);
 }
 
+extern "C" int dm4d_conv3x3_nhwc_bf16_stats(void* stream, const void* X, int B, int H, int W, int Cin, const void* Wt, void* Y, int Ho, int Wo,
+                                            int Cout, int stride, int pad, int upsample, const void* bias, const void* rowbias, int64_t ld_rowbias,
+                                            const void* residual, int64_t ld_res, float out_scale, void* ws, size_t ws_bytes, void* stats,
+                                            size_t stats_bytes, int* stats_wrote) {
+  return conv3x3_entry<false>("conv3x3", stream, X, B, H, W, Cin, Wt, Y, Ho, Wo, Cout, stride, pad, upsample, bias, rowbias, ld_rowbias, residual,
+                              ld_res, out_scale, 0, ws, ws_bytes, stats, stats_bytes, stats_wrote);
+}
+
+extern "C" int dm4d_gemm_bf16_stats(void* stream, const void* A, int64_t lda, const void* A2, int64_t lda2, int K1, const void* W, int64_t ldw,
+                                    void* C, int64_t ldc, int M, int N, int K, const void* bias, const void* rowbias, int64_t ld_rowbias,
+                                    int rows_per_rowbias, const void* residual, int64_t ld_res, unsigned flags, float out_scale, void* stats,
+                                    size_t stats_bytes, int rows_per_sample, int* stats_wrote) {
+  return gemm_entry<false>("gemm", stream, A, lda, A2, lda2, K1, W, ldw, C, ldc, M, N, K, bias, rowbias, ld_rowbias, rows_per_rowbias, residual, ld_res,
+                           flags, out_scale, 0, 0.0f, stats, stats_bytes, rows_per_sample, stats_wrote);
+}
+
 extern "C" int dm4d_conv_up2x_prepare_bf16(void* stream, const void* W, void* Wp, int Cout, int Cin) {
   return conv_up2x_prepare_entry<false>("conv_up2x_prepare", stream, W, Wp, Cout, Cin);
 }
diff --git a/diffuman4d_amd/csrc/gemm_common.h b/diffuman4d_amd/csrc/gemm_common.h
--- a/diffuman4d_amd/csrc/gemm_common.h
+++ b/diffuman4d_amd/csrc/gemm_common.h
@@ -88,7 +88,119 @@
   }
 }
 
-template <int MI, int NI, int TM, int TN, int MODE, int EPW, int J0, int JN, bool SYNC, bool STRAIGHT, int PAR = 0>
+template <int CPL>
+__device__ __forceinline__ void stats_merge(float (&m)[CPL], float (&q)[CPL], const float (&m2)[CPL], const float (&q2)[CPL], float half_n) {
+#pragma clang fp contract(off)
+#pragma unroll
+  for (int e = 0; e < CPL; ++e) {
+    const float d = m[e] - m2[e];
+    q[e] = (q[e] + q2[e]) + (d * d) * half_n;
+    m[e] = (m[e] + m2[e]) * 0.5f;
+  }
+}
+
+template <int TNO, int SROWB, int CHUNKB>
+struct EpiStatsCols {
+  static constexpr int CPL = TNO >= 128 ? 2 : 1;
+  const char* col;
+
+  __device__ __forceinline__ void load(int r, float (&x)[CPL]) const {
+    if constexpr (CPL == 2) {
+      const uint32_t u = *reinterpret_cast<const uint32_t*>(col + r * SROWB);
+      x[0] = __uint_as_float(u << 16);
+      x[1] = __uint_as_float(u & 0xffff0000u);
+    } else {
+      x[0] = bf2f(*reinterpret_cast<const u16*>(col + r * SROWB));
+    }
+  }
+  template <int LO, int N>
+  __device__ __forceinline__ void node(float (&m)[CPL], float (&q)[CPL]) const {
+    if constexpr (N == 2) {
+      float a[CPL], b[CPL];
+      load(LO, a);
+      load(LO + 1, b);
+      {
+#pragma clang fp contract(off)
+#pragma unroll
+        for (int e = 0; e < CPL; ++e) {
+          const float d = a[e] - b[e];
+          m[e] = (a[e] + b[e]) * 0.5f;
+          q[e] = (d * d) * 0.5f;
+        }
+      }
+    } else {
+      float m2[CPL], q2[CPL];
+      node<LO, N / 2>(m, q);
+      node<LO + N / 2, N / 2>(m2, q2);
+      stats_merge<CPL>(m, q, m2, q2, (float)(N / 4));
+    }
+  }
+  static __device__ __forceinline__ void run(const void* stage, float* w, int lane, int ncols) {
+    const int c = lane * CPL;
+    if (c >= TNO || c >= ncols) return;
+    const EpiStatsCols me{reinterpret_cast<const char*>(stage) + (c >> 3) * CHUNKB + (c & 7) * 2};
+    float m[CPL], q[CPL];
+    me.template node<0, 32>(m, q);
+    if constexpr (CPL == 2) {
+      const f32x4_t o = {m[0], q[0], m[1], q[1]};
+      *reinterpret_cast<f32x4_t*>(w + 2 * c) = o;
+    } else {
+      const float2 o = {m[0], q[0]};
+      *reinterpret_cast<float2*>(w + 2 * c) = o;
+    }
+  }
+};
+
+template <int CPR, int SLD, int CH>
+__device__ __forceinline__ void stats_readback(const GemmParams& p, float* stage, u16* c_base, const u16* res_base, const u16* rb_base, int q0,
+                                               int r0, int lane, bool col_ok) {
+  constexpr int T = CPR / 2, cshift = CPR >= 16 ? 4 : (CPR >= 8 ? 3 : 2), cmask = CPR - 1;
+  static_assert((CPR == 4 || CPR == 8 || CPR == 16) && T % CH == 0, "8-column chunks per staged row");
+#pragma unroll
+  for (int c0 = 0; c0 < T; c0 += CH) {
+    U4 trb[CH], trs[CH];
+    if (col_ok) {
+#pragma unroll
+      for (int u = 0; u < CH; ++u) {
+        const int id = lane + (c0 + u) * 64;
+        const int row = id >> cshift, cc = id & cmask;
+        if (rb_base) trb[u] = ldg16(rb_base + (int64_t)(q0 + ((r0 + row >= p.rows_per_rb) ? 1 : 0)) * p.ld_rb + cc * 8);
+        if (res_base) trs[u] = ldg16(res_base + (uint32_t)(row * (int)p.ld_res + cc * 8));
+      }
+    }
+#pragma unroll
+    for (int u = 0; u < CH; ++u) {
+      const int id = lane + (c0 + u) * 64;
+      const int row = id >> cshift, cc = id & cmask;
+      float v[8];
+      float* s = stage + row * SLD + cc * 8;
+      const f32x4_t s0 = *reinterpret_cast<const f32x4_t*>(s), s1 = *reinterpret_cast<const f32x4_t*>(s + 4);
+      v[0] = s0[0]; v[1] = s0[1]; v[2] = s0[2]; v[3] = s0[3];
+      v[4] = s1[0]; v[5] = s1[1]; v[6] = s1[2]; v[7] = s1[3];
+      if (rb_base && col_ok) {
+        float t[8];
+        unpack8(trb[u], t);
+#pragma unroll
+        for (int e = 0; e < 8; ++e) v[e] += t[e];
+      }
+      if (res_base && col_ok) {
+        float t[8];
+        unpack8(trs[u], t);
+#pragma unroll
+        for (int e = 0; e < 8; ++e) v[e] += t[e];
+      }
+      if (p.out_scale != 1.0f) {
+#pragma unroll
+        for (int e = 0; e < 8; ++e) v[e] *= p.out_scale;
+      }
+      const U4 o = pack8(v);
+      if (col_ok) stg16(c_base + (uint32_t)(row * (int)p.ldc + cc * 8), o);
+      *reinterpret_cast<U4*>(s) = o;
+    }
+  }
+}
+
+template <int MI, int NI, int TM, int TN, int MODE, int EPW, int J0, int JN, bool SYNC, bool STRAIGHT, int PAR = 0, bool STATS = false>
 __device__ __forceinline__ void gemm_epilogue_impl(const GemmParams& p, f32x16_t (&acc)[MI][NI], float* smem_f, int m0, int n0,
                                                    int wm, int wn, int wave, int lane) {
   const int l31 = lane & 31, lh = lane >> 5;
@@ -118,6 +230,47 @@
 #pragma unroll
   for (int i = 0; i < MI; ++i) {
     const int m_base = m0 + wm * TM + i * 32;
+    if constexpr (STATS && MODE == 0 && PAR == 0 && CPR_POW2) {
+      if (p.stats && fast_ok && m_base + 32 <= p.M && (!p.rowbias || p.rows_per_rb >= 32)) {
+        const bool col_ok = ncol0 + (lane & cmask) * 8 < p.N;
+        u16* c_base = p.C + (int64_t)m_base * p.ldc + ncol0;
+        float* st_w = p.stats + ((int64_t)(m_base >> 5) * p.N + ncol0) * 2;
+        if (plain) {
+          u16* sb = reinterpret_cast<u16*>(stage);
+          stage_block<NI, MODE, J0, JN, true>(acc[i], sb + l31 * SBH + 4 * lh);
+          __builtin_amdgcn_fence(__ATOMIC_RELEASE, "wavefront");
+          __builtin_amdgcn_fence(__ATOMIC_ACQUIRE, "wavefront");
+#pragma unroll
+          for (int it = 0; it < TASKS / 64; ++it) {
+            const int id = lane + it * 64;
+            const int row = id >> cshift, cc = id & cmask;
+            const uint2* s = reinterpret_cast<const uint2*>(sb + row * SBH + cc * 8);
+            const uint2 lo = s[0], hi = s[1];
+            U4 o;
+            o.x = lo.x; o.y = lo.y; o.z = hi.x; o.w = hi.y;
+            if (col_ok) stg16(c_base + (uint32_t)(row * (int)p.ldc + cc * 8), o);
+          }
+          EpiStatsCols<TNO, SBH * 2, 16>::run(sb, st_w, lane, p.N - ncol0);
+        } else {
+          stage_block<NI, MODE, J0, JN, false>(acc[i], stage + l31 * SLD + 4 * lh);
+          __builtin_amdgcn_fence(__ATOMIC_RELEASE, "wavefront");
+          __builtin_amdgcn_fence(__ATOMIC_ACQUIRE, "wavefront");
+          int q0 = 0, r0 = 0;
+          if (p.rowbias) {
+            q0 = m_base / p.rows_per_rb;
+            r0 = m_base - q0 * p.rows_per_rb;
+          }
+          stats_readback<CPR, SLD, STRAIGHT ? 2 : 1>(p, stage, c_base, p.res ? p.res + (int64_t)m_base * p.ld_res + ncol0 : nullptr,
+                                                     p.rowbias ? p.rowbias + ncol0 : nullptr, q0, r0, lane, col_ok);
+          __builtin_amdgcn_fence(__ATOMIC_RELEASE, "wavefront");
+          __builtin_amdgcn_fence(__ATOMIC_ACQUIRE, "wavefront");
+          EpiStatsCols<TNO, SLD * 4, 32>::run(stage, st_w, lane, p.N - ncol0);
+        }
+        __builtin_amdgcn_fence(__ATOMIC_RELEASE, "wavefront");
+        __builtin_amdgcn_fence(__ATOMIC_ACQUIRE, "wavefront");
+        continue;
+      }
+    }
     if (plain) {
       u16* sb = reinterpret_cast<u16*>(stage);
       u16* srow = sb + l31 * SBH + 4 * lh;
@@ -466,18 +619,18 @@
   static constexpr int EPW = TN <= 128 ? TN : 128;
 };
 
-template <int MI, int NI, int TM, int TN, int MODE, bool STRAIGHT, int PAR = 0>
+template <int MI, int NI, int TM, int TN, int MODE, bool STRAIGHT, int PAR = 0, bool STATS = false>
 __device__ __forceinline__ void gemm_epilogue_mode(const GemmParams& p, f32x16_t (&acc)[MI][NI], float* smem_f, int m0, int n0,
                                                    int wm, int wn, int wave, int lane) {
   constexpr int NJ = MODE == 2 ? NI / 2 : NI;
   constexpr int EPW = EpiGeom<TN>::EPW;
   constexpr int G = EPW / 32;
   if constexpr (NJ <= G) {
-    gemm_epilogue_impl<MI, NI, TM, TN, MODE, EPW, 0, NJ, true, STRAIGHT, PAR>(p, acc, smem_f, m0, n0, wm, wn, wave, lane);
+    gemm_epilogue_impl<MI, NI, TM, TN, MODE, EPW, 0, NJ, true, STRAIGHT, PAR, STATS>(p, acc, smem_f, m0, n0, wm, wn, wave, lane);
   } else {
     static_assert(NJ <= 2 * G, "at most two column groups");
-    gemm_epilogue_impl<MI, NI, TM, TN, MODE, EPW, 0, G, true, STRAIGHT, PAR>(p, acc, smem_f, m0, n0, wm, wn, wave, lane);
-    gemm_epilogue_impl<MI, NI, TM, TN, MODE, EPW, G, NJ - G, false, STRAIGHT, PAR>(p, acc, smem_f, m0, n0, wm, wn, wave, lane);
+    gemm_epilogue_impl<MI, NI, TM, TN, MODE, EPW, 0, G, true, STRAIGHT, PAR, STATS>(p, acc, smem_f, m0, n0, wm, wn, wave, lane);
+    gemm_epilogue_impl<MI, NI, TM, TN, MODE, EPW, G, NJ - G, false, STRAIGHT, PAR, STATS>(p, acc, smem_f, m0, n0, wm, wn, wave, lane);
   }
 }
 
@@ -486,17 +639,17 @@
   static constexpr bool STRAIGHT = NW <= 8 && MI * NI <= 8 && !(NW == 8 && SMEM <= 80 * 1024);
 };
 
-template <int MI, int NI, int TM, int TN, bool STRAIGHT = false, int PAR = 0>
+template <int MI, int NI, int TM, int TN, bool STRAIGHT = false, int PAR = 0, bool STATS = false>
 __device__ __forceinline__ void gemm_epilogue(const GemmParams& p, f32x16_t (&acc)[MI][NI], float* smem_f, int m0, int n0,
                                               int wm, int wn, int wave, int lane) {
   if constexpr (NI >= 2 && NI % 2 == 0) {
     if (p.flags & DM4D_EPI_GEGLU) {
-      gemm_epilogue_mode<MI, NI, TM, TN, 2, STRAIGHT, PAR>(p, acc, smem_f, m0, n0, wm, wn, wave, lane);
+      gemm_epilogue_mode<MI, NI, TM, TN, 2, STRAIGHT, PAR, STATS>(p, acc, smem_f, m0, n0, wm, wn, wave, lane);
       return;
     }
   }
-  if (p.flags & DM4D_EPI_SILU) gemm_epilogue_mode<MI, NI, TM, TN, 1, STRAIGHT, PAR>(p, acc, smem_f, m0, n0, wm, wn, wave, lane);
-  else gemm_epilogue_mode<MI, NI, TM, TN, 0, STRAIGHT, PAR>(p, acc, smem_f, m0, n0, wm, wn, wave, lane);
+  if (p.flags & DM4D_EPI_SILU) gemm_epilogue_mode<MI, NI, TM, TN, 1, STRAIGHT, PAR, STATS>(p, acc, smem_f, m0, n0, wm, wn, wave, lane);
+  else gemm_epilogue_mode<MI, NI, TM, TN, 0, STRAIGHT, PAR, STATS>(p, acc, smem_f, m0, n0, wm, wn, wave, lane);
 }
 
 
diff --git a/diffuman4d_amd/csrc/gemm_params.h b/diffuman4d_amd/csrc/gemm_params.h
--- a/diffuman4d_amd/csrc/gemm_params.h
+++ b/diffuman4d_amd/csrc/gemm_params.h
@@ -31,6 +31,7 @@
   int up_w;
   int scale_cols;
   float col_scale;
+  float* stats;
 };
 
 }
diff --git a/diffuman4d_amd/csrc/gemm_select.h b/diffuman4d_amd/csrc/gemm_select.h
--- a/diffuman4d_amd/csrc/gemm_select.h
+++ b/diffuman4d_amd/csrc/gemm_select.h
@@ -150,6 +150,27 @@
   return {choose_cfg<CONV>(p), 1};
 }
 
+constexpr bool stats_id(bool conv, int id) {
+  return conv ? (id == 33 || id == 35 || id == 36 || id == 37 || id == 23 || id == 24) : (id == 69 || id == 46);
+}
+
+template <bool CONV>
+inline bool epi_stats_ok(const GemmParams& p, int prec, int hw, int forced_id) {
+  if (prec != PREC_FAST || hw < 32 || hw % 32 != 0 || p.M % hw != 0) return false;
+  if (p.up_w != 0 || p.flags != 0) return false;
+  if ((p.N & 7) || (p.ldc & 7) || p.ldc >= (1 << 24)) return false;
+  if (p.res && ((p.ld_res & 7) || p.ld_res >= (1 << 24))) return false;
+  if (p.rowbias && ((p.ld_rb & 7) || p.rows_per_rb < 32)) return false;
+  const GemmChoice c = forced_id ? GemmChoice{forced_id, 1} : select_cfg<CONV>(p, prec);
+  return c.splits <= 1 && stats_id(CONV, c.id);
+}
+
+inline bool gn_partials_ok(int C1, int C2, int HW, int groups, bool has1, bool has2) {
+  if (HW < 32 || HW % 32 != 0 || groups <= 0) return false;
+  if (C1 <= 0 || (C1 & 7) || C2 < 0 || (C2 & 7) || (C1 + C2) % groups != 0) return false;
+  return has1 && (C2 == 0 || has2);
+}
+
 inline int choose_up2x(const GemmParams& p) {
   const long tm256 = (p.M + 255) / 256;
   if (p.N % 128 == 0) return tm256 * (p.N / 128) >= 200 ? 32 : 31;
diff --git a/diffuman4d_amd/csrc/norm.hip b/diffuman4d_amd/csrc/norm.hip
--- a/diffuman4d_amd/csrc/norm.hip
+++ b/diffuman4d_amd/csrc/norm.hip
@@ -1,6 +1,7 @@
 #include "common.h"
 #include "dm4d.h"
 #include "errors.h"
+#include "gemm_select.h"
 
 namespace {
 
@@ -70,6 +71,7 @@
   int silu;
   float* ws;
   u16* Yraw;
+  const float* stat;
 };
 
 template <int IO = 0>
@@ -177,6 +179,12 @@
   const int p0 = chunk * per, p1 = min(p0 + per, p.HW);
   const int tid = threadIdx.x;
   const int gs = C / p.groups;
+  if (p.stat) {
+    for (int g = tid; g < p.groups; g += GN_THREADS) {
+      mean[g] = p.stat[((int64_t)b * p.groups + g) * 2 + 0];
+      rstd[g] = p.stat[((int64_t)b * p.groups + g) * 2 + 1];
+    }
+  } else {
   {
     const int slices = GN_THREADS / p.groups > 0 ? GN_THREADS / p.groups : 1;
     const int g = tid % p.groups, sl = tid / p.groups;
@@ -205,6 +213,7 @@
     var = var < 0.f ? 0.f : var;
     mean[g] = gn_shift<IO>(p, b, g, gs) + dm;
     rstd[g] = rsqrtf(var + p.eps);
+  }
   }
   __syncthreads();
   const int PPB = CV >= GN_THREADS ? 1 : GN_THREADS / CV;
@@ -257,6 +266,49 @@
       put(r3, px + 3 * PPB);
     }
     for (; px < p1; px += PPB) put(io::ldraw(src + (int64_t)px * ld), px);
+  }
+}
+
+struct GNFinParams {
+  const float* S1;
+  const float* S2;
+  int C1, C2, B, HW, groups;
+  float eps;
+  float* stat;
+};
+
+__global__ __launch_bounds__(GN_THREADS) void gn_finalize_kernel(GNFinParams p) {
+  __shared__ float sn[GN_THREADS], sm[GN_THREADS], sq[GN_THREADS];
+  const int b = blockIdx.x / p.groups, g = blockIdx.x % p.groups, t = threadIdx.x;
+  const int C = p.C1 + p.C2, gs = C / p.groups, nb = p.HW / 32, c0 = g * gs;
+  auto part = [&](int blk, int c) -> const float* {
+    return c < p.C1 ? p.S1 + (((int64_t)b * nb + blk) * p.C1 + c) * 2 : p.S2 + (((int64_t)b * nb + blk) * p.C2 + (c - p.C1)) * 2;
+  };
+  const float shift = part(0, c0)[0];
+  float n = 0.f, dm = 0.f, q = 0.f;
+  for (int k = t; k < nb * gs; k += GN_THREADS) {
+    const float* v = part(k / gs, c0 + k % gs);
+    const float d = (v[0] - shift) - dm, nt = n + 32.f, w = 32.f / nt;
+    dm += d * w;
+    q += v[1] + d * d * (n * w);
+    n = nt;
+  }
+  sn[t] = n; sm[t] = dm; sq[t] = q;
+  __syncthreads();
+  for (int s = GN_THREADS / 2; s > 0; s >>= 1) {
+    if (t < s && sn[t + s] > 0.f) {
+      const float na = sn[t], nb2 = sn[t + s], nt = na + nb2, w = nb2 / nt, d = sm[t + s] - sm[t];
+      sm[t] += d * w;
+      sq[t] += sq[t + s] + d * d * (na * w);
+      sn[t] = nt;
+    }
+    __syncthreads();
+  }
+  if (t == 0) {
+    float var = sq[0] / sn[0];
+    var = var < 0.f ? 0.f : var;
+    p.stat[((int64_t)b * p.groups + g) * 2 + 0] = shift + sm[0];
+    p.stat[((int64_t)b * p.groups + g) * 2 + 1] = rsqrtf(var + p.eps);
   }
 }
 
@@ -567,6 +619,33 @@
   return groupnorm_impl<0>(stream, X1, C1, X2, C2, B, HW, groups, eps, gamma, beta, Y, apply_silu, ws);
 }
 
+extern "C" int dm4d_groupnorm_partials_supported(int C1, int C2, int HW, int groups, int has1, int has2) {
+  if (!gn_partials_ok(C1, C2, HW, groups, has1 != 0, has2 != 0) || C1 + C2 > GN_MAXC) return 0;
+  int gps, SV, RPB, NV;
+  return !(g_gn_resident && gn_resident_plan(C1 + C2, HW, groups, &gps, &SV, &RPB, &NV));
+}
+
+extern "C" int dm4d_groupnorm_nhwc_bf16_partials(void* stream, const void* X1, int C1, const void* S1, const void* X2, int C2, const void* S2,
+                                                 int B, int HW, int groups, float eps, const void* gamma, const void* beta, void* Y,
+                                                 int apply_silu, void* stat) {
+  if (!X1 || !gamma || !beta || !Y || !stat || B <= 0 || HW <= 0 || groups <= 0)
+    return dm4d_set_error(DM4D_ERR_ARG, "groupnorm_partials: null pointer or empty shape");
+  if (!X2) C2 = 0;
+  if (!dm4d_groupnorm_partials_supported(C1, C2, HW, groups, S1 != nullptr, S2 != nullptr))
+    return dm4d_set_error(DM4D_ERR_ARG, "groupnorm_partials: not eligible (dm4d_groupnorm_partials_supported)");
+  const int C = C1 + C2;
+  hipStream_t st = (hipStream_t)stream;
+  const GNFinParams f{(const float*)S1, (const float*)S2, C1, C2, B, HW, groups, eps, (float*)stat};
+  hipLaunchKernelGGL(gn_finalize_kernel, dim3(B * groups), dim3(GN_THREADS), 0, st, f);
+  int rc = dm4d_check_launch("gn_finalize_kernel");
+  if (rc) return rc;
+  GNParams p{X1, X2, C1, C2, B, HW, groups, gn_nchunk(B, HW), eps, (const u16*)gamma, (const u16*)beta, (u16*)Y, apply_silu, nullptr, nullptr,
+             (const float*)stat};
+  const size_t sm2 = ((size_t)(2 * C > 2 * GN_THREADS ? 2 * C : 2 * GN_THREADS) + 2 * groups) * sizeof(float);
+  hipLaunchKernelGGL(gn_apply_kernel<0>, dim3(B * p.nchunk), dim3(GN_THREADS), sm2, st, p);
+  return dm4d_check_launch("gn_apply_kernel");
+}
+
 extern "C" int dm4d_groupnorm_f32_f16_general(void* stream, const float* X1, int C1, const float* X2, int C2, int B, int HW, int groups,
                                               float eps, const void* gamma, const void* beta, void* Y, int apply_silu, void* ws);
 extern "C" int dm4d_groupnorm_nhwc_f32_f16(void* stream, const float* X1, int C1, const float* X2, int C2, int B, int HW, int groups,
diff --git a/diffuman4d_amd/host/lib.py b/diffuman4d_amd/host/lib.py
--- a/diffuman4d_amd/host/lib.py
+++ b/diffuman4d_amd/host/lib.py
@@ -24,6 +24,12 @@
     "dm4d_conv2d_direct_nhwc_f32": (_i, [_vp, _vp, _i, _i, _i, _i, _vp, _vp, _vp, _i, _i, _i, _i, _i, _i, _i]),
     "dm4d_groupnorm_ws_bytes": (C.c_size_t, [_i, _i, _i]),
     "dm4d_groupnorm_nhwc_bf16": (_i, [_vp, _vp, _i, _vp, _i, _i, _i, _i, _f, _vp, _vp, _vp, _i, _vp]),
+    "dm4d_conv3x3_nhwc_bf16_stats": (_i, [_vp, _vp, _i, _i, _i, _i, _vp, _vp, _i, _i, _i, _i, _i, _i, _vp, _vp, _i64, _vp,
+                                          _i64, _f, _vp, C.c_size_t, _vp, C.c_size_t, C.POINTER(_i)]),
+    "dm4d_gemm_bf16_stats": (_i, [_vp, _vp, _i64, _vp, _i64, _i, _vp, _i64, _vp, _i64, _i, _i, _i, _vp, _vp, _i64, _i, _vp,
+                                  _i64, _u, _f, _vp, C.c_size_t, _i, C.POINTER(_i)]),
+    "dm4d_groupnorm_partials_supported": (_i, [_i, _i, _i, _i, _i, _i]),
+    "dm4d_groupnorm_nhwc_bf16_partials": (_i, [_vp, _vp, _i, _vp, _vp, _i, _vp, _i, _i, _i, _f, _vp, _vp, _vp, _i, _vp]),
     "dm4d_layernorm_bf16": (_i, [_vp, _vp, _i64, _vp, _vp, _vp, _i64, _i, _i, _f]),
     "dm4d_attention_bf16": (_i, [_vp, _vp, _vp, _vp, _vp, _i64, _i64, _i64, _i64, _i, _i, _i, _f]),
     "dm4d_attention_kv_bf16": (_i, [_vp, _vp, _vp, _vp, _vp, _i64, _i64, _i64, _i64, _i, _i, _i, _i, _f]),
diff --git a/diffuman4d_amd/host/ops.py b/diffuman4d_amd/host/ops.py
--- a/diffuman4d_amd/host/ops.py
+++ b/diffuman4d_amd/host/ops.py
@@ -1,5 +1,6 @@
 from __future__ import annotations
 
+import ctypes
 import os
 
 from typing import Optional, Tuple
@@ -39,11 +40,25 @@
     return None if t is None else t.data_ptr()
 
 
+GN_EPI_STATS = os.environ.get("DM4D_GN_EPI_STATS", "0") != "0"
+
+
+def gn_stats_wanted(C: int, HW: int, groups: int) -> bool:
+    return GN_EPI_STATS and bool(_l.load().dm4d_groupnorm_partials_supported(C, 0, HW, groups, 1, 0))
+
+
+def _stats_buffer(samples: int, rows_per_sample: int, N: int, device) -> Optional[torch.Tensor]:
+    if not GN_EPI_STATS or rows_per_sample < 32 or rows_per_sample % 32 or N % 8:
+        return None
+    return torch.empty((samples, rows_per_sample // 32, N, 2), dtype=F32, device=device)
+
+
 def gemm(a: torch.Tensor, w: torch.Tensor, *, a2: Optional[torch.Tensor] = None, bias=None, rowbias=None,
          rows_per_rowbias: int = 1, residual=None, geglu: bool = False, silu: bool = False, out_scale: float = 1.0,
          out: Optional[torch.Tensor] = None, out_f32: bool = False, split_out: bool = False, scale_cols: int = 0,
-         col_scale: float = 1.0) -> torch.Tensor:
+         col_scale: float = 1.0, stats_rows: int = 0):
     if isinstance(w, torch.Tensor) and w.dtype == F16:
+        assert not stats_rows
         return _gemm_f16(a, w, a2, bias, rowbias, rows_per_rowbias, residual, geglu, silu, out_scale, out, out_f32, scale_cols, col_scale)
     assert scale_cols == 0
     lib = _l.load()
@@ -71,16 +86,24 @@
     assert out.shape[1] >= ocols or out.stride(0) >= ocols
     flags = ((_l.EPI_GEGLU if geglu else 0) | (_l.EPI_SILU if silu else 0) | (_l.EPI_F32OUT if out_f32 else 0)
              | (_l.EPI_F32SIDE if f32_side else 0) | (_l.EPI_SPLITOUT if split_out else 0))
+    stats = _stats_buffer(M // stats_rows, stats_rows, N, a.device) if stats_rows > 0 and M % stats_rows == 0 and not flags else None
     with _Prof("linear", 2.0 * M * w.shape[0] * K, "flop", M):
-        rc = lib.dm4d_gemm_bf16(_stream(), _p(a), a.stride(0), _p(a2), a2.stride(0) if a2 is not None else 0,
-                                K1 if a2 is not None else 0, _p(w), w.stride(0), _p(out), out.stride(0), M, N, K,
-                                _p(bias), _p(rowbias), rowbias.stride(0) if rowbias is not None else 0,
-                                rows_per_rowbias, _p(residual), residual.stride(0) if residual is not None else 0,
-                                flags, out_scale)
+        args = (_stream(), _p(a), a.stride(0), _p(a2), a2.stride(0) if a2 is not None else 0,
+                K1 if a2 is not None else 0, _p(w), w.stride(0), _p(out), out.stride(0), M, N, K,
+                _p(bias), _p(rowbias), rowbias.stride(0) if rowbias is not None else 0,
+                rows_per_rowbias, _p(residual), residual.stride(0) if residual is not None else 0,
+                flags, out_scale)
+        if stats is not None:
+            wrote = ctypes.c_int(0)
+            rc = lib.dm4d_gemm_bf16_stats(*args, _p(stats), stats.numel() * 4, stats_rows, ctypes.byref(wrote))
+            if not wrote.value:
+                stats = None
+        else:
+            rc = lib.dm4d_gemm_bf16(*args)
     _l.check(rc, "dm4d_gemm_bf16")
     _trace("gemm", out, a=a, w=w, a2=a2, bias=bias, rowbias=rowbias, rows_per_rowbias=rows_per_rowbias, residual=residual, geglu=geglu,
            silu=silu, out_scale=out_scale, out_f32=out_f32, split_out=split_out)
-    return out
+    return (out, stats) if stats_rows > 0 else out
 
 
 def _gemm_f16(a, w, a2, bias, rowbias, rows_per_rowbias, residual, geglu, silu, out_scale, out, out_f32, scale_cols, col_scale):
@@ -127,10 +150,12 @@
 
 def conv3x3(x: torch.Tensor, wt: torch.Tensor, *, bias=None, rowbias=None, residual=None, stride: int = 1,
             pad: int = 1, pad_hi: Optional[int] = None, upsample: bool = False, out_scale: float = 1.0,
-            out_f32: bool = False) -> torch.Tensor:
+            out_f32: bool = False, stats_out: bool = False):
     lib = _l.load()
     if isinstance(wt, torch.Tensor) and wt.dtype == F16:
+        assert not stats_out
         return _conv3x3_f16(x, wt, bias, rowbias, residual, stride, pad, pad_hi, upsample, out_scale, out_f32)
+    assert not (stats_out and out_f32)
     _req(x, "x"), _req(wt, "wt")
     assert x.is_contiguous() and wt.is_contiguous()
     B, H, W, Cin = x.shape
@@ -157,15 +182,23 @@
         return y
     ws_bytes = lib.dm4d_conv3x3_ws_bytes(B, H, W, Cin, Ho, Wo, Cout, stride, pad, 1 if upsample else 0)
     ws = torch.empty(ws_bytes // 4, dtype=torch.float32, device=x.device) if ws_bytes else None
+    stats = _stats_buffer(B, Ho * Wo, Cout, x.device) if stats_out else None
     with _Prof("conv3x3", 2.0 * B * Ho * Wo * 9 * Cin * Cout, "flop", B * Ho * Wo):
-        rc = lib.dm4d_conv3x3_nhwc_bf16_ws(_stream(), _p(x), B, H, W, Cin, _p(wt), _p(y), Ho, Wo, Cout, stride, pad,
-                                           1 if upsample else 0, _p(bias), _p(rowbias),
-                                           rowbias.stride(0) if rowbias is not None else 0, _p(residual),
-                                           Cout if residual is not None else 0, out_scale, _p(ws), ws_bytes)
+        args = (_stream(), _p(x), B, H, W, Cin, _p(wt), _p(y), Ho, Wo, Cout, stride, pad,
+                1 if upsample else 0, _p(bias), _p(rowbias),
+                rowbias.stride(0) if rowbias is not None else 0, _p(residual),
+                Cout if residual is not None else 0, out_scale, _p(ws), ws_bytes)
+        if stats is not None:
+            wrote = ctypes.c_int(0)
+            rc = lib.dm4d_conv3x3_nhwc_bf16_stats(*args, _p(stats), stats.numel() * 4, ctypes.byref(wrote))
+            if not wrote.value:
+                stats = None
+        else:
+            rc = lib.dm4d_conv3x3_nhwc_bf16_ws(*args)
     _l.check(rc, "dm4d_conv3x3_nhwc_bf16_ws")
     _trace("conv3x3", y, x=x, wt=wt, bias=bias, rowbias=rowbias, residual=residual, stride=stride, pad=pad, pad_hi=pad_hi,
            upsample=upsample, out_scale=out_scale, out_f32=False)
-    return y
+    return (y, stats) if stats_out else y
 
 
 def _conv3x3_f16(x, wt, bias, rowbias, residual, stride, pad, pad_hi, upsample, out_scale, out_f32) -> torch.Tensor:
@@ -463,7 +496,8 @@
 
 
 def groupnorm(x1: torch.Tensor, gamma: torch.Tensor, beta: torch.Tensor, groups: int, eps: float, *,
-              x2: Optional[torch.Tensor] = None, silu: bool = False, raw_out: bool = False):
+              x2: Optional[torch.Tensor] = None, silu: bool = False, raw_out: bool = False,
+              stats1: Optional[torch.Tensor] = None, stats2: Optional[torch.Tensor] = None, stat_out: Optional[list] = None):
     lib = _l.load()
     if isinstance(x1, torch.Tensor) and x1.dtype == F32:
         return _groupnorm_f32(x1, gamma, beta, groups, eps, x2, silu, raw_out)
@@ -480,6 +514,21 @@
         assert x2.is_contiguous() and x2.shape[0] == B
         C2 = x2.shape[-1]
     y = torch.empty(x1.shape[:-1] + (C1 + C2,), dtype=BF16, device=x1.device)
+    if (GN_EPI_STATS and stats1 is not None
+            and lib.dm4d_groupnorm_partials_supported(C1, C2, HW, groups, 1, 1 if stats2 is not None else 0)):
+        for st, c in ((stats1, C1), (stats2, C2)):
+            if st is not None:
+                _req(st, "stats", F32)
+                assert st.is_contiguous() and tuple(st.shape) == (B, HW // 32, c, 2), (tuple(st.shape), (B, HW // 32, c, 2))
+        stat = torch.empty((B, groups, 2), dtype=F32, device=x1.device)
+        with _Prof("groupnorm", 2.0 * y.numel() * 2, "byte", B * HW):
+            rc = lib.dm4d_groupnorm_nhwc_bf16_partials(_stream(), _p(x1), C1, _p(stats1), _p(x2), C2, _p(stats2), B, HW, groups, eps,
+                                                       _p(gamma), _p(beta), _p(y), 1 if silu else 0, _p(stat))
+        _l.check(rc, "dm4d_groupnorm_nhwc_bf16_partials")
+        if stat_out is not None:
+            stat_out.append(stat)
+        _trace("groupnorm", y, x1=x1, x2=x2, gamma=gamma, beta=beta, groups=groups, eps=eps, silu=silu)
+        return y
     ws = torch.empty(lib.dm4d_groupnorm_ws_bytes(B, HW, groups) // 4, dtype=torch.float32, device=x1.device)
     with _Prof("groupnorm", 2.0 * y.numel() * 2, "byte", B * HW):
         rc = lib.dm4d_groupnorm_nhwc_bf16(_stream(), _p(x1), C1, _p(x2), C2, B, HW, groups, eps, _p(gamma), _p(beta),
diff --git a/diffuman4d_amd/host/unet.py b/diffuman4d_amd/host/unet.py
--- a/diffuman4d_amd/host/unet.py
+++ b/diffuman4d_amd/host/unet.py
@@ -154,6 +154,31 @@
         return outs[0] if len(outs) == 1 else torch.cat(outs)
 
 
+class _GNStats:
+
+    def __init__(self):
+        self.d = {}
+
+    def want(self, x: torch.Tensor, C: int, HW: int, groups: int) -> bool:
+        return x.is_cuda and x.dtype == BF16 and ops.gn_stats_wanted(C, HW, groups)
+
+    def put(self, t: torch.Tensor, stats) -> torch.Tensor:
+        if stats is not None:
+            self.d[id(t)] = (t, stats)
+        return t
+
+    def take(self, t: Optional[torch.Tensor]):
+        e = self.d.pop(id(t), None) if t is not None else None
+        return None if e is None else e[1]
+
+
+def _gn_kw(st: Optional[_GNStats], x1: torch.Tensor, x2: Optional[torch.Tensor] = None) -> Dict:
+    if st is None:
+        return {}
+    s1, s2 = st.take(x1), st.take(x2)
+    return {} if s1 is None else {"stats1": s1, "stats2": s2}
+
+
 class _Resnet:
     def __init__(self, W: _Weights, pfx: str, groups: int, eps: float, scale: float, temb_list: List):
         self.groups, self.eps, self.scale, self.wide, self.h16 = groups, eps, scale, W.wide, W.h16
@@ -168,17 +193,21 @@
         self.t_off = sum(t[0].shape[0] for t in temb_list)
         temb_list.append((W.get(pfx + "time_emb_proj.weight"), W.get(pfx + "time_emb_proj.bias")))
 
-    def __call__(self, x: torch.Tensor, tproj: torch.Tensor, skip: Optional[torch.Tensor] = None) -> torch.Tensor:
+    def __call__(self, x: torch.Tensor, tproj: torch.Tensor, skip: Optional[torch.Tensor] = None, st: Optional[_GNStats] = None) -> torch.Tensor:
         P = self.wide
         B, H, Wd = x.shape[:3]
         raw = None
         if self.h16 and self.has_sc:
             h, raw = ops.groupnorm(x, self.n1w, self.n1b, self.groups, self.eps, x2=skip, silu=True, raw_out=True)
         else:
-            h = ops.groupnorm(x, self.n1w, self.n1b, self.groups, self.eps, x2=skip, silu=True)
-        h = ops.conv3x3(h, self.c1w, bias=self.c1b, rowbias=tproj[:, self.t_off:self.t_off + self.cout],
-                        out_f32=P and not (self.h16 and H16_CONV1_F16))
-        h = ops.groupnorm(h, self.n2w, self.n2b, self.groups, self.eps, silu=True)
+            h = ops.groupnorm(x, self.n1w, self.n1b, self.groups, self.eps, x2=skip, silu=True, **_gn_kw(st, x, skip))
+        want = st is not None and not P and st.want(x, self.cout, H * Wd, self.groups)
+        if want:
+            h = st.put(*ops.conv3x3(h, self.c1w, bias=self.c1b, rowbias=tproj[:, self.t_off:self.t_off + self.cout], stats_out=True))
+        else:
+            h = ops.conv3x3(h, self.c1w, bias=self.c1b, rowbias=tproj[:, self.t_off:self.t_off + self.cout],
+                            out_f32=P and not (self.h16 and H16_CONV1_F16))
+        h = ops.groupnorm(h, self.n2w, self.n2b, self.groups, self.eps, silu=True, **_gn_kw(st, h))
         if self.has_sc:
             M = B * H * Wd
             if raw is not None:
@@ -192,6 +221,8 @@
         else:
             assert skip is None
             sc = x
+        if want:
+            return st.put(*ops.conv3x3(h, self.c2w, bias=self.c2b, residual=sc, out_scale=1.0 / self.scale, stats_out=True))
         return ops.conv3x3(h, self.c2w, bias=self.c2b, residual=sc, out_scale=1.0 / self.scale, out_f32=P)
 
 
@@ -283,11 +314,11 @@
                 "unet_multiview_condition.py:222-228); the HIP attention kernels are built for head dimensions "
                 + ", ".join(str(x) for x in HEAD_DIMS) + " (64: SD-2.1 geometry; 40 / 80 / 160: SD-1.x, attention_head_dim = 8)")
 
-    def __call__(self, x: torch.Tensor, num_frames: int, shard=None) -> torch.Tensor:
+    def __call__(self, x: torch.Tensor, num_frames: int, shard=None, st: Optional[_GNStats] = None) -> torch.Tensor:
         B, H, Wd, C = x.shape
         M, HW = B * H * Wd, H * Wd
         P = self.wide
-        n = ops.groupnorm(x, self.nw, self.nb, self.groups, 1e-6, silu=False)
+        n = ops.groupnorm(x, self.nw, self.nb, self.groups, 1e-6, silu=False, **_gn_kw(st, x))
         qkv = None
         if not P and shard is None and self.blocks:
             b0 = self.blocks[0]
@@ -298,6 +329,9 @@
             h = blk(h, B // num_frames, num_frames * HW, shard, operand_out=P and i == len(self.blocks) - 1, qkv=qkv if i == 0 else None)
         if P and not self.blocks:
             h = ops.split(h, h16=self.h16)
+        if st is not None and not P and st.want(x, C, HW, self.groups):
+            y, ys = ops.gemm(h, self.pow, bias=self.pob, residual=x.view(M, C), stats_rows=HW)
+            return st.put(y.view(B, H, Wd, C), ys)
         return ops.gemm(h, self.pow, bias=self.pob, residual=x.view(M, C), out_f32=P).view(B, H, Wd, C)
 
 
@@ -424,25 +458,41 @@
             pose_features = pose_features.contiguous()
         else:
             pose_features = None
-        x = ops.conv3x3(sample, self.conv_in_w, bias=self.conv_in_b, residual=pose_features, out_f32=P)
-        skips = [x]
+        st = None if P else _GNStats()
+        if st is not None and st.want(sample, self.conv_in_w.shape[0], sample.shape[1] * sample.shape[2], cfg.norm_num_groups):
+            x, xs = ops.conv3x3(sample, self.conv_in_w, bias=self.conv_in_b, residual=pose_features, stats_out=True)
+        else:
+            x, xs = ops.conv3x3(sample, self.conv_in_w, bias=self.conv_in_b, residual=pose_features, out_f32=P), None
+        skips, skip_stats = [x], [xs]
+        peek = lambda t: st.d.get(id(t), (None, None))[1] if st is not None else None
+        if st is not None:
+            st.put(x, xs)
         nd = len(self.down)
         for i, (res, att, ds) in enumerate(self.down):
             is3d = att is not None and nd - i - 1 < cfg.num_3d_attn_blocks
             for j, r in enumerate(res):
-                x = r(x, tproj)
+                x = r(x, tproj, st=st)
                 if att is not None:
-                    x = att[j](x, num_frames if is3d else 1, shard if is3d else None)
+                    x = att[j](x, num_frames if is3d else 1, shard if is3d else None, st=st)
                 skips.append(x)
+                skip_stats.append(peek(x))
             if ds is not None:
+                if st is not None:
+                    st.take(x)
                 x = ops.conv3x3(ops.split(x, h16=self.h16) if P else x, ds[0], bias=ds[1], stride=2, pad=1, out_f32=P)
                 skips.append(x)
-        x = self.mid[0][0](x, tproj)
-        x = self.mid[1](x, num_frames, shard)
-        x = self.mid[0][1](x, tproj)
+                skip_stats.append(None)
+        x = self.mid[0][0](x, tproj, st=st)
+        x = self.mid[1](x, num_frames, shard, st=st)
+        x = self.mid[0][1](x, tproj, st=st)
+
         def prune(x, tproj, skips):
-            return (x.index_select(0, keep_rows), tproj.index_select(0, keep_rows),
-                    [sk.index_select(0, keep_rows) for sk in skips])
+            xs = st.take(x) if st is not None else None
+            x = x.index_select(0, keep_rows)
+            if xs is not None:
+                st.put(x, xs.index_select(0, keep_rows))
+            skip_stats[:] = [None if s is None else s.index_select(0, keep_rows) for s in skip_stats]
+            return (x, tproj.index_select(0, keep_rows), [sk.index_select(0, keep_rows) for sk in skips])
 
         last3d = max((i for i, (_, att, _) in enumerate(self.up) if att is not None and i < cfg.num_3d_attn_blocks), default=-1)
         if keep_rows is not None and last3d < 0:
@@ -450,14 +500,19 @@
         for i, (res, att, us) in enumerate(self.up):
             is3d = att is not None and i < cfg.num_3d_attn_blocks
             for j, r in enumerate(res):
-                x = r(x, tproj, skip=skips.pop())
+                sk, sks = skips.pop(), skip_stats.pop()
+                if st is not None:
+                    st.put(sk, sks)
+                x = r(x, tproj, skip=sk, st=st)
                 if att is not None:
-                    x = att[j](x, num_frames if is3d else 1, shard if is3d else None)
+                    x = att[j](x, num_frames if is3d else 1, shard if is3d else None, st=st)
             if keep_rows is not None and i == last3d:
                 x, tproj, skips = prune(x, tproj, skips)
             if us is not None:
+                if st is not None:
+                    st.take(x)
                 x = us(x)
-        x = ops.groupnorm(x, self.no_w, self.no_b, cfg.norm_num_groups, cfg.norm_eps, silu=True)
+        x = ops.groupnorm(x, self.no_w, self.no_b, cfg.norm_num_groups, cfg.norm_eps, silu=True, **_gn_kw(st, x))
         return ops.conv3x3(x, self.conv_out_w, bias=self.conv_out_b, out_f32=P)
 
     __call__ = forward
diff --git a/include/dm4d.h b/include/dm4d.h
--- a/include/dm4d.h
+++ b/include/dm4d.h
@@ -55,6 +55,19 @@
 size_t dm4d_groupnorm_ws_bytes(int B, int HW, int groups);
 int dm4d_groupnorm_nhwc_bf16(void* stream, const void* X1, int C1, const void* X2, int C2, int B, int HW, int groups,
                              float eps, const void* gamma, const void* beta, void* Y, int apply_silu, void* ws);
+
+int dm4d_conv3x3_nhwc_bf16_stats(void* stream, const void* X, int B, int H, int W, int Cin, const void* Wt, void* Y, int Ho, int Wo,
+                                 int Cout, int stride, int pad, int upsample, const void* bias, const void* rowbias, int64_t ld_rowbias,
+                                 const void* residual, int64_t ld_res, float out_scale, void* ws, size_t ws_bytes, void* stats,
+                                 size_t stats_bytes, int* stats_wrote);
+int dm4d_gemm_bf16_stats(void* stream, const void* A, int64_t lda, const void* A2, int64_t lda2, int K1, const void* W, int64_t ldw,
+                         void* C, int64_t ldc, int M, int N, int K, const void* bias, const void* rowbias, int64_t ld_rowbias,
+                         int rows_per_rowbias, const void* residual, int64_t ld_res, unsigned flags, float out_scale, void* stats,
+                         size_t stats_bytes, int rows_per_sample, int* stats_wrote);
+int dm4d_groupnorm_partials_supported(int C1, int C2, int HW, int groups, int has1, int has2);
+int dm4d_groupnorm_nhwc_bf16_partials(void* stream, const void* X1, int C1, const void* S1, const void* X2, int C2, const void* S2,
+                                      int B, int HW, int groups, float eps, const void* gamma, const void* beta, void* Y,
+                                      int apply_silu, void* stat);
 
 int dm4d_layernorm_bf16(void* stream, const void* X, int64_t ldx, const void* gamma, const void* beta, void* Y,
                         int64_t ldy, int M, int C, float eps);
```

After: 28.86 latents/s, median of 4. No clear change (+0.0%).
